# raw-lab/mercat2

Measured on AMD Instinct MI355X. Metric: bases/sec at k=31, 10Mx150bp, higher is better.
Workload: dtype u64

## Files before the change

### include/mercat_hip.h

```cpp
#ifndef MERCAT_HIP_H
#define MERCAT_HIP_H

#include <stddef.h>
#include <stdint.h>

#ifdef __cplusplus
extern "C" {
#endif

#define MK_OK 0
#define MK_ERR_ARG (-1)
#define MK_ERR_HIP (-2)
#define MK_ERR_NOMEM (-3)
#define MK_ERR_STATE (-4)
#define MK_ERR_NON_ASCII (-5)
#define MK_ERR_IO (-6)
#define MK_ERR_RANGE (-7)
#define MK_ERR_UNSUPPORTED (-8)

#define MK_ALPHABET_NT2 0
#define MK_ALPHABET_AA5 1
#define MK_ALPHABET_RAW 2

typedef struct mk_ctx mk_ctx;

typedef struct mk_stats_t {
  uint64_t raw_bytes;
  uint64_t symbols;
  uint64_t windows;
  uint64_t exotic_windows;
  uint64_t chunks;
  uint64_t survivors;
  uint64_t rows;
  uint64_t table_slots;
  int32_t mode;
  int32_t profiled;
  double ms_parse, ms_pack, ms_count, ms_exotic, ms_filter, ms_export;
  uint64_t n_parse, n_pack, n_count, n_exotic, n_filter, n_export;
  double ms_part;
  uint64_t n_part;
  uint64_t records;
  uint64_t distinct;
  uint64_t part_retries;
  uint64_t part_reused;
  uint64_t fused_chunks;
  uint64_t fuse_spilled;
  uint64_t parse_retries;
} mk_stats_t;

int mk_create(int device, int alphabet, int k, mk_ctx** out);
int mk_device_count(void);
void mk_destroy(mk_ctx* ctx);
const char* mk_last_error(const mk_ctx* ctx);
int mk_reset(mk_ctx* ctx);
int mk_reset_for(mk_ctx* ctx, uint64_t expect_rows);
int mk_set_canonical(mk_ctx* ctx, int on);

int mk_set_clean(mk_ctx* ctx, int on, int toupper);
typedef struct mk_clean_gpu_t {
  uint64_t raw_bytes;
  uint64_t symbols;
  uint64_t gc_count;
  uint64_t n_bytes;
  uint64_t n_runs;
  uint64_t header_lines;
  uint64_t last_runs;
} mk_clean_gpu_t;
int mk_clean_stats(mk_ctx* ctx, mk_clean_gpu_t* out);
int mk_clean_runs(mk_ctx* ctx, uint64_t* starts, uint64_t* ends, size_t cap, size_t* n);

int mk_chunk_begin(mk_ctx* ctx);
int mk_chunk_feed(mk_ctx* ctx, const uint8_t* text, size_t n);
int mk_chunk_feed_device(mk_ctx* ctx, const uint8_t* d_text, size_t n);
int mk_chunk_end(mk_ctx* ctx, uint64_t min_count);
int mk_count_device(mk_ctx* ctx, const uint8_t* d_text, size_t n, uint64_t min_count);

typedef struct mk_file_stats_t {
  uint64_t disk_bytes;
  uint64_t text_bytes;
  uint64_t chunks;
  int32_t gz;
  int32_t chunked;
  int32_t members;
  int32_t threads;
  int32_t contexts;
  int32_t devices;
  int32_t split_pieces;
  int32_t pad_;
  double s_wait_io;
  double s_wait_gpu;
  double s_total;
  double s_merge;
  double s_setup;
  double s_scan;
  double s_feed;
  double s_retire;
  double s_drain;
} mk_file_stats_t;
int mk_count_file(mk_ctx* const* ctxs, int nctx, const char* path, uint64_t chunk_bytes, uint64_t min_count,
                  int threads, mk_file_stats_t* st);

int mk_export_size(mk_ctx* ctx, size_t* rows);
int mk_export(mk_ctx* ctx, uint8_t* kmers, uint64_t* counts, size_t rows_cap);
int mk_write_tsv(mk_ctx* ctx, const char* path, const char* basename, size_t* rows);

typedef struct mk_export_stats_t {
  uint64_t rows;
  uint64_t bytes;
  double s_sort;
  double s_d2h;
  double s_format;
  double s_write;
  double s_total;
} mk_export_stats_t;
int mk_export_stats(mk_ctx* ctx, mk_export_stats_t* out);

int mk_merged_export(mk_ctx* const* ctxs, int n, uint8_t* kmers, uint64_t* matrix, size_t rows_cap, size_t* rows);
int mk_write_merged_tsv(mk_ctx* const* ctxs, int n, const char* const* names, const char* first_column,
                        const char* path, size_t* rows);
int mk_write_merged_tsv_as_reference(mk_ctx* const* ctxs, int n, const char* const* names, const char* first_column,
                                     const char* path, size_t* rows);
int mk_write_merged_tsv_t(mk_ctx* const* ctxs, int n, const char* const* names, const char* path, size_t* rows);
typedef struct mk_alpha_t {
  uint64_t observed;
  uint64_t total;
  uint64_t freq[11];
  double sum_sq;
  double sum_clnc;
} mk_alpha_t;
int mk_alpha_stats(mk_ctx* ctx, mk_alpha_t* out);

int mk_trim(mk_ctx* ctx);

int mk_export_pairs_device(mk_ctx* ctx, uint64_t* d_keys, uint64_t* d_counts, size_t cap, size_t* rows);
int mk_import_pairs_device(mk_ctx* ctx, const uint64_t* d_keys, const uint64_t* d_counts, size_t rows);
int mk_export_exotic(mk_ctx* ctx, uint8_t* kmers, uint64_t* counts, size_t cap, size_t* rows);
int mk_import_exotic(mk_ctx* ctx, const uint8_t* kmers, const uint64_t* counts, size_t rows);
int mk_words_per_key(const mk_ctx* ctx);
int mk_merge_from(mk_ctx* dst, mk_ctx* src);

int mk_share_table(mk_ctx* ctx, mk_ctx* owner);

int mk_owner_bounds(int key_bits, int n, uint64_t* bounds);
int mk_plan_contexts(const int* devices, int ndev, int streams, int* ctx_device);
int mk_bucket_rows_device(mk_ctx* ctx, const uint64_t* bounds, int n, uint64_t* d_rows, size_t cap_rows, uint64_t* counts);
int mk_import_rows_device(mk_ctx* ctx, const uint64_t* d_rows, size_t rows);

int mk_sample_keys(mk_ctx* ctx, size_t stride, uint64_t* out, size_t cap, size_t* n);
int mk_dense_bins_device(mk_ctx* ctx, uint64_t* d_bins, size_t nbins, int store);

#define MK_MERGE_RANGES 0
#define MK_MERGE_GATHER 1
#define MK_MERGE_BALANCED 2
#define MK_MERGE_RCCL 4
typedef struct mk_merge_stats_t {
  uint64_t rows_in;
  uint64_t rows_out;
  uint64_t rows_moved;
  uint64_t bytes_moved;
  uint64_t max_owned;
  int32_t contexts, devices;
  int32_t peer_direct;
  int32_t rccl;
  double s_bucket, s_copy, s_import, s_total;
} mk_merge_stats_t;
int mk_merge_devices(mk_ctx* const* ctxs, int n, int flags, mk_merge_stats_t* st);
int mk_export_size_multi(mk_ctx* const* ctxs, int n, size_t* rows);
int mk_export_multi(mk_ctx* const* ctxs, int n, uint8_t* kmers, uint64_t* counts, size_t rows_cap);
int mk_write_tsv_multi(mk_ctx* const* ctxs, int n, const char* path, const char* basename, size_t* rows);

int mk_filter_min(mk_ctx* ctx, uint64_t min_count);

int mk_set_profiling(mk_ctx* ctx, int on);
int mk_get_stats(mk_ctx* ctx, mk_stats_t* out);
int mk_reset_stats(mk_ctx* ctx);

int mk_chunk_cuts(const uint8_t* text, size_t n, uint64_t chunksize, uint64_t* cuts, size_t cap, size_t* ncuts);
int mk_stream_cuts(const uint8_t* text, size_t n, uint64_t chunksize, size_t block, uint64_t* cuts, size_t cap,
                   size_t* ncuts);
int mk_record_cuts(const uint8_t* text, size_t n, uint64_t piece, size_t block, uint64_t* cuts, size_t cap, size_t* ncuts);
int mk_gunzip(const uint8_t* gz, size_t n, uint8_t* out, size_t cap, size_t block, size_t* written, int* members);
int mk_gunzip_parallel(const uint8_t* gz, size_t n, uint8_t* out, size_t cap, int threads, size_t piece_bytes,
                       size_t* written, int* members);
uint32_t mk_crc32_of(const uint8_t* p, size_t n, uint32_t seed);
typedef struct mk_clean_stats_t {
  uint64_t gc_count;
  uint64_t total_length;
  uint64_t records, split_records, pieces, n_runs;
  int64_t unsupported_record;
} mk_clean_stats_t;
int mk_remove_n(const uint8_t* text, size_t n, int toupper, uint8_t** out, size_t* out_len, mk_clean_stats_t* st);
void mk_free(void* p);
int mk_textwrap(const uint8_t* text, size_t n, size_t width, uint8_t** out, size_t* out_len);
int mk_synth_reads(uint64_t genome_len, uint64_t genome_seed, uint64_t reads, uint32_t read_len,
                   uint64_t read_seed, uint32_t sub_ppm, uint64_t first_index, uint8_t* out, size_t cap,
                   size_t* written);
const char* mk_version(void);

#ifdef __cplusplus
}
#endif
#endif
```

### mercat2_amd/csrc/mk_api.hip

```cpp
#include "mk_common.h"
#include <algorithm>
#include <chrono>
#include <cstdio>
#include <cstdlib>
#include <cstring>
#include <new>
#include <thread>

typedef unsigned long long u64;

static thread_local std::string g_err;

static size_t pow2_at_least(size_t v) {
  size_t p = 1024;
  while (p < v) p <<= 1;
  return p;
}

static void drain_table_users(mk_ctx* t);

int mk_buf_reserve(mk_ctx* c, MkDevBuf& b, size_t bytes, bool keep) {
  if (bytes <= b.cap) return MK_OK;
  size_t want = bytes;
  if (keep && b.cap) want = std::max(bytes, b.cap + b.cap / 2);
  want = (want + 255) & ~(size_t)255;
  void* p = nullptr;
  hipError_t e = hipMalloc(&p, want);
  if (e != hipSuccess) {
    c->err = "hipMalloc(" + std::to_string(want) + " bytes): " + hipGetErrorString(e);
    return MK_ERR_NOMEM;
  }
  if (b.p) {
    if (keep) {
      e = hipMemcpyAsync(p, b.p, b.cap, hipMemcpyDeviceToDevice, c->stream);
      if (e == hipSuccess) e = hipStreamSynchronize(c->stream);
      if (e != hipSuccess) {
        (void)hipFree(p);
        c->err = std::string("hipMemcpy (grow): ") + hipGetErrorString(e);
        return MK_ERR_HIP;
      }
    } else {
      (void)hipStreamSynchronize(c->stream);
    }
    (void)hipFree(b.p);
  }
  b.p = p;
  b.cap = want;
  return MK_OK;
}

static void buf_free(MkDevBuf& b) {
  if (b.p) (void)hipFree(b.p);
  b.p = nullptr;
  b.cap = 0;
}

static hipEvent_t get_event(mk_ctx* c) {
  if (!c->event_pool.empty()) {
    hipEvent_t e = c->event_pool.back();
    c->event_pool.pop_back();
    return e;
  }
  hipEvent_t e = nullptr;
  (void)hipEventCreate(&e);
  return e;
}

void mk_prof_begin(mk_ctx* c, int id) {
  if (!c->profile) return;
  MkEventPair p{get_event(c), get_event(c), id};
  (void)hipEventRecord(p.a, c->stream);
  c->events.push_back(p);
}

void mk_prof_end(mk_ctx* c) {
  if (!c->profile || c->events.empty()) return;
  (void)hipEventRecord(c->events.back().b, c->stream);
}

static void prof_collect(mk_ctx* c) {
  if (c->events.empty()) return;
  (void)hipStreamSynchronize(c->stream);
  double* ms[MK_K_NUM] = {&c->st.ms_parse, &c->st.ms_pack, &c->st.ms_count, &c->st.ms_exotic, &c->st.ms_filter, &c->st.ms_export, &c->st.ms_part};
  uint64_t* nn[MK_K_NUM] = {&c->st.n_parse, &c->st.n_pack, &c->st.n_count, &c->st.n_exotic, &c->st.n_filter, &c->st.n_export, &c->st.n_part};
  for (auto& p : c->events) {
    float t = 0.f;
    if (hipEventElapsedTime(&t, p.a, p.b) == hipSuccess) {
      *ms[p.id] += t;
      *nn[p.id] += 1;
    }
    c->event_pool.push_back(p.a);
    c->event_pool.push_back(p.b);
  }
  c->events.clear();
}

extern "C" const char* mk_version(void) { return "mercat_hip 4.0 (gfx950)"; }

extern "C" int mk_device_count(void) {
  int n = 0;
  if (hipGetDeviceCount(&n) != hipSuccess) { (void)hipGetLastError(); return 0; }
  return n < 0 ? 0 : n;
}

extern "C" const char* mk_last_error(const mk_ctx* c) { return c ? c->err.c_str() : g_err.c_str(); }

extern "C" int mk_words_per_key(const mk_ctx* c) { return c ? (c->mode == MK_MODE_HASH128 ? 2 : 1) : 0; }

static void fold_pending(mk_ctx* c) {
  if (!c->pending_rows) return;
  const MkChunkInfo* p = c->h_info + 1;
  if (c->mode == MK_MODE_HASH128) c->run128_rows += (size_t)p->new_rows;
  else c->run_rows += (size_t)p->new_rows;
  c->run_ref_rows += (size_t)p->new_rows_ref;
  c->pending_rows = false;
}

static int pull_info(mk_ctx* c) {
  if (c->clean_mode && c->clean_meta.p) MK_HIP(hipMemcpyAsync(c->h_clean, c->clean_meta.p, 8 * sizeof(u64), hipMemcpyDeviceToHost, c->stream));
  MK_HIP(hipMemcpyAsync(c->h_info, c->info.p, sizeof(MkChunkInfo), hipMemcpyDeviceToHost, c->stream));
  MK_HIP(hipStreamSynchronize(c->stream));
  fold_pending(c);
  return MK_OK;
}

static int settle(mk_ctx* c) {
  if (!c->pending_rows) return MK_OK;
  MK_HIP(hipSetDevice(c->device));
  MK_HIP(hipStreamSynchronize(c->stream));
  fold_pending(c);
  return MK_OK;
}

int mk_settle(mk_ctx* c) { return settle(c); }
int mk_pull_info(mk_ctx* c) { return pull_info(c); }

extern "C" int mk_create(int device, int alphabet, int k, mk_ctx** out) {
  if (!out) { g_err = "mk_create: out is NULL"; return MK_ERR_ARG; }
  *out = nullptr;
  if (k < 1 || k > (1 << 20)) { g_err = "mk_create: k must be in [1, 2^20]"; return MK_ERR_ARG; }
  if (alphabet != MK_ALPHABET_NT2 && alphabet != MK_ALPHABET_AA5 && alphabet != MK_ALPHABET_RAW) {
    g_err = "mk_create: unknown alphabet";
    return MK_ERR_ARG;
  }
  int ndev = 0;
  hipError_t e = hipGetDeviceCount(&ndev);
  if (e != hipSuccess || ndev <= 0) {
    g_err = std::string("mk_create: no HIP device (") + (e == hipSuccess ? "0 devices" : hipGetErrorString(e)) +
            "); this engine has no CPU fallback";
    return MK_ERR_HIP;
  }
  if (device < 0 || device >= ndev) { g_err = "mk_create: device index out of range"; return MK_ERR_ARG; }
  mk_ctx* c = new (std::nothrow) mk_ctx();
  if (!c) { g_err = "mk_create: out of host memory"; return MK_ERR_NOMEM; }
  c->device = device;
  c->alphabet = alphabet;
  c->k = k;
  c->bits = alphabet == MK_ALPHABET_NT2 ? 2 : (alphabet == MK_ALPHABET_AA5 ? 5 : 0);
  c->syms_per_word = alphabet == MK_ALPHABET_NT2 ? 32 : 12;
  const long kb = (long)k * c->bits;
  c->mode = (c->bits == 0) ? MK_MODE_BYREF : (kb <= 15 ? MK_MODE_DENSE : (kb <= 64 ? MK_MODE_HASH64 : MK_MODE_BYREF));
  if (alphabet == MK_ALPHABET_NT2 && k >= 33 && k <= 64) c->mode = MK_MODE_HASH128;
  if (alphabet == MK_ALPHABET_AA5 && k >= 13 && k <= 25 && !getenv("MK_NO_AA128")) c->mode = MK_MODE_HASH128;
  c->st.mode = c->mode;
  c->use_partition = getenv("MK_NO_PARTITION") ? 0 : 1;
  c->use_fast_parse = getenv("MK_NO_FAST_PARSE") ? 0 : 1;
  c->use_superkmer = getenv("MK_NO_SUPERKMER") ? 0 : 1;
  c->use_superkmer2 = getenv("MK_NO_SUPERKMER2") ? 0 : 1;
  c->run_bucket_major = (getenv("MK_BUCKET_MAJOR") && alphabet == MK_ALPHABET_NT2 && c->mode == MK_MODE_HASH64 && k >= 12 && k <= 32) ? 1 : 0;
  if (const char* e = getenv("MK_SK_MIN_K")) { const int v = atoi(e); if (v >= 12 && v <= 33) c->sk_min_k = v; }
  int rc = MK_OK;
  auto fail = [&](int code, const std::string& msg) {
    g_err = msg;
    mk_destroy(c);
    return code;
  };
  if ((e = hipSetDevice(device)) != hipSuccess) return fail(MK_ERR_HIP, std::string("hipSetDevice: ") + hipGetErrorString(e));
  if ((e = hipStreamCreateWithFlags(&c->stream, hipStreamNonBlocking)) != hipSuccess)
    return fail(MK_ERR_HIP, std::string("hipStreamCreate: ") + hipGetErrorString(e));
  c->use_speculation = getenv("MK_NO_SPECULATION") ? 0 : 1;
  c->use_reuse = getenv("MK_NO_REUSE") ? 0 : 1;
  c->use_fused = getenv("MK_NO_FUSE") ? 0 : 1;
  c->dup_hint = 2.0;
  c->nk_hint = 5.0;
  if ((e = hipHostMalloc((void**)&c->h_info, 2 * sizeof(MkChunkInfo) + 8 * sizeof(u64), hipHostMallocDefault)) != hipSuccess)
    return fail(MK_ERR_HIP, std::string("hipHostMalloc: ") + hipGetErrorString(e));
  c->h_clean = (u64*)(c->h_info + 2);
  if ((rc = mk_buf_reserve(c, c->info, sizeof(MkChunkInfo) + 64)) != MK_OK) return fail(rc, c->err);
  if (c->mode == MK_MODE_DENSE) {
    const size_t bytes = ((size_t)1 << kb) * sizeof(u64);
    if ((rc = mk_buf_reserve(c, c->ctab, bytes)) != MK_OK) return fail(rc, c->err);
    if ((rc = mk_buf_reserve(c, c->run, bytes)) != MK_OK) return fail(rc, c->err);
    (void)hipMemsetAsync(c->ctab.p, 0, bytes, c->stream);
    (void)hipMemsetAsync(c->run.p, 0, bytes, c->stream);
    c->ctab_slots = c->run_slots = (size_t)1 << kb;
  }
  if ((e = hipStreamSynchronize(c->stream)) != hipSuccess)
    return fail(MK_ERR_HIP, std::string("hipStreamSynchronize: ") + hipGetErrorString(e));
  *out = c;
  return MK_OK;
}

extern "C" void mk_destroy(mk_ctx* c) {
  if (!c) return;
  (void)hipSetDevice(c->device);
  if (c->stream) (void)hipStreamSynchronize(c->stream);
  if (c->share_owner) (void)mk_share_table(c, nullptr);
  for (mk_ctx* s : std::vector<mk_ctx*>(c->sharers)) (void)mk_share_table(s, nullptr);
  for (auto& p : c->events) { (void)hipEventDestroy(p.a); (void)hipEventDestroy(p.b); }
  for (auto& e : c->event_pool) (void)hipEventDestroy(e);
  MkDevBuf* all[] = {&c->raw, &c->seq, &c->codes, &c->bad, &c->tile_maps, &c->info, &c->ctab, &c->rtab_chunk, &c->run,
                     &c->run_ref, &c->arena, &c->run128, &c->ex128, &c->ex128_out, &c->ex_keys, &c->ex_cnts, &c->ex_keys2, &c->ex_cnts2, &c->ex_tmp, &c->part, &c->part_meta, &c->surv_keys, &c->surv_cnts, &c->surv_keys2,
                     &c->xfer_out, &c->xfer_in, &c->xfer_meta, &c->clean_meta, &c->clean_runs};
  for (auto* b : all) buf_free(*b);
  if (c->h_info) (void)hipHostFree(c->h_info);
  if (c->ingest_ring) (void)hipHostFree(c->ingest_ring);
  if (c->tsv_pin) { (void)hipHostUnregister(c->tsv_pin); free(c->tsv_pin); }
  if (c->stream) (void)hipStreamDestroy(c->stream);
  delete c;
}

static int reset_impl(mk_ctx* c, size_t expect_rows) {
  if (!c) return MK_ERR_ARG;
  MK_HIP(hipSetDevice(c->device));
  if (c->pending_rows) { MK_HIP(hipStreamSynchronize(c->stream)); c->pending_rows = false; }
  std::unique_lock<std::shared_mutex> table_lock(c->table_mu, std::defer_lock);
  if (!c->sharers.empty()) { table_lock.lock(); drain_table_users(c); }
  if (expect_rows && c->mode != MK_MODE_DENSE) {
    const size_t want = pow2_at_least(4 * expect_rows);
    if (c->run_slots > want) c->run_slots = want;
    if (c->run128_slots > want) c->run128_slots = want;
  }
  if (c->mode == MK_MODE_DENSE) {
    MK_HIP(hipMemsetAsync(c->run.p, 0, c->run_slots * sizeof(u64), c->stream));
  } else if (c->run_slots) {
    int rc = mk_launch_clear_slots(c, (MkSlot*)c->run.p, c->run_slots);
    if (rc) return rc;
  }
  if (c->run_ref_slots) {
    int rc = mk_launch_clear_slots(c, (MkSlot*)c->run_ref.p, c->run_ref_slots);
    if (rc) return rc;
  }
  if (c->run128_slots) MK_HIP(hipMemsetAsync(c->run128.p, 0, c->run128_slots * sizeof(MkSlot128), c->stream));
  c->run_rows = 0;
  c->run_ref_rows = 0;
  c->run128_rows = 0;
  c->run_side = 0;
  c->in_chunk = false;
  c->raw_len = 0;
  c->part_reuse_ok = false;
  c->dup_known = false;
  c->fuse_cap = 0;
  c->clean_n_runs = c->clean_n_bytes = c->clean_gc = c->clean_symbols = c->clean_raw = c->clean_headers = c->clean_last_runs = 0;
  MK_HIP(hipStreamSynchronize(c->stream));
  return MK_OK;
}
extern "C" int mk_reset(mk_ctx* c) { return reset_impl(c, 0); }
extern "C" int mk_reset_for(mk_ctx* c, uint64_t expect_rows) { return reset_impl(c, (size_t)(expect_rows ? expect_rows : 1)); }

extern "C" int mk_set_canonical(mk_ctx* c, int on) {
  if (!c) return MK_ERR_ARG;
  { int rc_ = settle(c); if (rc_) return rc_; }
  if (on && c->alphabet != MK_ALPHABET_NT2) { c->err = "mk_set_canonical: only the nucleotide alphabet has a reverse complement"; return MK_ERR_ARG; }
  if (on && c->mode != MK_MODE_DENSE && c->mode != MK_MODE_HASH64 && !(c->mode == MK_MODE_HASH128 && c->use_superkmer2)) {
    c->err = "mk_set_canonical: canonical counting is implemented for nucleotide k <= 64 (two-word keys: on the partitioned path only)";
    return MK_ERR_ARG;
  }
  c->part_reuse_ok = false;
  if (c->in_chunk || c->run_rows || c->run_ref_rows || c->run128_rows || c->run_side || c->st.chunks) {
    if ((on != 0) != (c->canonical != 0) && (c->run_rows || c->run_ref_rows || c->run128_rows || c->run_side || c->in_chunk)) {
      c->err = "mk_set_canonical: the running table already holds rows counted in the other mode (mk_reset first)";
      return MK_ERR_STATE;
    }
  }
  c->canonical = on ? 1 : 0;
  return MK_OK;
}

extern "C" int mk_set_clean(mk_ctx* c, int on, int toupper) {
  if (!c) return MK_ERR_ARG;
  if (on && c->alphabet != MK_ALPHABET_NT2) { c->err = "mk_set_clean: removeN applies to nucleotide FASTA (bin/mercat2.py:276)"; return MK_ERR_ARG; }
  if (c->in_chunk) { c->err = "mk_set_clean: a chunk is open"; return MK_ERR_STATE; }
  c->clean_mode = on ? 1 : 0;
  c->clean_upper = (on && toupper) ? 1 : 0;
  return MK_OK;
}

extern "C" int mk_clean_stats(mk_ctx* c, mk_clean_gpu_t* out) {
  if (!c || !out) return MK_ERR_ARG;
  out->raw_bytes = c->clean_raw;
  out->symbols = c->clean_symbols;
  out->gc_count = c->clean_gc;
  out->n_bytes = c->clean_n_bytes;
  out->n_runs = c->clean_n_runs;
  out->header_lines = c->clean_headers;
  out->last_runs = c->clean_last_runs;
  return MK_OK;
}

extern "C" int mk_clean_runs(mk_ctx* c, uint64_t* starts, uint64_t* ends, size_t cap, size_t* n) {
  if (!c || !n || (cap && (!starts || !ends))) return MK_ERR_ARG;
  if ((size_t)c->clean_last_runs > ((size_t)1 << 16)) {
    *n = 0;
    c->err = "mk_clean_runs: the last chunk holds " + std::to_string(c->clean_last_runs) + " runs of N, more than the 65536 the list keeps";
    return MK_ERR_RANGE;
  }
  const size_t kept = (size_t)c->clean_last_runs;
  *n = kept;
  if (!kept || !cap) return MK_OK;
  MK_HIP(hipSetDevice(c->device));
  std::vector<u64> a(kept), b(kept);
  MK_HIP(hipMemcpyAsync(a.data(), c->clean_runs.p, kept * 8, hipMemcpyDeviceToHost, c->stream));
  MK_HIP(hipMemcpyAsync(b.data(), (const u64*)c->clean_runs.p + ((size_t)1 << 16), kept * 8, hipMemcpyDeviceToHost, c->stream));
  MK_HIP(hipStreamSynchronize(c->stream));
  std::sort(a.begin(), a.end());
  std::sort(b.begin(), b.end());
  for (size_t i = 0; i < kept && i < cap; ++i) { starts[i] = a[i]; ends[i] = b[i]; }
  return MK_OK;
}

static int grow_run64(mk_ctx* c, size_t need_rows);
static int grow_run64_body(mk_ctx* c, size_t need_rows);
static mk_ctx* table_of_ctx(mk_ctx* c) { return c->share_owner ? c->share_owner : c; }

static void drain_table_users(mk_ctx* t) {
  (void)hipStreamSynchronize(t->stream);
  for (mk_ctx* s : t->sharers) (void)hipStreamSynchronize(s->stream);
}

extern "C" int mk_share_table(mk_ctx* c, mk_ctx* owner) {
  if (!c || c == owner) return MK_ERR_ARG;
  if (c->in_chunk) { c->err = "mk_share_table: a chunk is open"; return MK_ERR_STATE; }
  if (c->share_owner == owner) return MK_OK;
  if (c->share_owner) {
    mk_ctx* old = c->share_owner;
    std::unique_lock<std::shared_mutex> wr(old->table_mu);
    (void)hipSetDevice(c->device);
    (void)hipStreamSynchronize(c->stream);
    old->sharers.erase(std::remove(old->sharers.begin(), old->sharers.end(), c), old->sharers.end());
    c->share_owner = nullptr;
    c->fuse_target = nullptr;
  }
  if (!owner) return MK_OK;
  if (owner->share_owner || !c->sharers.empty()) { c->err = "mk_share_table: tables are shared one level deep (the owner must own its table, a sharer cannot be an owner)"; return MK_ERR_ARG; }
  if (owner->device != c->device || owner->alphabet != c->alphabet || owner->k != c->k || owner->canonical != c->canonical || owner->mode != c->mode) {
    c->err = "mk_share_table: contexts differ in device, alphabet, k or canonical mode";
    return MK_ERR_ARG;
  }
  if (c->mode != MK_MODE_HASH64) { c->err = "mk_share_table: only one-word hashed tables are shared"; return MK_ERR_ARG; }
  std::unique_lock<std::shared_mutex> wr(owner->table_mu);
  owner->sharers.push_back(c);
  c->share_owner = owner;
  return MK_OK;
}

extern "C" int mk_chunk_begin(mk_ctx* c) {
  if (!c) return MK_ERR_ARG;
  if (c->in_chunk) { c->err = "mk_chunk_begin: a chunk is already open"; return MK_ERR_STATE; }
  c->in_chunk = true;
  c->raw_len = 0;
  return MK_OK;
}

static int feed(mk_ctx* c, const uint8_t* p, size_t n, hipMemcpyKind kind) {
  if (!c) return MK_ERR_ARG;
  if (!c->in_chunk) { c->err = "mk_chunk_feed: no open chunk (call mk_chunk_begin)"; return MK_ERR_STATE; }
  if (n == 0) return MK_OK;
  if (!p) { c->err = "mk_chunk_feed: text is NULL"; return MK_ERR_ARG; }
  MK_HIP(hipSetDevice(c->device));
  int rc = mk_buf_reserve(c, c->raw, c->raw_len + n + 64, true);
  if (rc) return rc;
  MK_HIP(hipMemcpyAsync((uint8_t*)c->raw.p + c->raw_len, p, n, kind, c->stream));
  if (kind == hipMemcpyHostToDevice) MK_HIP(hipStreamSynchronize(c->stream));
  c->raw_len += n;
  return MK_OK;
}

int mk_feed_host_async(mk_ctx* c, const uint8_t* p, size_t n, bool wait) {
  if (!c || !c->in_chunk) return MK_ERR_STATE;
  if (n == 0) return MK_OK;
  MK_HIP(hipSetDevice(c->device));
  int rc = mk_buf_reserve(c, c->raw, c->raw_len + n + 64, true);
  if (rc) return rc;
  MK_HIP(hipMemcpyAsync((uint8_t*)c->raw.p + c->raw_len, p, n, hipMemcpyHostToDevice, c->stream));
  if (wait) MK_HIP(hipStreamSynchronize(c->stream));
  c->raw_len += n;
  return MK_OK;
}

int mk_reserve_raw(mk_ctx* c, size_t bytes) {
  MK_HIP(hipSetDevice(c->device));
  return mk_buf_reserve(c, c->raw, bytes, true);
}

extern "C" int mk_chunk_feed(mk_ctx* c, const uint8_t* text, size_t n) { return feed(c, text, n, hipMemcpyHostToDevice); }
extern "C" int mk_chunk_feed_device(mk_ctx* c, const uint8_t* d_text, size_t n) {
  return feed(c, d_text, n, hipMemcpyDeviceToDevice);
}

static size_t run_slots_for(size_t need_rows) {
  static const bool x4 = getenv("MK_GROW_X4") != nullptr;
  return pow2_at_least(x4 ? 4 * need_rows : need_rows * 5 / 2);
}

static int grow_run64_body(mk_ctx* c, size_t need_rows);
static int grow_run64(mk_ctx* c, size_t need_rows) {
  if (c->sharers.empty()) return grow_run64_body(c, need_rows);
  std::unique_lock<std::shared_mutex> wr(c->table_mu);
  if (2 * need_rows <= c->run_slots) return MK_OK;
  drain_table_users(c);
  return grow_run64_body(c, need_rows);
}
static int grow_run64_body(mk_ctx* c, size_t need_rows) {
  if (2 * need_rows <= c->run_slots) return MK_OK;
  const size_t slots = run_slots_for(need_rows);
  MkDevBuf nb;
  int rc = mk_buf_reserve(c, nb, slots * sizeof(MkSlot));
  if (rc) return rc;
  if ((rc = mk_launch_clear_slots(c, (MkSlot*)nb.p, slots)) != MK_OK) return rc;
  if (c->run_slots && (rc = mk_launch_rehash64(c, (const MkSlot*)c->run.p, c->run_slots, (MkSlot*)nb.p, slots)) != MK_OK) return rc;
  MK_HIP(hipStreamSynchronize(c->stream));
  buf_free(c->run);
  c->run = nb;
  c->run_slots = slots;
  return MK_OK;
}

static int grow_run128(mk_ctx* c, size_t need_rows) {
  if (2 * need_rows <= c->run128_slots) return MK_OK;
  const size_t slots = pow2_at_least(4 * need_rows);
  MkDevBuf nb;
  int rc = mk_buf_reserve(c, nb, slots * sizeof(MkSlot128));
  if (rc) return rc;
  MK_HIP(hipMemsetAsync(nb.p, 0, slots * sizeof(MkSlot128), c->stream));
  if (c->run128_slots && (rc = mk_launch_rehash128(c, (const MkSlot128*)c->run128.p, c->run128_slots, (MkSlot128*)nb.p, slots)) != MK_OK) return rc;
  MK_HIP(hipStreamSynchronize(c->stream));
  buf_free(c->run128);
  c->run128 = nb;
  c->run128_slots = slots;
  return MK_OK;
}

static int grow_run_ref(mk_ctx* c, size_t need_rows) {
  int rc;
  if (need_rows > c->arena_rows_cap) {
    const size_t rows = std::max(need_rows, c->arena_rows_cap * 2);
    if ((rc = mk_buf_reserve(c, c->arena, rows * (size_t)c->k + 64, true)) != MK_OK) return rc;
    c->arena_rows_cap = rows;
  }
  if (2 * need_rows <= c->run_ref_slots) return MK_OK;
  const size_t slots = pow2_at_least(4 * need_rows);
  MkDevBuf nb;
  if ((rc = mk_buf_reserve(c, nb, slots * sizeof(MkSlot))) != MK_OK) return rc;
  if ((rc = mk_launch_clear_slots(c, (MkSlot*)nb.p, slots)) != MK_OK) return rc;
  if (c->run_ref_slots &&
      (rc = mk_launch_rehash_ref(c, (const MkSlot*)c->run_ref.p, c->run_ref_slots, (MkSlot*)nb.p, slots)) != MK_OK)
    return rc;
  MK_HIP(hipStreamSynchronize(c->stream));
  buf_free(c->run_ref);
  c->run_ref = nb;
  c->run_ref_slots = slots;
  return MK_OK;
}

int mk_grow_run(mk_ctx* c, size_t more_rows) {
  if (c->mode == MK_MODE_HASH64) return grow_run64(c, c->run_rows + more_rows);
  if (c->mode == MK_MODE_HASH128) return grow_run128(c, c->run128_rows + more_rows);
  return MK_OK;
}

bool mk_binned_takes(const mk_ctx* c);
int mk_launch_count_binned(mk_ctx* c, size_t seq_len, uint64_t min_count);

#define MK_RETRY_GENERAL 1

static int process_chunk_fast(mk_ctx* c, const uint8_t* d_raw, size_t n, u64 min_count) {
  int rc;
  const size_t begin = (size_t)((uintptr_t)d_raw & 15);
  const uint8_t* d_al = d_raw - begin;
  MK_HIP(hipSetDevice(c->device));
  MK_HIP(hipMemsetAsync(c->info.p, 0, sizeof(MkChunkInfo), c->stream));
  if ((rc = mk_buf_reserve(c, c->seq, n + 256)) != MK_OK) return rc;
  const size_t bad_words = n / 64 + 4;
  if ((rc = mk_buf_reserve(c, c->bad, (bad_words + 2) * 8)) != MK_OK) return rc;
  if ((rc = mk_buf_reserve(c, c->codes, (2 * bad_words + 8) * 8)) != MK_OK) return rc;
  static const bool always_seq = getenv("MK_ALWAYS_SEQ") != nullptr;
  if ((rc = mk_launch_fparse(c, d_al, begin, n, true, always_seq)) != MK_OK) return rc;
  const bool two = c->mode == MK_MODE_HASH128;
  c->rtab_chunk_slots = 0;
  c->surv_regions = 0;
  c->ctab_slots = 0;
  c->fuse_cap = 0;
  if (!two && c->use_fused && min_count >= 2 && c->surv_hint_ok && !c->run_bucket_major) {
    static const bool cores = getenv("MK_CORES") != nullptr;
    const unsigned long long per_bucket = (c->surv_hint >> 13) * (cores ? 2 : 1);
    const int cap = per_bucket <= 110 ? 512 : (per_bucket <= 360 ? 1024 : 0);
    if (cap) {
      if ((rc = settle(c)) != MK_OK) return rc;
      mk_ctx* t = table_of_ctx(c);
      static const bool roomy = getenv("MK_FUSE_ROOMY") != nullptr;
      const size_t expect = (roomy ? 2 * (size_t)c->surv_hint : (size_t)c->surv_hint) + 4096;
      if (t != c) {
        std::shared_lock<std::shared_mutex> rd(t->table_mu);
        size_t rows_now;
        { std::lock_guard<std::mutex> g(t->rows_mu); rows_now = t->run_rows; }
        if (t->run_slots < 1024 || 2 * (rows_now + expect) > t->run_slots) t = c;
      }
      if (t == c) {
        size_t rows_now;
        { std::lock_guard<std::mutex> g(c->rows_mu); rows_now = c->run_rows; }
        if ((rc = grow_run64(c, rows_now + expect * (1 + c->sharers.size()))) != MK_OK) return rc;
      }
      c->fuse_target = t;
      c->fuse_cap = cap;
    }
  }
  {
    mk_ctx* t = c->fuse_cap ? c->fuse_target : c;
    std::shared_lock<std::shared_mutex> rd(t->table_mu, std::defer_lock);
    if (t != c) rd.lock();
    rc = two ? mk_launch_count_superkmer2(c, n, min_count) : mk_launch_count_superkmer(c, n, min_count);
  }
  c->fuse_cap = 0;
  if (rc) return rc;
  const bool fused = !two && c->fused_last;
  if ((rc = pull_info(c)) != MK_OK) return rc;
  MkChunkInfo* h = c->h_info;
  if (h->parse_fallback) { c->st.parse_retries += 1; return MK_RETRY_GENERAL; }
  if (h->non_ascii) {
    c->err = "input holds " + std::to_string(h->non_ascii) +
             " sequence byte(s) >= 0x80 (non-ASCII sequence text is not supported; the chunk was not counted)";
    return MK_ERR_NON_ASCII;
  }
  const size_t seq_len = (size_t)h->seq_len;
  if (h->bad_symbols) {
    if (!always_seq) {
      if ((rc = mk_buf_reserve(c, c->ex_tmp, sizeof(MkChunkInfo) + 64)) != MK_OK) return rc;
      MK_HIP(hipMemcpyAsync(c->ex_tmp.p, c->info.p, sizeof(MkChunkInfo), hipMemcpyDeviceToDevice, c->stream));
      if ((rc = mk_launch_fparse(c, d_al, begin, n, false, true)) != MK_OK) return rc;
      MK_HIP(hipMemcpyAsync(c->info.p, c->ex_tmp.p, sizeof(MkChunkInfo), hipMemcpyDeviceToDevice, c->stream));
    }
    const u64 bound = std::min<u64>((u64)seq_len, h->bad_symbols * (u64)c->k);
    c->rtab_chunk_slots = pow2_at_least(2 * (size_t)bound);
    if ((rc = mk_buf_reserve(c, c->rtab_chunk, c->rtab_chunk_slots * sizeof(MkSlot))) != MK_OK) return rc;
    if ((rc = mk_launch_clear_slots(c, (MkSlot*)c->rtab_chunk.p, c->rtab_chunk_slots)) != MK_OK) return rc;
    if ((rc = mk_launch_count_byref(c, seq_len, true)) != MK_OK) return rc;
    if ((rc = mk_launch_count_survivors(c, min_count)) != MK_OK) return rc;
    if ((rc = pull_info(c)) != MK_OK) return rc;
  }
  if (h->part_overflow) {
    if (!c->part_sampled) { c->err = "partition overflow without sampling (internal error)"; return MK_ERR_STATE; }
    if (getenv("MK_VERBOSE")) fprintf(stderr, "[mk] sampled partition too small (where=%llu): exact pass\n", h->part_overflow);
    h->windows = h->records = h->distinct = h->survivors = h->side = h->errors = h->part_overflow = 0;
    MK_HIP(hipMemcpyAsync(c->info.p, h, sizeof(MkChunkInfo), hipMemcpyHostToDevice, c->stream));
    c->st.part_retries += 1;
    rc = two ? mk_launch_count_superkmer2(c, seq_len, min_count, true) : mk_launch_count_superkmer(c, seq_len, min_count, true);
    if (rc) return rc;
    if ((rc = pull_info(c)) != MK_OK) return rc;
    if (h->part_overflow) { c->err = "partition overflow after the exact pass (internal error: nothing was counted)"; return MK_ERR_STATE; }
  }
  if (h->errors) {
    c->err = "counting kernel reported " + std::to_string(h->errors) + " unrecoverable condition(s) (bucket too large to split)";
    return MK_ERR_RANGE;
  }
  c->part_dirty = false;
  const bool fused_done = !two && c->fused_last;
  if (fused_done) {
    {
      mk_ctx* t = c->fuse_target ? c->fuse_target : c;
      std::lock_guard<std::mutex> g(t->rows_mu);
      t->run_rows += (size_t)h->new_rows;
    }
    h->new_rows = 0;
    c->st.fused_chunks += 1;
    c->st.fuse_spilled += h->spilled;
    if (h->spilled || h->survivors_ref)
      MK_HIP(hipMemsetAsync(&((MkChunkInfo*)c->info.p)->new_rows, 0, sizeof(unsigned long long), c->stream));
    if (h->spilled) {
      if ((rc = grow_run64(c, c->run_rows + (size_t)h->spilled)) != MK_OK) return rc;
      if ((rc = mk_launch_import_pairs(c, (const uint64_t*)c->surv_keys.p, (const uint64_t*)c->surv_cnts.p, (size_t)h->spilled)) != MK_OK) return rc;
    }
  }
  (void)fused;
  if (!two && !fused_done && h->survivors && (rc = grow_run64(c, c->run_rows + (size_t)h->survivors)) != MK_OK) return rc;
  if (h->survivors_ref && (rc = grow_run_ref(c, c->run_ref_rows + (size_t)h->survivors_ref)) != MK_OK) return rc;
  if (two && (h->survivors || h->survivors_ref) &&
      (rc = grow_run128(c, c->run128_rows + (size_t)h->survivors + (size_t)h->survivors_ref)) != MK_OK) return rc;
  if (h->survivors && seq_len && !fused_done) {
    const size_t p1 = (size_t)1 << c->p1_log2;
    const uint64_t* meta = (const uint64_t*)c->part_meta.p;
    mk_prof_begin(c, MK_K_FILTER);
    rc = two ? mk_launch_import128_regions(c, (const uint64_t*)c->surv_keys.p, (const uint64_t*)c->surv_keys2.p,
                                           (const uint64_t*)c->surv_cnts.p, meta + 4 * p1 + 1, meta + 6 * p1 + 2, p1)
             : mk_launch_import_regions(c, (const uint64_t*)c->surv_keys.p, (const uint64_t*)c->surv_cnts.p,
                                        meta + 4 * p1 + 1, meta + 6 * p1 + 2, p1, (size_t)h->survivors);
    mk_prof_end(c);
    if (rc) return rc;
  }
  if ((rc = mk_launch_accumulate(c, min_count)) != MK_OK) return rc;
  if (!fused_done || h->spilled || h->survivors_ref) {
    MK_HIP(hipMemcpyAsync(c->h_info + 1, c->info.p, sizeof(MkChunkInfo), hipMemcpyDeviceToHost, c->stream));
    c->pending_rows = true;
  }
  if (h->side && h->side >= min_count) c->run_side += h->side;
  const bool full_chunk = !c->dup_known || seq_len * 4 >= c->part_prev_len * 3;
  if (!two && (full_chunk || !c->surv_hint_ok)) { c->surv_hint = h->survivors; c->surv_hint_ok = true; }
  if (h->distinct && full_chunk) { c->dup_hint = (double)h->windows / (double)h->distinct; c->dup_known = true; }
  if (h->records) { c->nk_hint = (double)(h->windows + h->exotic) / (double)h->records; c->items_hint = (double)h->records * 32.0 / (double)(seq_len ? seq_len : 1); }
  if (getenv("MK_VERBOSE"))
    fprintf(stderr, "[mk] chunk (one read-back): raw=%zu seq=%zu windows=%llu records=%llu distinct=%llu survivors=%llu p1=2^%d dup=%.2f nk=%.2f fused=%d spilled=%llu rows=%zu slots=%zu\n",
            n, seq_len, (unsigned long long)h->windows, (unsigned long long)h->records, (unsigned long long)h->distinct,
            (unsigned long long)h->survivors, c->p1_log2, c->dup_hint, c->nk_hint, fused_done ? 1 : 0, (unsigned long long)h->spilled,
            c->run_rows, c->run_slots);
  c->st.table_slots = c->rtab_chunk_slots;
  c->st.raw_bytes += n;
  c->st.symbols += h->symbols;
  c->st.windows += h->windows + h->exotic;
  c->st.exotic_windows += h->exotic;
  c->st.chunks += 1;
  c->st.records += h->records;
  c->st.distinct += h->distinct;
  c->st.survivors += h->survivors + h->survivors_ref + ((h->side && h->side >= min_count) ? 1 : 0);
  return MK_OK;
}

static int process_chunk(mk_ctx* c, const uint8_t* d_raw, size_t n, u64 min_count) {
  int rc;
  bool known_blank = false;
  if (c->clean_mode) {
    if (!c->use_fast_parse) { c->err = "clean mode needs the fast parser (MK_NO_FAST_PARSE is set)"; return MK_ERR_UNSUPPORTED; }
    if (d_raw != (const uint8_t*)c->raw.p) { c->err = "clean mode rewrites the text in place: feed it (mk_chunk_feed), do not pass caller memory"; return MK_ERR_STATE; }
    MK_HIP(hipSetDevice(c->device));
    if ((rc = mk_launch_clean_pre(c, (uint8_t*)c->raw.p, n)) != MK_OK) return rc;
  }
  if (!c->clean_mode && c->use_speculation && c->use_fast_parse && c->alphabet == MK_ALPHABET_NT2 && n && n < 0xFE000000ull &&
      ((c->mode == MK_MODE_HASH64 && c->use_partition && c->use_superkmer && c->k >= c->sk_min_k && c->k <= 32) ||
       (c->mode == MK_MODE_HASH128 && c->use_superkmer2))) {
    rc = process_chunk_fast(c, d_raw, n, min_count);
    if (rc != MK_RETRY_GENERAL) return rc;
    known_blank = true;
  }
  if ((rc = settle(c)) != MK_OK) return rc;
  const size_t begin = (size_t)((uintptr_t)d_raw & 15);
  const uint8_t* d_al = d_raw - begin;
  MK_HIP(hipSetDevice(c->device));
  MK_HIP(hipMemsetAsync(c->info.p, 0, sizeof(MkChunkInfo), c->stream));
  if ((rc = mk_buf_reserve(c, c->seq, n + 256)) != MK_OK) return rc;
  const bool packed = c->mode != MK_MODE_BYREF;
  const size_t bad_words = n / 64 + 4;
  const size_t code_words = c->alphabet == MK_ALPHABET_NT2 ? 2 * bad_words : (bad_words * 64 + 11) / 12;
  if (packed) {
    if ((rc = mk_buf_reserve(c, c->bad, (bad_words + 2) * 8)) != MK_OK) return rc;
    if ((rc = mk_buf_reserve(c, c->codes, (code_words + 8) * 8)) != MK_OK) return rc;
  }
  for (int attempt = 0; attempt < 2; ++attempt) {
    const bool fast = c->use_fast_parse && attempt == 0 && !known_blank;
    const bool fused = fast && packed && c->alphabet == MK_ALPHABET_NT2;
    if (!fast && begin) {
      if ((rc = mk_buf_reserve(c, c->raw, n + 64)) != MK_OK) return rc;
      MK_HIP(hipMemcpyAsync(c->raw.p, d_raw, n, hipMemcpyDeviceToDevice, c->stream));
      d_raw = (const uint8_t*)c->raw.p;
    }
    if ((rc = fast ? mk_launch_fparse(c, d_al, begin, n, fused) : mk_launch_parse(c, d_raw, n)) != MK_OK) return rc;
    if (packed && !fused && (rc = mk_launch_pack(c, n)) != MK_OK) return rc;
    if (c->clean_mode && (rc = mk_launch_clean_post(c, n)) != MK_OK) return rc;
    if ((rc = pull_info(c)) != MK_OK) return rc;
    if (c->clean_mode) {
      const u64* m = c->h_clean;
      const u64 headers = c->h_info->seq_len - c->h_info->symbols;
      const char* why = c->h_info->parse_fallback ? "a blank inside a sequence line"
                        : m[2]                    ? "a 0x7F byte in the text, or blanks in front of the first header"
                        : m[1] != headers         ? "a '>' that does not start a header line"
                                                  : nullptr;
      if (why) {
        c->err = std::string("clean mode: ") + why + " (removeN's rewrite of such text is not reproduced on the GPU; nothing was counted)";
        return MK_ERR_UNSUPPORTED;
      }
      c->clean_raw += n;
      c->clean_headers += headers;
      c->clean_n_bytes += m[3];
      c->clean_n_runs += m[4];
      c->clean_gc += m[5];
      c->clean_symbols += c->h_info->symbols - m[3];
      c->clean_last_runs = m[4];
      c->h_info->symbols -= m[3];
      break;
    }
    if (!fast || !c->h_info->parse_fallback) break;
    c->st.parse_retries += 1;
    MK_HIP(hipMemsetAsync(c->info.p, 0, sizeof(MkChunkInfo), c->stream));
  }
  if (c->h_info->non_ascii) {
    c->err = "input holds " + std::to_string(c->h_info->non_ascii) +
             " sequence byte(s) >= 0x80 (non-ASCII sequence text is not supported; the chunk was not counted)";
    return MK_ERR_NON_ASCII;
  }
  const size_t seq_len = (size_t)c->h_info->seq_len;
  const u64 bad_symbols = c->h_info->bad_symbols;

  c->rtab_chunk_slots = 0;
  const bool partitioned = c->mode == MK_MODE_HASH64 && c->use_partition;
  c->surv_regions = 0;
  c->ctab_slots = c->mode == MK_MODE_DENSE ? c->ctab_slots : 0;
  if (c->mode == MK_MODE_HASH64 && !partitioned) {
    c->ctab_slots = pow2_at_least(2 * seq_len);
    if ((rc = mk_buf_reserve(c, c->ctab, c->ctab_slots * sizeof(MkSlot))) != MK_OK) return rc;
    if ((rc = mk_launch_clear_slots(c, (MkSlot*)c->ctab.p, c->ctab_slots)) != MK_OK) return rc;
  }
  const bool sk2 = c->mode == MK_MODE_HASH128 && c->alphabet == MK_ALPHABET_NT2 && c->use_superkmer2 && seq_len < 0xFFFFFF00ull;
  if (c->mode == MK_MODE_HASH128 && c->canonical && !sk2) {
    c->err = "canonical counting of 33..64-mers needs the partitioned path (chunk of 4 G symbols or more)";
    return MK_ERR_RANGE;
  }
  if (c->mode == MK_MODE_BYREF || (c->mode == MK_MODE_HASH128 && !sk2)) {
    c->rtab_chunk_slots = pow2_at_least(2 * seq_len);
  } else if (bad_symbols) {
    const u64 bound = std::min<u64>((u64)seq_len, bad_symbols * (u64)c->k);
    c->rtab_chunk_slots = pow2_at_least(2 * (size_t)bound);
  }
  if (c->rtab_chunk_slots) {
    if ((rc = mk_buf_reserve(c, c->rtab_chunk, c->rtab_chunk_slots * sizeof(MkSlot))) != MK_OK) return rc;
    if ((rc = mk_launch_clear_slots(c, (MkSlot*)c->rtab_chunk.p, c->rtab_chunk_slots)) != MK_OK) return rc;
  }
  c->st.table_slots = (c->mode == MK_MODE_BYREF || c->mode == MK_MODE_HASH128) ? c->rtab_chunk_slots : c->ctab_slots;

  if (c->mode == MK_MODE_DENSE) rc = mk_launch_count_dense(c, seq_len);
  else if (partitioned) {
    const bool sk = c->use_superkmer && c->alphabet == MK_ALPHABET_NT2 && c->k >= c->sk_min_k && c->k <= 32 && seq_len < 0xFE000000ull;
    const bool binned = !sk && mk_binned_takes(c) && seq_len < 0xFFFFFF00ull;
    rc = sk ? mk_launch_count_superkmer(c, seq_len, min_count)
            : (binned ? mk_launch_count_binned(c, seq_len, min_count) : mk_launch_count_partitioned(c, seq_len, min_count));
  }
  else if (c->mode == MK_MODE_HASH64) rc = mk_launch_count_hash64(c, seq_len);
  else if (c->mode == MK_MODE_HASH128) rc = sk2 ? mk_launch_count_superkmer2(c, seq_len, min_count) : mk_launch_count_ref128(c, seq_len);
  if (rc) return rc;
  if (c->rtab_chunk_slots && (c->mode != MK_MODE_HASH128 || bad_symbols) &&
      (rc = mk_launch_count_byref(c, seq_len, packed)) != MK_OK) return rc;

  if ((rc = mk_launch_count_survivors(c, min_count)) != MK_OK) return rc;
  if ((rc = pull_info(c)) != MK_OK) return rc;
  if (c->h_info->part_overflow) {
    if (!c->part_sampled) { c->err = "partition overflow without sampling (internal error)"; return MK_ERR_STATE; }
    MkChunkInfo* h = c->h_info;
    if (getenv("MK_VERBOSE")) fprintf(stderr, "[mk] sampled partition too small (where=%llu: 1 records total, 2 survivors total, 4 a bucket, 8 a survivor region): exact pass\n", h->part_overflow);
    h->windows = h->records = h->distinct = h->survivors = h->side = h->errors = h->part_overflow = 0;
    MK_HIP(hipMemcpyAsync(c->info.p, h, sizeof(MkChunkInfo), hipMemcpyHostToDevice, c->stream));
    c->st.part_retries += 1;
    rc = sk2 ? mk_launch_count_superkmer2(c, seq_len, min_count, true)
             : mk_launch_count_superkmer(c, seq_len, min_count, true);
    if (rc) return rc;
    if ((rc = pull_info(c)) != MK_OK) return rc;
    if (c->h_info->part_overflow) { c->err = "partition overflow after the exact pass (internal error: nothing was counted)"; return MK_ERR_STATE; }
  }
  if (c->h_info->errors) {
    c->err = "counting kernel reported " + std::to_string(c->h_info->errors) + " unrecoverable condition(s) (bucket too large to split)";
    return MK_ERR_RANGE;
  }
  c->part_dirty = false;
  if (c->mode == MK_MODE_HASH64 && c->h_info->survivors)
    if ((rc = grow_run64(c, c->run_rows + (size_t)c->h_info->survivors)) != MK_OK) return rc;
  if (c->h_info->survivors_ref)
    if ((rc = grow_run_ref(c, c->run_ref_rows + (size_t)c->h_info->survivors_ref)) != MK_OK) return rc;
  if (c->mode == MK_MODE_HASH128 && (c->h_info->survivors || c->h_info->survivors_ref))
    if ((rc = grow_run128(c, c->run128_rows + (size_t)c->h_info->survivors + (size_t)c->h_info->survivors_ref)) != MK_OK) return rc;
  if (sk2 && c->surv_regions == 2 && seq_len && c->h_info->survivors) {
    const size_t p1 = (size_t)1 << c->p1_log2;
    const uint64_t* meta = (const uint64_t*)c->part_meta.p;
    mk_prof_begin(c, MK_K_FILTER);
    rc = mk_launch_import128_regions(c, (const uint64_t*)c->surv_keys.p, (const uint64_t*)c->surv_keys2.p,
                                     (const uint64_t*)c->surv_cnts.p, meta + 4 * p1 + 1, meta + 6 * p1 + 2, p1);
    mk_prof_end(c);
    if (rc) return rc;
  }
  if (partitioned && c->h_info->survivors) {
    mk_prof_begin(c, MK_K_FILTER);
    if (c->surv_regions) {
      const size_t p1 = (size_t)1 << c->p1_log2;
      const uint64_t* meta = (const uint64_t*)c->part_meta.p;
      rc = mk_launch_import_regions(c, (const uint64_t*)c->surv_keys.p, (const uint64_t*)c->surv_cnts.p,
                                    meta + 4 * p1 + 1, meta + 6 * p1 + 2, p1, (size_t)c->h_info->survivors);
    } else {
      rc = mk_launch_import_pairs(c, (const uint64_t*)c->surv_keys.p, (const uint64_t*)c->surv_cnts.p, (size_t)c->h_info->survivors, true);
    }
    mk_prof_end(c);
    if (rc) return rc;
  }
  if ((rc = mk_launch_accumulate(c, min_count)) != MK_OK) return rc;
  if ((rc = pull_info(c)) != MK_OK) return rc;
  if (c->mode == MK_MODE_HASH128) c->run128_rows += (size_t)c->h_info->new_rows;
  else c->run_rows += (size_t)c->h_info->new_rows;
  c->run_ref_rows += (size_t)c->h_info->new_rows_ref;
  if (c->h_info->side && c->h_info->side >= min_count) c->run_side += c->h_info->side;
  if (partitioned && c->h_info->distinct) { c->dup_hint = (double)c->h_info->windows / (double)c->h_info->distinct; c->dup_known = true; }
  if (sk2 && c->h_info->distinct) { c->dup_hint = (double)c->h_info->windows / (double)c->h_info->distinct; c->dup_known = true; }
  if ((partitioned || sk2) && c->h_info->records) {
    c->nk_hint = (double)(c->h_info->windows + c->h_info->exotic) / (double)c->h_info->records;
    c->items_hint = (double)c->h_info->records * 32.0 / (double)(seq_len ? seq_len : 1);
  }

  if (getenv("MK_VERBOSE"))
    fprintf(stderr, "[mk] chunk: raw=%zu seq=%zu windows=%llu records=%llu distinct=%llu survivors=%llu new_rows=%llu p1=2^%d dup=%.2f nk=%.2f\n", n, seq_len,
            (unsigned long long)c->h_info->windows, (unsigned long long)c->h_info->records, (unsigned long long)c->h_info->distinct,
            (unsigned long long)c->h_info->survivors, (unsigned long long)c->h_info->new_rows, c->p1_log2, c->dup_hint, c->nk_hint);
  c->st.raw_bytes += n;
  c->st.symbols += c->h_info->symbols;
  c->st.windows += c->h_info->windows + c->h_info->exotic;
  c->st.exotic_windows += c->h_info->exotic;
  c->st.chunks += 1;
  c->st.records += c->h_info->records;
  c->st.distinct += c->h_info->distinct;
  c->st.survivors += c->h_info->survivors + c->h_info->survivors_ref +
                     ((c->h_info->side && c->h_info->side >= min_count) ? 1 : 0);
  return MK_OK;
}

extern "C" int mk_chunk_end(mk_ctx* c, uint64_t min_count) {
  if (!c) return MK_ERR_ARG;
  if (!c->in_chunk) { c->err = "mk_chunk_end: no open chunk"; return MK_ERR_STATE; }
  c->in_chunk = false;
  int rc = process_chunk(c, (const uint8_t*)c->raw.p, c->raw_len, min_count);
  c->raw_len = 0;
  return rc;
}

extern "C" int mk_count_device(mk_ctx* c, const uint8_t* d_text, size_t n, uint64_t min_count) {
  if (!c) return MK_ERR_ARG;
  if (c->in_chunk) { c->err = "mk_count_device: a chunk is open"; return MK_ERR_STATE; }
  if (n && !d_text) { c->err = "mk_count_device: d_text is NULL"; return MK_ERR_ARG; }
  if (!c->clean_mode && (((uintptr_t)d_text & 15) == 0 || c->use_fast_parse)) return process_chunk(c, d_text, n, min_count);
  int rc = mk_chunk_begin(c);
  if (!rc) rc = mk_chunk_feed_device(c, d_text, n);
  if (rc) { c->in_chunk = false; return rc; }
  return mk_chunk_end(c, min_count);
}

struct ExportView {
  std::vector<u64> pkeys, pcnts;
  int words = 1;
  size_t packed_rows() const { return pcnts.size(); }
  std::vector<uint8_t> rstr;
  std::vector<u64> rcnt;
  std::vector<u64> rorder;
};

static int gather_packed(mk_ctx* c, ExportView& v, u64* d_keys_out, u64* d_cnts_out, size_t cap, size_t* rows_out,
                         bool to_host) {
  int rc;
  size_t rows = 0;
  const auto t_gather = std::chrono::steady_clock::now();
  if (c->mode == MK_MODE_DENSE) {
    const size_t nbins = c->run_slots;
    std::vector<u64> bins(nbins);
    MK_HIP(hipMemcpyAsync(bins.data(), c->run.p, nbins * sizeof(u64), hipMemcpyDeviceToHost, c->stream));
    MK_HIP(hipStreamSynchronize(c->stream));
    for (size_t i = 0; i < nbins; ++i)
      if (bins[i]) { v.pkeys.push_back(i); v.pcnts.push_back(bins[i]); }
    rows = v.pkeys.size();
    if (!to_host) {
      if (rows > cap) { c->err = "export: device buffers too small"; return MK_ERR_RANGE; }
      if (rows) {
        MK_HIP(hipMemcpyAsync(d_keys_out, v.pkeys.data(), rows * 8, hipMemcpyHostToDevice, c->stream));
        MK_HIP(hipMemcpyAsync(d_cnts_out, v.pcnts.data(), rows * 8, hipMemcpyHostToDevice, c->stream));
        MK_HIP(hipStreamSynchronize(c->stream));
      }
    }
  } else if (c->mode == MK_MODE_HASH64) {
    rows = c->run_rows;
    const size_t side = c->run_side ? 1 : 0;
    if (!to_host && rows + side > cap) { c->err = "export: device buffers too small"; return MK_ERR_RANGE; }
    if (rows) {
      mk_prof_begin(c, MK_K_EXPORT);
      if ((rc = mk_buf_reserve(c, c->ex_keys, rows * 8 + 64)) != MK_OK) return rc;
      if ((rc = mk_buf_reserve(c, c->ex_cnts, rows * 8 + 64)) != MK_OK) return rc;
      u64* d_cursor = (u64*)((char*)c->info.p + sizeof(MkChunkInfo));
      MK_HIP(hipMemsetAsync(d_cursor, 0, 8, c->stream));
      if ((rc = mk_launch_compact(c, (const MkSlot*)c->run.p, c->run_slots, (uint64_t*)c->ex_keys.p,
                                  (uint64_t*)c->ex_cnts.p, rows, (uint64_t*)d_cursor)) != MK_OK) return rc;
      u64* ok = d_keys_out;
      u64* oc = d_cnts_out;
      if (to_host) {
        if ((rc = mk_buf_reserve(c, c->ex_keys2, rows * 8 + 64)) != MK_OK) return rc;
        if ((rc = mk_buf_reserve(c, c->ex_cnts2, rows * 8 + 64)) != MK_OK) return rc;
        ok = (u64*)c->ex_keys2.p;
        oc = (u64*)c->ex_cnts2.p;
      }
      if ((rc = mk_sort_pairs(c, (const uint64_t*)c->ex_keys.p, (const uint64_t*)c->ex_cnts.p, (uint64_t*)ok,
                              (uint64_t*)oc, rows, c->bits * c->k)) != MK_OK) return rc;
      mk_prof_end(c);
      if (to_host) {
        MK_HIP(hipStreamSynchronize(c->stream));
        c->ex_st.s_sort += std::chrono::duration<double>(std::chrono::steady_clock::now() - t_gather).count();
        v.pkeys.resize(rows);
        v.pcnts.resize(rows);
        MK_HIP(hipMemcpyAsync(v.pkeys.data(), ok, rows * 8, hipMemcpyDeviceToHost, c->stream));
        MK_HIP(hipMemcpyAsync(v.pcnts.data(), oc, rows * 8, hipMemcpyDeviceToHost, c->stream));
      }
      u64 got = 0;
      MK_HIP(hipMemcpyAsync(&got, d_cursor, 8, hipMemcpyDeviceToHost, c->stream));
      MK_HIP(hipStreamSynchronize(c->stream));
      if (got != rows) {
        c->err = "export: table holds " + std::to_string(got) + " rows, expected " + std::to_string(rows);
        return MK_ERR_STATE;
      }
    }
    if (side) {
      if (to_host) { v.pkeys.push_back(MK_EMPTY); v.pcnts.push_back(c->run_side); }
      else {
        u64 kk = MK_EMPTY, cc = c->run_side;
        MK_HIP(hipMemcpyAsync(d_keys_out + rows, &kk, 8, hipMemcpyHostToDevice, c->stream));
        MK_HIP(hipMemcpyAsync(d_cnts_out + rows, &cc, 8, hipMemcpyHostToDevice, c->stream));
        MK_HIP(hipStreamSynchronize(c->stream));
      }
      rows += 1;
    }
  }
  else if (c->mode == MK_MODE_HASH128) {
    v.words = 2;
    rows = c->run128_rows;
    if (!to_host && rows > cap) { c->err = "export: device buffers too small"; return MK_ERR_RANGE; }
    if (rows) {
      mk_prof_begin(c, MK_K_EXPORT);
      if ((rc = mk_buf_reserve(c, c->ex128, 7 * rows * 8 + 64)) != MK_OK) return rc;
      u64* hi = (u64*)c->ex128.p;
      u64* lo = hi + rows;
// ... 896 lines not shown
```

### mercat2_amd/csrc/mk_common.h

```cpp
#pragma once
#include <hip/hip_runtime.h>
#include <stdint.h>
#include <stddef.h>
#include <string>
#include <mutex>
#include <shared_mutex>
#include <vector>
#include "../../include/mercat_hip.h"


#ifndef MK_SK_MIN_K
#define MK_SK_MIN_K 12
#endif
#define MK_SEP 0x0Au
#define MK_EMPTY 0xFFFFFFFFFFFFFFFFull

struct __attribute__((aligned(16))) MkSlot {
  unsigned long long key;
  unsigned long long cnt;
};

#define MK_LOCK128 0xFFFFFFFFFFFFFFFFull
struct __attribute__((aligned(32))) MkSlot128 {
  unsigned long long hi;
  unsigned long long lo;
  unsigned long long cnt;
  unsigned long long pad;
};

struct MkChunkInfo {
  unsigned long long seq_len;
  unsigned long long symbols;
  unsigned long long non_ascii;
  unsigned long long bad_symbols;
  unsigned long long windows;
  unsigned long long exotic;
  unsigned long long survivors;
  unsigned long long survivors_ref;
  unsigned long long side;
  unsigned long long new_rows;
  unsigned long long new_rows_ref;
  unsigned long long distinct;
  unsigned long long errors;
  unsigned long long parse_fallback;
  unsigned long long records;
  unsigned long long part_overflow;
  unsigned long long spilled;
};

enum MkMode { MK_MODE_DENSE = 0, MK_MODE_HASH64 = 1, MK_MODE_HASH128 = 2, MK_MODE_BYREF = 3 };
enum MkKernelId { MK_K_PARSE = 0, MK_K_PACK, MK_K_COUNT, MK_K_EXOTIC, MK_K_FILTER, MK_K_EXPORT, MK_K_PART, MK_K_NUM };

__host__ __device__ static inline unsigned long long mk_mix64(unsigned long long x) {
  x ^= x >> 30;
  x *= 0xBF58476D1CE4E5B9ull;
  x ^= x >> 27;
  x *= 0x94D049BB133111EBull;
  x ^= x >> 31;
  return x;
}

#define MK_POLY_B 0x9E3779B97F4A7C15ull

struct MkDevBuf {
  void* p = nullptr;
  size_t cap = 0;
};

struct mk_ctx;
int mk_buf_reserve(mk_ctx* c, MkDevBuf& b, size_t bytes, bool keep = false);
int mk_feed_host_async(mk_ctx* c, const uint8_t* p, size_t n, bool wait);
int mk_reserve_raw(mk_ctx* c, size_t bytes);

struct MkEventPair {
  hipEvent_t a, b;
  int id;
};

struct mk_ctx {
  int device = 0;
  int alphabet = 0;
  int k = 0;
  int bits = 0;
  int syms_per_word = 0;
  int mode = 0;
  hipStream_t stream = nullptr;
  std::string err;
  bool in_chunk = false;
  bool profile = false;

  MkDevBuf raw;
  size_t raw_len = 0;
  MkDevBuf seq, codes, bad;
  MkDevBuf tile_maps;
  MkDevBuf info;
  MkChunkInfo* h_info = nullptr;
  bool pending_rows = false;
  int use_speculation = 1;

  MkDevBuf ctab;
  size_t ctab_slots = 0;
  MkDevBuf rtab_chunk;
  size_t rtab_chunk_slots = 0;

  MkDevBuf run;
  size_t run_slots = 0;
  size_t run_rows = 0;
  unsigned long long run_side = 0;
  MkDevBuf run_ref;
  size_t run_ref_slots = 0;
  size_t run_ref_rows = 0;
  MkDevBuf arena;
  size_t arena_rows_cap = 0;
  MkDevBuf run128;
  size_t run128_slots = 0;
  size_t run128_rows = 0;

  MkDevBuf part;
  MkDevBuf part_meta;
  MkDevBuf surv_keys, surv_cnts;
  MkDevBuf surv_keys2;
  int use_superkmer2 = 1;
  int p1_log2 = 10;
  double dup_hint = 1.0;
  bool dup_known = false;
  int use_partition = 1;
  int use_fast_parse = 1;
  int canonical = 0;
  int use_superkmer = 1;
  int run_bucket_major = 0;
  int sk_min_k = MK_SK_MIN_K;
  bool part_sampled = false;
  bool part_reuse_ok = false;
  bool part_dirty = false;
  size_t part_prev_len = 0;
  int part_prev_p1 = 0;
  int part_nseg = 1;
  unsigned long long part_prev_minc = 0;
  int part_cooldown = 0;
  int use_reuse = 1;
  int surv_regions = 0;
  double nk_hint = 8.0;
  double items_hint = 0;
  int use_fused = 1;
  int fuse_cap = 0;
  bool fused_last = false;
  unsigned long long surv_hint = 0;
  bool surv_hint_ok = false;
  mk_ctx* share_owner = nullptr;
  mk_ctx* fuse_target = nullptr;
  std::vector<mk_ctx*> sharers;
  std::shared_mutex table_mu;
  std::mutex rows_mu;

  MkDevBuf ex_keys, ex_cnts, ex_keys2, ex_cnts2, ex_tmp;
  MkDevBuf ex128, ex128_out;

  int clean_mode = 0, clean_upper = 0;
  MkDevBuf clean_meta, clean_runs;
  unsigned long long* h_clean = nullptr;
  unsigned long long clean_n_runs = 0, clean_n_bytes = 0, clean_gc = 0, clean_symbols = 0, clean_raw = 0, clean_headers = 0;
  unsigned long long clean_last_runs = 0;

  MkDevBuf xfer_out, xfer_in, xfer_meta;

  void* ingest_ring = nullptr;
  size_t ingest_ring_bytes = 0;
  void* tsv_pin = nullptr;
  size_t tsv_pin_bytes = 0;

  mk_stats_t st{};
  mk_export_stats_t ex_st{};
  std::vector<MkEventPair> events;
  std::vector<hipEvent_t> event_pool;
};

#define MK_HIP(call)                                                                         \
  do {                                                                                       \
    hipError_t e__ = (call);                                                                 \
    if (e__ != hipSuccess) {                                                                 \
      c->err = std::string(#call) + ": " + hipGetErrorString(e__);                           \
      return MK_ERR_HIP;                                                                     \
    }                                                                                        \
  } while (0)

int mk_launch_parse(mk_ctx* c, const uint8_t* d_raw, size_t n);
int mk_launch_fparse(mk_ctx* c, const uint8_t* d_raw, size_t begin, size_t len, bool fuse_pack_nt, bool write_seq = true);
int mk_launch_pack(mk_ctx* c, size_t seq_cap);
int mk_launch_count_dense(mk_ctx* c, size_t seq_cap);
int mk_launch_count_hash64(mk_ctx* c, size_t seq_cap);
int mk_launch_count_byref(mk_ctx* c, size_t seq_cap, bool exotic_only);
int mk_launch_count_ref128(mk_ctx* c, size_t seq_len);
int mk_launch_count_partitioned(mk_ctx* c, size_t seq_len, uint64_t min_count);
int mk_launch_count_superkmer(mk_ctx* c, size_t seq_len, uint64_t min_count, bool exact = false);
bool mk_part_inherit(mk_ctx* c, size_t seq_len, int p1_log2, uint64_t min_count, bool sampled, bool exact);
void mk_launch_sk_scan(mk_ctx* c, const unsigned long long* hist, const unsigned long long* khist, unsigned long long* start,
                       unsigned* cursor, unsigned long long* kstart, int p1_log2, int sample_log2, int nkmax,
                       unsigned long long surv_div, unsigned long long part_cap, unsigned long long surv_cap, float sigmas,
                       int nseg);
int mk_launch_sk_count(mk_ctx* c, const unsigned long long* start, unsigned* cursor, const unsigned long long* kstart,
                       unsigned long long* nsurv, uint64_t min_count, int nkmax, size_t p1, bool exact, int nseg);
int mk_launch_sk_count_small(mk_ctx* c, const unsigned long long* start, unsigned* cursor, const unsigned long long* kstart,
                             unsigned long long* nsurv, uint64_t min_count, int nkmax, size_t p1, bool exact, int nseg);
int mk_launch_count_superkmer2(mk_ctx* c, size_t seq_len, uint64_t min_count, bool exact = false);
int mk_launch_import_ref128_regions(mk_ctx* c, const uint64_t* hi, const uint64_t* lo, const uint64_t* cnts,
                                    const uint64_t* kstart, const uint64_t* nsurv, size_t p1);
int mk_launch_clear_slots(mk_ctx* c, MkSlot* t, size_t slots);
int mk_launch_count_survivors(mk_ctx* c, uint64_t min_count);
int mk_sort_rows(mk_ctx* c, const uint8_t* d_arena, size_t rows, int k, uint64_t** d_order);
int mk_launch_rows_by_slot(mk_ctx* c, const uint64_t* slot_keys, const uint64_t* slot_cnts, size_t rows, uint64_t* cnt_by_row, uint64_t* d_bad);
int mk_launch_rows_gather(mk_ctx* c, const uint8_t* arena, const uint64_t* order, const uint64_t* cnt_by_row, size_t rows, int k,
                          uint8_t* out_rows, uint64_t* out_cnts);
int mk_launch_alpha(mk_ctx* c, unsigned long long* d_out);
int mk_launch_accumulate(mk_ctx* c, uint64_t min_count);
int mk_launch_merge_table64(mk_ctx* c, const MkSlot* from, size_t from_slots);
int mk_launch_rehash64(mk_ctx* c, const MkSlot* from, size_t from_slots, MkSlot* to, size_t to_slots);
int mk_launch_rehash_ref(mk_ctx* c, const MkSlot* from, size_t from_slots, MkSlot* to, size_t to_slots);
int mk_launch_import_pairs(mk_ctx* c, const uint64_t* d_keys, const uint64_t* d_counts, size_t rows, bool distinct = false);
int mk_launch_import_regions(mk_ctx* c, const uint64_t* d_keys, const uint64_t* d_counts, const uint64_t* kstart,
                             const uint64_t* nsurv, size_t p1, size_t survivors);
int mk_launch_import_ref(mk_ctx* c, const uint8_t* d_kmers, const uint64_t* d_counts, size_t rows);
int mk_launch_import128_regions(mk_ctx* c, const uint64_t* hi, const uint64_t* lo, const uint64_t* cnts, const uint64_t* kstart,
                                const uint64_t* nsurv, size_t p1);
int mk_launch_import128_pairs(mk_ctx* c, const uint64_t* d_keys2, const uint64_t* d_counts, size_t rows);
int mk_launch_refilter64(mk_ctx* c, const MkSlot* from, MkSlot* to, size_t slots, uint64_t min_count, uint64_t* d_kept);
int mk_launch_refilter128(mk_ctx* c, const MkSlot128* from, MkSlot128* to, size_t slots, uint64_t min_count, uint64_t* d_kept);
int mk_launch_refilter_dense(mk_ctx* c, uint64_t* bins, size_t nbins, uint64_t min_count);
int mk_launch_rehash128(mk_ctx* c, const MkSlot128* from, size_t from_slots, MkSlot128* to, size_t to_slots);
int mk_launch_compact128(mk_ctx* c, const MkSlot128* t, size_t slots, uint64_t* hi, uint64_t* lo, uint64_t* cnts, size_t cap,
                         uint64_t* d_cursor);
int mk_sort_pairs128(mk_ctx* c, const uint64_t* hi, const uint64_t* lo, const uint64_t* cnts, size_t n, int lo_bits,
                     uint64_t* scratch, uint64_t* keys2_out, uint64_t* cnts_out);
int mk_launch_compact(mk_ctx* c, const MkSlot* t, size_t slots, uint64_t* d_keys, uint64_t* d_counts, size_t cap,
                      uint64_t* d_cursor);
int mk_sort_pairs(mk_ctx* c, const uint64_t* keys_in, const uint64_t* vals_in, uint64_t* keys_out, uint64_t* vals_out,
                  size_t n, int key_bits);

int mk_settle(mk_ctx* c);
int mk_pull_info(mk_ctx* c);
int mk_grow_run(mk_ctx* c, size_t more_rows);
int mk_launch_import_rows(mk_ctx* c, const uint64_t* d_rows, size_t rows);

int mk_launch_clean_pre(mk_ctx* c, uint8_t* d_raw, size_t n);
int mk_launch_clean_post(mk_ctx* c, size_t seq_cap);

void mk_prof_begin(mk_ctx* c, int id);
void mk_prof_end(mk_ctx* c);
```

### mercat2_amd/csrc/mk_fparse.hip

```cpp
#include "mk_common.h"
#include "mk_device.h"

typedef unsigned long long u64;

#define FP_THREADS 256
#ifndef FP_SUB
#define FP_SUB 8
#endif
#define FP_WAVE_BYTES (FP_SUB * 1024)
#define FP_WAVES (FP_THREADS / 64)

struct FpEntry {
  unsigned a;
  unsigned b;
};

__device__ __forceinline__ uint4 classify16(const uint8_t* __restrict__ raw, size_t pos, size_t begin, size_t n, unsigned& nl,
                                            unsigned& gt, unsigned& st, unsigned& low, unsigned& hi) {
  uint4 v;
  if (pos + 16 <= n && pos >= begin) {
    v = *reinterpret_cast<const uint4*>(raw + pos);
  } else {
    unsigned w0 = 0, w1 = 0, w2 = 0, w3 = 0;
#pragma unroll
    for (int j = 0; j < 16; ++j) {
      const unsigned c = (pos + j < n && pos + j >= begin) ? (unsigned)raw[pos + j] : 10u;
      const unsigned sh = 8 * (j & 3);
      if (j < 4) w0 |= c << sh; else if (j < 8) w1 |= c << sh; else if (j < 12) w2 |= c << sh; else w3 |= c << sh;
    }
    v = make_uint4(w0, w1, w2, w3);
  }
#define FP_NZ7(t) ((((t) & 0x7F7F7F7Fu) + 0x7F7F7F7Fu) | (t))
  unsigned a_nl[2] = {0, 0}, a_gt[2] = {0, 0}, a_st[2] = {0, 0}, a_lo[2] = {0, 0}, a_hi[2] = {0, 0};
#pragma unroll
  for (int d = 0; d < 4; ++d) {
    const unsigned xd = d == 0 ? v.x : (d == 1 ? v.y : (d == 2 ? v.z : v.w));
    const unsigned K = (d & 1) ? 0x80402010u : 0x08040201u;
    const unsigned notnl = FP_NZ7(xd ^ 0x0A0A0A0Au) & FP_NZ7(xd ^ 0x0D0D0D0Du);
    const unsigned ge21 = ((xd & 0x7F7F7F7Fu) + 0x5F5F5F5Fu) | xd;
    a_nl[d >> 1] = __builtin_amdgcn_udot4(~notnl & 0x80808080u, K, a_nl[d >> 1], false);
    a_gt[d >> 1] = __builtin_amdgcn_udot4(~FP_NZ7(xd ^ 0x3E3E3E3Eu) & 0x80808080u, K, a_gt[d >> 1], false);
    a_st[d >> 1] = __builtin_amdgcn_udot4(~FP_NZ7(xd ^ 0x2A2A2A2Au) & 0x80808080u, K, a_st[d >> 1], false);
    a_lo[d >> 1] = __builtin_amdgcn_udot4(~ge21 & notnl & 0x80808080u, K, a_lo[d >> 1], false);
    a_hi[d >> 1] = __builtin_amdgcn_udot4(xd & 0x80808080u, K, a_hi[d >> 1], false);
  }
#undef FP_NZ7
  nl = (a_nl[0] >> 7) | ((a_nl[1] >> 7) << 8);
  gt = (a_gt[0] >> 7) | ((a_gt[1] >> 7) << 8);
  st = (a_st[0] >> 7) | ((a_st[1] >> 7) << 8);
  low = (a_lo[0] >> 7) | ((a_lo[1] >> 7) << 8);
  hi = (a_hi[0] >> 7) | ((a_hi[1] >> 7) << 8);
  return v;
}

__device__ __forceinline__ unsigned lane_header(unsigned start, unsigned nl, unsigned hin, unsigned& hout) {
  const unsigned p = ~nl & 0xFFFFu;
  const unsigned a = start | p, b = start;
  const unsigned sum = a + b + hin;
  const unsigned ci = sum ^ a ^ b;
  hout = (ci >> 16) & 1u;
  return (ci >> 1) & 0xFFFFu;
}

__device__ __forceinline__ unsigned wave_step(unsigned nl, unsigned gt, unsigned st, unsigned low, unsigned prev_nl,
                                              unsigned cin, unsigned& out, unsigned& sep, unsigned& bad_low,
                                              unsigned& last_nl) {
  const int lane = threadIdx.x & 63;
  const unsigned my_last_nl = (nl >> 15) & 1u;
  const unsigned prev = (unsigned)__builtin_amdgcn_update_dpp((int)prev_nl, (int)my_last_nl, 0x138, 0xf, 0xf, false);
  const unsigned ls = ((nl << 1) | prev) & 0xFFFFu;
  const unsigned start = ls & gt;
  unsigned hout0;
  (void)lane_header(start, nl, 0u, hout0);
  const u64 G = __ballot(hout0 != 0);
  const u64 P = __ballot(nl == 0);
  const u64 A = G | P, B = G;
  const u64 sum = A + B + (u64)cin;
  const u64 CI = sum ^ A ^ B;
  const unsigned hin = (unsigned)(CI >> lane) & 1u;
  unsigned hout;
  const unsigned H = lane_header(start, nl, hin, hout);
  sep = start;
  out = ((~H & ~nl & ~st) | start) & 0xFFFFu;
  bad_low = low & ~H;
  last_nl = mk_wave_last(my_last_nl);
  return mk_wave_last(hout);
}

__global__ __launch_bounds__(FP_THREADS) void mk_fparse_summ(const uint8_t* __restrict__ raw, size_t begin, size_t n, size_t nwaves,
                                                             FpEntry* __restrict__ entries, MkChunkInfo* __restrict__ info,
                                                             u64* __restrict__ zero_codes, u64* __restrict__ zero_bad,
                                                             size_t code_words, size_t bad_words) {
  const size_t wave = (size_t)blockIdx.x * FP_WAVES + (threadIdx.x >> 6);
  if (wave >= nwaves) return;
  const int lane = threadIdx.x & 63;
  const size_t base = wave * FP_WAVE_BYTES;
  if (zero_codes) {
    constexpr size_t CW = FP_WAVE_BYTES / 32, BW = FP_WAVE_BYTES / 64;
    const size_t c_end = wave + 1 == nwaves ? code_words : (wave + 1) * CW, b_end = wave + 1 == nwaves ? bad_words : (wave + 1) * BW;
    for (size_t w = wave * CW + (size_t)lane; w < c_end && w < code_words; w += 64) zero_codes[w] = 0ull;
    for (size_t w = wave * BW + (size_t)lane; w < b_end && w < bad_words; w += 64) zero_bad[w] = 0ull;
  }
  unsigned prev_nl = (base <= begin) ? 1u : ((raw[base - 1] == 10 || raw[base - 1] == 13) ? 1u : 0u);
  unsigned s0 = 0, s1 = 1, c0 = 0, c1 = 0, seps = 0, any_nl = 0, flag_low = 0;
#pragma unroll 1
  for (int sub = 0; sub < FP_SUB; ++sub) {
    const size_t pos = base + (size_t)sub * 1024 + (size_t)lane * 16;
    unsigned nl, gt, st, low, hi;
    (void)classify16(raw, pos, begin, n, nl, gt, st, low, hi);
    unsigned out, sep, bl, last_nl;
    const unsigned e0 = wave_step(nl, gt, st, low, prev_nl, s0, out, sep, bl, last_nl);
    c0 += __popc(out);
    seps += __popc(sep);
    (void)bl;
    if (s1 != s0) {
      unsigned out1, sep1, bl1, ln1;
      const unsigned e1 = wave_step(nl, gt, st, low, prev_nl, s1, out1, sep1, bl1, ln1);
      c1 += __popc(out1);
      s1 = e1;
    } else {
      c1 += __popc(out);
      s1 = e0;
    }
    s0 = e0;
    any_nl |= (__ballot(nl != 0) != 0) ? 1u : 0u;
    prev_nl = last_nl;
  }
  c0 = mk_wave_sum(c0);
  c1 = mk_wave_sum(c1);
  seps = mk_wave_sum(seps);
  (void)flag_low;
  if (lane == 0) {
    entries[wave].a = any_nl | (s0 << 1) | (seps << 2);
    entries[wave].b = c0 | (c1 << 16);
  }
}

struct FpScan {
  u64 off;
  unsigned st;
  unsigned pad;
};

__global__ __launch_bounds__(1024) void mk_fparse_scan(const FpEntry* __restrict__ entries, size_t nwaves,
                                                       FpScan* __restrict__ scan, MkChunkInfo* __restrict__ info,
                                                       u64* __restrict__ bad) {
  const size_t per = (nwaves + 1023) / 1024;
  const size_t lo = (size_t)threadIdx.x * per, hi = (lo + per < nwaves) ? lo + per : nwaves;
  unsigned e0 = 0, e1 = 1, has = 0;
  u64 c0 = 0, c1 = 0, nsep = 0;
  for (size_t w0 = lo; w0 < hi; w0 += 8) {
    FpEntry en[8];
#pragma unroll
    for (int i = 0; i < 8; ++i) en[i] = (w0 + i < hi) ? entries[w0 + i] : FpEntry{0u, 0u};
#pragma unroll
    for (int i = 0; i < 8; ++i) {
      if (w0 + i >= hi) break;
      const unsigned wnl = en[i].a & 1u, wx0 = (en[i].a >> 1) & 1u;
      const unsigned k0 = en[i].b & 0xFFFFu, k1 = en[i].b >> 16;
      nsep += en[i].a >> 2;
      c0 += e0 ? k1 : k0;
      c1 += e1 ? k1 : k0;
      e0 = wnl ? wx0 : (e0 | wx0);
      e1 = wnl ? wx0 : (e1 | wx0);
      has |= wnl;
    }
  }
  __shared__ unsigned long long w_G[16], w_P[16];
  __shared__ unsigned w_cin[16];
  __shared__ u64 w_cnt[16], w_sep[16];
  const int lane = threadIdx.x & 63, wv = threadIdx.x >> 6;
  const u64 G = __ballot(e0 != 0), P = __ballot(has == 0);
  if (lane == 0) { w_G[wv] = G; w_P[wv] = P; }
  __syncthreads();
  if (threadIdx.x == 0) {
    unsigned cin = 0;
    for (int w = 0; w < 16; ++w) {
      w_cin[w] = cin;
      const u64 A = w_G[w] | w_P[w], B = w_G[w];
      const u64 sum = A + B + cin;
      const u64 CI = sum ^ A ^ B;
      cin = (unsigned)((w_G[w] >> 63) | ((w_P[w] >> 63) & (CI >> 63))) & 1u;
    }
  }
  __syncthreads();
  unsigned q;
  {
    const u64 A = G | P, B = G;
    const u64 CI = (A + B + (u64)w_cin[wv]) ^ A ^ B;
    q = (unsigned)(CI >> lane) & 1u;
  }
  const u64 mine = q ? c1 : c0;
  u64 inc = mine;
#pragma unroll
  for (int d = 1; d < 64; d <<= 1) {
    const u64 up = __shfl_up(inc, d);
    if (lane >= d) inc += up;
  }
  for (int d = 32; d > 0; d >>= 1) nsep += __shfl_down(nsep, d);
  if (lane == 63) w_cnt[wv] = inc;
  if (lane == 0) w_sep[wv] = nsep;
  __syncthreads();
  u64 off = inc - mine;
  u64 total = 0, seps = 0;
#pragma unroll
  for (int w = 0; w < 16; ++w) {
    const u64 v = w_cnt[w];
    if (w < wv) off += v;
    total += v;
    seps += w_sep[w];
  }
  if (threadIdx.x == 0) {
    info->seq_len = total;
    info->symbols = total - seps;
    if (bad) {
      if (total & 63) atomicOr(&bad[total >> 6], ~0ull << (total & 63));
      const u64 w = (total + 63) >> 6;
      bad[w] = ~0ull;
      bad[w + 1] = ~0ull;
      bad[w + 2] = ~0ull;
    }
  }
  for (size_t w0 = lo; w0 < hi; w0 += 8) {
    FpEntry en[8];
#pragma unroll
    for (int i = 0; i < 8; ++i) en[i] = (w0 + i < hi) ? entries[w0 + i] : FpEntry{0u, 0u};
#pragma unroll
    for (int i = 0; i < 8; ++i) {
      if (w0 + i >= hi) break;
      scan[w0 + i].off = off;
      scan[w0 + i].st = q;
      const unsigned wnl = en[i].a & 1u, wx0 = (en[i].a >> 1) & 1u;
      off += q ? (en[i].b >> 16) : (en[i].b & 0xFFFFu);
      q = wnl ? wx0 : (q | wx0);
    }
  }
}

__global__ __launch_bounds__(FP_THREADS) void mk_fparse_emit(const uint8_t* __restrict__ raw, size_t begin, size_t n, size_t nwaves,
                                                             FpScan* __restrict__ scan, uint8_t* __restrict__ seq,
                                                             MkChunkInfo* __restrict__ info, u64* __restrict__ codes,
                                                             u64* __restrict__ bad, int write_seq) {
  __shared__ __attribute__((aligned(16))) uint8_t stage[FP_WAVES][64 + FP_WAVE_BYTES + 32 + 64 + 256];
  const int wv = threadIdx.x >> 6;
  const size_t wave = (size_t)blockIdx.x * FP_WAVES + wv;
  if (wave >= nwaves) return;
  const int lane = threadIdx.x & 63;
  const size_t base = wave * FP_WAVE_BYTES;
  const FpScan sc = scan[wave];
  const unsigned shift = (unsigned)(sc.off & 15);
  uint8_t* __restrict__ lds = stage[wv] + 64;
  unsigned prev_nl = (base <= begin) ? 1u : ((raw[base - 1] == 10 || raw[base - 1] == 13) ? 1u : 0u);
  unsigned state = sc.st;
  unsigned filled = 0;
  int nbad = 0;
  unsigned flag_low = 0;
  unsigned nhi = 0;
#pragma unroll 1
  for (int sub = 0; sub < FP_SUB; ++sub) {
    const size_t pos = base + (size_t)sub * 1024 + (size_t)lane * 16;
    unsigned nl, gt, st, low, hi;
    const uint4 v = classify16(raw, pos, begin, n, nl, gt, st, low, hi);
    unsigned out, sep, bl, last_nl;
    state = wave_step(nl, gt, st, low, prev_nl, state, out, sep, bl, last_nl);
    prev_nl = last_nl;
    flag_low |= bl;
    const unsigned cnt = __popc(out);
    nbad -= (int)__popc(sep);
    nhi += __popc(hi & out & ~sep);
    const unsigned inc = mk_wave_scan_incl(cnt);
    unsigned at = shift + filled + inc - cnt;
#define FP_BYTE(j) ((uint8_t)(((j) < 4 ? v.x : ((j) < 8 ? v.y : ((j) < 12 ? v.z : v.w))) >> (8 * ((j) & 3))))
    if (out == 0xFFFFu && sep == 0) {
#ifdef FP_BYTE_STORES
#pragma unroll
      for (int j = 0; j < 16; ++j) lds[at + j] = FP_BYTE(j);
#else
      __builtin_memcpy(lds + at, &v, 16);
#endif
    } else if (out) {
      const unsigned dump = FP_WAVE_BYTES + 32 + 64 + ((unsigned)lane << 2);
      unsigned a = at;
#pragma unroll
      for (int j = 0; j < 16; ++j) {
        const unsigned kept = (out >> j) & 1u;
        lds[kept ? a : dump] = FP_BYTE(j);
        a += kept;
      }
      for (unsigned sp = sep; sp; sp &= sp - 1) lds[at + __popc(out & ((1u << (__ffs(sp) - 1)) - 1u))] = (uint8_t)MK_SEP;
    }
#undef FP_BYTE
    filled += mk_wave_last(inc);
  }
  __builtin_amdgcn_wave_barrier();
  __threadfence_block();
  uint8_t* __restrict__ dst = seq + (sc.off - shift);
  const unsigned end = shift + filled;
  for (unsigned c = (unsigned)lane * 16; write_seq && c < end; c += 64 * 16) {
    if (c >= shift && c + 16 <= end) {
      *reinterpret_cast<uint4*>(dst + c) = *reinterpret_cast<const uint4*>(lds + c);
    } else {
      const unsigned lo = c < shift ? shift : c;
      const unsigned hi = c + 16 < end ? c + 16 : end;
      for (unsigned j = lo; j < hi; ++j) dst[j] = lds[j];
    }
  }
  if (codes) {
    const u64 g0 = sc.off, g1 = sc.off + filled;
    for (u64 b = (g0 >> 6) + lane; b < ((g1 + 63) >> 6); b += 64) {
      const u64 s_lo = b << 6, s_hi = s_lo + 64;
      const u64 lo = s_lo > g0 ? s_lo : g0, hi = s_hi < g1 ? s_hi : g1;
      u64 w0 = 0, w1 = 0, bd = 0;
      unsigned b8[8] = {0, 0, 0, 0, 0, 0, 0, 0};
      const uint4* p = reinterpret_cast<const uint4*>(lds + (long)shift + (long)(s_lo - g0));
#pragma unroll
      for (int q = 0; q < 4; ++q) {
        const uint4 v = p[q];
#pragma unroll
        for (int d = 0; d < 4; ++d) {
          const unsigned xd = d == 0 ? v.x : (d == 1 ? v.y : (d == 2 ? v.z : v.w));
          const unsigned c = ((xd >> 1) & 0x03030303u) ^ ((xd >> 2) & 0x01010101u);
          const unsigned df = __builtin_amdgcn_perm(0u, 0x54474341u, c) ^ xd;
          const unsigned nz = (((df & 0x7F7F7F7Fu) + 0x7F7F7F7Fu) | df) & 0x80808080u;
          const unsigned m1 = nz >> 7;
          const unsigned ck = c & ~(m1 | (m1 << 1));
          const unsigned g = __builtin_amdgcn_udot4(ck, 0x01041040u, 0u, false);
          const int idx = q * 4 + d;
          if (idx < 8) w0 |= (u64)g << (56 - 8 * idx); else w1 |= (u64)g << (56 - 8 * (idx - 8));
          b8[idx >> 1] = __builtin_amdgcn_udot4(nz, (idx & 1) ? 0x80402010u : 0x08040201u, b8[idx >> 1], false);
        }
      }
#pragma unroll
      for (int i = 0; i < 8; ++i) bd |= (u64)(b8[i] >> 7) << (8 * i);
      if (hi - lo == 64) {
        codes[2 * b] = w0;
        codes[2 * b + 1] = w1;
        bad[b] = bd;
      } else {
        const unsigned a = (unsigned)(lo - s_lo), e = (unsigned)(hi - s_lo);
        const u64 inmask = ((e - a) >= 64 ? ~0ull : ((1ull << (e - a)) - 1)) << a;
        const unsigned a0 = a < 32 ? a : 32, e0 = e < 32 ? e : 32, a1 = a > 32 ? a - 32 : 0, e1 = e > 32 ? e - 32 : 0;
        const u64 m0 = a0 < e0 ? ((~0ull >> (2 * a0)) & ~(e0 == 32 ? 0ull : (~0ull >> (2 * e0)))) : 0ull;
        const u64 m1 = a1 < e1 ? ((~0ull >> (2 * a1)) & ~(e1 == 32 ? 0ull : (~0ull >> (2 * e1)))) : 0ull;
        w0 &= m0;
        w1 &= m1;
        bd &= inmask;
        if (w0) atomicOr(&codes[2 * b], w0);
        if (w1) atomicOr(&codes[2 * b + 1], w1);
        if (bd) atomicOr(&bad[b], bd);
      }
      nbad += (int)__popcll(bd);
    }
  }
  for (int d = 32; d > 0; d >>= 1) nbad += __shfl_down(nbad, d);
  if (codes && lane == 0 && nbad > 0) atomicAdd(&info->bad_symbols, (u64)nbad);
  if (__ballot(flag_low != 0) && lane == 0) atomicOr(&info->parse_fallback, 1ull);
  if (__ballot(nhi != 0)) {
    for (int d = 32; d > 0; d >>= 1) nhi += __shfl_down(nhi, d);
    if (lane == 0) atomicAdd(&info->non_ascii, (u64)nhi);
  }
}

int mk_launch_fparse(mk_ctx* c, const uint8_t* d_raw, size_t begin, size_t len, bool fuse_pack_nt, bool write_seq) {
  if (!fuse_pack_nt) write_seq = true;
  const size_t n = begin + len;
  u64* codes = fuse_pack_nt ? (u64*)c->codes.p : nullptr;
  u64* bad = fuse_pack_nt ? (u64*)c->bad.p : nullptr;
  const size_t bad_words = n / 64 + 4;
  if (fuse_pack_nt && len == 0) {
    MK_HIP(hipMemsetAsync(c->codes.p, 0, 2 * bad_words * sizeof(u64), c->stream));
    MK_HIP(hipMemsetAsync(c->bad.p, 0, bad_words * sizeof(u64), c->stream));
    if (n == 0) MK_HIP(hipMemsetAsync(c->bad.p, 0xFF, 4 * sizeof(u64), c->stream));
  }
  if (len == 0) return MK_OK;
  const size_t nwaves = (n + FP_WAVE_BYTES - 1) / FP_WAVE_BYTES;
  const size_t e_bytes = (nwaves * sizeof(FpEntry) + 15) & ~(size_t)15;
  int rc = mk_buf_reserve(c, c->tile_maps, e_bytes + nwaves * sizeof(FpScan));
  if (rc) return rc;
  FpEntry* entries = (FpEntry*)c->tile_maps.p;
  FpScan* scan = (FpScan*)((char*)c->tile_maps.p + e_bytes);
  MkChunkInfo* info = (MkChunkInfo*)c->info.p;
  const unsigned blocks = (unsigned)((nwaves + FP_WAVES - 1) / FP_WAVES);
  mk_prof_begin(c, MK_K_PARSE);
  hipLaunchKernelGGL(mk_fparse_summ, dim3(blocks), dim3(FP_THREADS), 0, c->stream, d_raw, begin, n, nwaves, entries, info, codes, bad,
                     2 * bad_words, bad_words);
  hipLaunchKernelGGL(mk_fparse_scan, dim3(1), dim3(1024), 0, c->stream, (const FpEntry*)entries, nwaves, scan, info, bad);
  hipLaunchKernelGGL(mk_fparse_emit, dim3(blocks), dim3(FP_THREADS), 0, c->stream, d_raw, begin, n, nwaves, scan,
                     (uint8_t*)c->seq.p, info, codes, bad, write_seq ? 1 : 0);
  mk_prof_end(c);
  MK_HIP(hipGetLastError());
  return MK_OK;
}
```

### mercat2_amd/csrc/mk_skmer.hip

```cpp
#include "mk_skmer_dev.h"
#include <cstdlib>
#include <cstdio>
#include <vector>
#include <type_traits>

#define SK_NKMAX 8
#ifndef SK_HIST_THREADS
#define SK_HIST_THREADS 256
#endif
#ifndef SK_HIST_GRID
#define SK_HIST_GRID 512
#endif
#ifndef SK_SCAT_THREADS
#define SK_SCAT_THREADS 1024
#endif
#ifndef SK_SCAT_GRID
#define SK_SCAT_GRID 4096
#endif
#ifndef SK_SCAT_SUBT
#define SK_SCAT_SUBT 2
#endif
#ifndef SK_MAX_P1_LOG2
#define SK_MAX_P1_LOG2 14
#endif
#define SK_MAX_P1 (1 << SK_MAX_P1_LOG2)
#define SK_LH_LOG2 13
#define SK_LH (1 << SK_LH_LOG2)
#ifndef SK_BUCKET_SYMS
#define SK_BUCKET_SYMS 8192
#endif
#define SK_NOFIT 0xFF000000u
static size_t div_up(size_t a, size_t b) { return (a + b - 1) / b; }

template <int W, class F>
__device__ __forceinline__ void sk_for_each_record(u64 w0, u64 w1, u64 badw, int k, int nkmax, bool canon, F&& emit) {
  const SkRuns r = sk_analyse<W>(w0, w1, sk_valid32(badw, k), canon);
  sk_walk(r, w0, w1, nkmax, canon, emit);
}

__device__ __forceinline__ ulonglong2 sk_make_record(u64 w0, u64 w1, int jstart, int nk, int k) {
  const int s = 2 * jstart;
  u64 hi = (w0 << s) | ((w1 >> 1) >> (63 - s));
  u64 lo = w1 << s;
  const int t = 2 * (nk + k - 1);
  const u64 mh = t >= 64 ? ~0ull : (~0ull << ((64 - t) & 63));
  const u64 ml = t <= 64 ? 0ull : (~0ull << ((128 - t) & 63));
  hi &= mh;
  lo = (lo & ml) | (u64)nk;
  return make_ulonglong2(hi, lo);
}

template <int W, bool CANON>
__global__ __launch_bounds__(SK_HIST_THREADS) void mk_sk_hist_k(const u64* __restrict__ codes, const u64* __restrict__ bad,
                                                                const MkChunkInfo* __restrict__ info, u64* __restrict__ hist,
                                                                u64* __restrict__ khist, int p1_log2, int k, int nkmax,
                                                                size_t nthreads_total, int canon, int sample_log2) {
  extern __shared__ unsigned sk_hist_lds[];
  const unsigned p1 = 1u << p1_log2;
  unsigned* const lh = sk_hist_lds;
  unsigned* const lk = sk_hist_lds + p1;
  for (unsigned i = threadIdx.x; i < p1; i += blockDim.x) { lh[i] = 0; lk[i] = 0; }
  __syncthreads();
  const size_t seq_len = info->seq_len;
  const size_t ngroups = (nthreads_total + ((size_t)1 << sample_log2) - 1) >> sample_log2;
  for (size_t g = (size_t)blockIdx.x * blockDim.x + threadIdx.x; g < ngroups; g += (size_t)gridDim.x * blockDim.x) {
    size_t t = g;
    if (sample_log2) t = (g << sample_log2) + (((unsigned)g * 0x9E3779B1u >> 7) & ((1u << sample_log2) - 1));
    const size_t p0 = t * SK_R;
    if (t >= nthreads_total || p0 >= seq_len) continue;
    const u64 w0 = codes[t], w1 = codes[t + 1];
    const u64 badw = bad_window(bad, p0);
    (void)canon;
    sk_for_each_record<W>(w0, w1, badw, k, nkmax, CANON, [&](int, int nk, unsigned mm) {
      const unsigned b = sk_bucket(mm, p1_log2);
      atomicAdd(&lh[b], 1u);
      atomicAdd(&lk[b], (unsigned)nk);
    });
  }
  __syncthreads();
  for (unsigned b = threadIdx.x; b < p1; b += blockDim.x) {
    const unsigned v = lh[b];
    if (v) atomicAdd(&hist[b], (u64)v | ((u64)lk[b] << 32));
  }
}

#ifndef SK_TU_CANON
__device__ __forceinline__ u64 sk_cap(u64 h, int sample_log2, u64 weight, float sigmas) {
  if (sample_log2 == 0) return h;
  const u64 est = h << sample_log2;
  const float dev = sigmas * __builtin_sqrtf((float)((u64)weight << sample_log2) * (float)est);
  return est + (u64)dev + 1 + (sigmas > 0 ? 16 * weight : 0);
}
__device__ __forceinline__ u64 sk_seg_cap(u64 h, int sample_log2, u64 weight, float sigmas, int nseg) {
  const float est = (float)(h << sample_log2);
  const float var = (float)weight * est * (1.0f / (float)nseg + (float)(1u << sample_log2) / (float)(nseg * nseg));
  return (u64)(est / (float)nseg) + (u64)(sigmas * __builtin_sqrtf(var)) + 1 + (sigmas > 0 ? 4 * weight : 0);
}
__global__ __launch_bounds__(1024) void mk_sk_scan_k(const u64* __restrict__ hist, const u64* __restrict__ khist,
                                                     u64* __restrict__ start, SkCursor* __restrict__ cursor, u64* __restrict__ kstart,
                                                     MkChunkInfo* __restrict__ info, int p1_log2, int sample_log2, int nkmax,
                                                     u64 div, u64 part_cap, u64 surv_cap, float sigmas, int nseg) {
  constexpr int PER = SK_MAX_P1 / 1024;
  __shared__ u64 wsum[16], wksum[16];
  const unsigned p1 = 1u << p1_log2;
  const unsigned per = (p1 + 1023) / 1024;
  const unsigned lo = threadIdx.x * per;
  const int lane = threadIdx.x & 63, wv = threadIdx.x >> 6;
  u64 cap[PER], kcap[PER];
  u64 acc = 0, kacc = 0;
#pragma unroll
  for (int q = 0; q < PER; ++q) {
    const unsigned i = lo + q;
    const bool on = (unsigned)q < per && i < p1;
    const u64 hk = on ? hist[i] : 0ull;
    cap[q] = !on ? 0 : (nseg > 1 ? sk_seg_cap(hk & 0xFFFFFFFFull, sample_log2, SK_R / SK_NKMAX, sigmas, 8)
                                 : sk_cap(hk & 0xFFFFFFFFull, sample_log2, SK_R / SK_NKMAX, sigmas));
    kcap[q] = on ? (sk_cap(hk >> 32, sample_log2, SK_R, sigmas) + div - 1) / div : 0;
    acc += cap[q];
    kacc += kcap[q];
  }
  u64 inc = acc, kinc = kacc;
#pragma unroll
  for (int d = 1; d < 64; d <<= 1) {
    const u64 a = __shfl_up(inc, d), b = __shfl_up(kinc, d);
    if (lane >= d) { inc += a; kinc += b; }
  }
  if (lane == 63) { wsum[wv] = inc; wksum[wv] = kinc; }
  __syncthreads();
  u64 run = inc - acc, krun = kinc - kacc;
  for (int w = 0; w < wv; ++w) { run += wsum[w]; krun += wksum[w]; }
  __shared__ u64 s_total;
  if (threadIdx.x == 1023) {
    const u64 total = run + acc, ktotal = krun + kacc;
    s_total = total;
    const u64 all = nseg > 1 ? 16 * total : total;
    start[(size_t)nseg * p1] = all;
    kstart[p1] = ktotal;
    if (all > part_cap) atomicOr(&info->part_overflow, 1ull);
    if (ktotal > surv_cap) atomicOr(&info->part_overflow, 2ull);
  }
  __shared__ unsigned s_run[SK_MAX_P1];
#pragma unroll
  for (int q = 0; q < PER; ++q) {
    const unsigned i = lo + q;
    if ((unsigned)q < per && i < p1) {
      s_run[i] = (unsigned)run;
      kstart[i] = krun;
      run += cap[q];
      krun += kcap[q];
    }
  }
  __syncthreads();
  const u64 total = s_total;
  for (int x = 0; x < nseg; ++x)
    for (unsigned i = threadIdx.x; i < p1; i += 1024) {
      const u64 at = x < 8 ? (u64)x * total + s_run[i] : 8 * total + 8 * (u64)s_run[i];
      start[(size_t)x * p1 + i] = at;
      cursor[(size_t)x * p1 + i] = (SkCursor)at;
    }
}

#endif

template <int W, bool CANON>
__global__ __launch_bounds__(1024) void mk_sk_scatter_k(const u64* __restrict__ codes, const u64* __restrict__ bad,
                                                                   MkChunkInfo* __restrict__ info, const u64* __restrict__ start,
                                                                   SkCursor* __restrict__ cursor, ulonglong2* __restrict__ part,
                                                                   int p1_log2, int k, int nkmax, size_t ntiles, int canon) {
  __shared__ unsigned lh[SK_MAX_P1];
  constexpr int PK = SK_SCAT_SUBT > 1 ? SK_SCAT_SUBT - 1 : 1;
  __shared__ uint2 pk_mask[PK][SK_SCAT_THREADS];
  __shared__ ulonglong2 pk_w[PK][SK_SCAT_THREADS];
  __shared__ ulonglong2 pk_pos[PK][2][SK_SCAT_THREADS];
  __shared__ unsigned s_abort;
  if (threadIdx.x == 0) s_abort = info->part_overflow != 0;
  __syncthreads();
  if (s_abort) return;
  unsigned spilled = 0;
  constexpr int NB = SK_MAX_P1 / SK_SCAT_THREADS;
  const unsigned p1 = 1u << p1_log2;
  const size_t seq_len = info->seq_len;
  for (unsigned i = threadIdx.x; i < p1; i += blockDim.x) lh[i] = 0;
  __syncthreads();
  for (size_t tile = blockIdx.x; tile < ntiles; tile += gridDim.x) {
    SkRuns runs;
    u64 ww0 = 0, ww1 = 0;
#pragma unroll
    for (int st = 0; st < SK_SCAT_SUBT; ++st) {
      const size_t t = (tile * SK_SCAT_SUBT + st) * SK_SCAT_THREADS + threadIdx.x;
      const size_t p0 = t * SK_R;
      runs.valid = 0;
      runs.starts = 0;
      runs.pos[0] = runs.pos[1] = runs.pos[2] = runs.pos[3] = 0;
      ww0 = ww1 = 0;
      if (p0 < seq_len) {
        ww0 = codes[t];
        ww1 = codes[t + 1];
        runs = sk_analyse<W>(ww0, ww1, sk_valid32(bad_window(bad, p0), k), CANON);
        sk_walk(runs, ww0, ww1, nkmax, CANON,
                [&](int, int, unsigned mm) { atomicAdd(&lh[sk_bucket(mm, p1_log2)], 1u); });
      }
      if (st + 1 < SK_SCAT_SUBT) {
        pk_mask[st][threadIdx.x] = make_uint2(runs.valid, runs.starts);
        pk_w[st][threadIdx.x] = make_ulonglong2(ww0, ww1);
        pk_pos[st][0][threadIdx.x] = make_ulonglong2(runs.pos[0], runs.pos[1]);
        pk_pos[st][1][threadIdx.x] = make_ulonglong2(runs.pos[2], runs.pos[3]);
      }
    }
    __syncthreads();
    {
      unsigned v[NB];
      u64 r[NB];
#pragma unroll
      for (int i = 0; i < NB; ++i) {
        const unsigned b = threadIdx.x + i * SK_SCAT_THREADS;
        v[i] = b < p1 ? lh[b] : 0u;
      }
#pragma unroll
      for (int i = 0; i < NB; ++i) {
        const unsigned b = threadIdx.x + i * SK_SCAT_THREADS;
#ifdef SK_ABL_NOCURSOR
        r[i] = v[i] ? start[b] : 0ull;
#elif defined(SK_ABL_WGSCOPE)
        r[i] = v[i] ? __hip_atomic_fetch_add(&cursor[b], (u64)v[i], __ATOMIC_RELAXED, __HIP_MEMORY_SCOPE_WORKGROUP) : 0ull;
#else
        r[i] = v[i] ? atomicAdd(&cursor[b], (u64)v[i]) : 0ull;
#endif
      }
#pragma unroll
      for (int i = 0; i < NB; ++i) {
        const unsigned b = threadIdx.x + i * SK_SCAT_THREADS;
        if (b < p1) {
          const bool fits = v[i] == 0 || r[i] + v[i] <= start[b + 1];
          spilled |= fits ? 0u : 1u;
          lh[b] = fits ? (unsigned)r[i] : SK_NOFIT;
        }
      }
    }
    __syncthreads();
#pragma unroll
    for (int st = SK_SCAT_SUBT - 1; st >= 0; --st) {
      if (st + 1 < SK_SCAT_SUBT) {
        const uint2 m = pk_mask[st][threadIdx.x];
        const ulonglong2 w = pk_w[st][threadIdx.x], pa = pk_pos[st][0][threadIdx.x], pb = pk_pos[st][1][threadIdx.x];
        runs.valid = m.x;
        runs.starts = m.y;
        runs.pos[0] = pa.x; runs.pos[1] = pa.y; runs.pos[2] = pb.x; runs.pos[3] = pb.y;
        ww0 = w.x;
        ww1 = w.y;
      }
      const u64 w0 = ww0, w1 = ww1;
      (void)canon;
      sk_walk(runs, w0, w1, nkmax, CANON, [&](int jstart, int nk, unsigned mm) {
        const unsigned b = sk_bucket(mm, p1_log2);
        const unsigned at = atomicAdd(&lh[b], 1u);
        ulonglong2 rec = sk_make_record(w0, w1, jstart, nk, k);
        asm volatile("" : "+v"(rec.x), "+v"(rec.y));
#ifdef SK_ABL_NOSTORE
        if (at == 0xFFFFFFFFu) part[(size_t)at] = rec;
#else
        if (at < SK_NOFIT) part[(size_t)at] = rec;
#endif
      });
    }
    __syncthreads();
    for (unsigned i = threadIdx.x; i < p1; i += blockDim.x) lh[i] = 0;
    __syncthreads();
  }
  if (spilled) atomicOr(&info->part_overflow, 4ull);
}

#ifdef MK_STAMP
static __device__ u64 skq_dbg[1024 * 8];
#endif
#define SKQ_CAP 512
#if defined(SK_ABL_COARSE) && !defined(SK_PLAIN_CURSORS)
#error "SK_ABL_COARSE needs -DSK_PLAIN_CURSORS (the ablation's region ends differ from the ones sk_reserve8k checks)"
#endif
#ifndef SKQ_THREADS
#define SKQ_THREADS 512
#endif
#define SKQ_WAVES (SKQ_THREADS / 64)
#define SKQ_WALKED 0xFFFFFFFFu
template <int W, bool CANON, int SKQ_SUBT, int SKQ_QCAP>
__global__ __launch_bounds__(SKQ_THREADS) __attribute__((amdgpu_waves_per_eu(4, 4))) void mk_sk_scatterq_k(const u64* __restrict__ codes, const u64* __restrict__ bad,
                                                         MkChunkInfo* __restrict__ info, const u64* __restrict__ start,
                                                         SkCursor* __restrict__ cursor, ulonglong2* __restrict__ part,
                                                         int p1_log2, int k, int nkmax, size_t ntiles, unsigned qcap, int nseg) {
  SkCursor* const shared_cursor = cursor + ((size_t)8 << p1_log2);
  const u64* const shared_start = start + ((size_t)8 << p1_log2);
  if (nseg > 1) {
    unsigned xcc;
    asm volatile("s_getreg_b32 %0, hwreg(HW_REG_XCC_ID)" : "=s"(xcc));
    const size_t seg = xcc & 7u;
    cursor += seg << p1_log2;
    start += seg << p1_log2;
  }
  __shared__ unsigned lh[SK_LH];
  __shared__ u64 pk_x[SKQ_SUBT][SKQ_WAVES][65];
  __shared__ unsigned queue[SKQ_SUBT][SKQ_WAVES][SKQ_QCAP];
  __shared__ unsigned s_abort;
  if (threadIdx.x == 0) s_abort = info->part_overflow != 0;
  __syncthreads();
  if (s_abort) return;
  unsigned spilled = 0;
  constexpr int NB = SK_LH / SKQ_THREADS;
  const unsigned p1 = 1u << p1_log2;
  const unsigned lhn = p1 < (unsigned)SK_LH ? p1 : (unsigned)SK_LH;
  const unsigned nround = p1 / lhn;
  const size_t seq_len = info->seq_len;
  const int lane = threadIdx.x & 63;
#define wv sk_wave_id()
  auto sk_wave_id = [&]() { int w = (int)threadIdx.x; asm volatile("" : "+v"(w)); return w >> 6; };
  for (unsigned i = threadIdx.x; i < lhn; i += blockDim.x) lh[i] = 0;
  __syncthreads();
  u64 tA = 0, tB = 0, tC = 0, tD = 0, tE = 0, tF = 0, t0 = 0, ntile = 0;
  (void)tA; (void)tB; (void)tC; (void)tD; (void)tE; (void)tF; (void)t0; (void)ntile;
  STAMP(t0);
  for (size_t tile = blockIdx.x; tile < ntiles; tile += gridDim.x) {
    ntile += 1;
    unsigned qn[SKQ_SUBT];
#pragma unroll
    for (int st = 0; st < SKQ_SUBT; ++st) {
      const size_t t = (tile * SKQ_SUBT + st) * SKQ_THREADS + threadIdx.x;
      const size_t p0 = t * SK_R;
      SkRuns runs;
      runs.valid = 0;
      runs.starts = 0;
      runs.pos[0] = runs.pos[1] = runs.pos[2] = runs.pos[3] = 0;
      u64 ww0 = 0, ww1 = 0;
      if (p0 < seq_len) {
        ww0 = codes[t];
        ww1 = codes[t + 1];
        runs = sk_analyse<W>(ww0, ww1, sk_valid32(bad_window(bad, p0), k), CANON);
      } else if (p0 < seq_len + SK_R) {
        ww0 = codes[t];
      }
      pk_x[st][wv][lane] = ww0;
      if (lane == 63) pk_x[st][wv][64] = ww1;
      const unsigned s2 = sk_cut_starts(runs.starts, runs.valid, nkmax);
      const unsigned cnt = __popc(s2);
      const unsigned inc = mk_wave_scan_incl(cnt);
      const unsigned total = mk_wave_last(inc);
      unsigned* const myq = queue[st][wv];
      if (total <= qcap) {
        unsigned todo = s2, at = inc - cnt;
        while (todo) {
          const int j = __ffs(todo) - 1;
          todo &= todo - 1;
          const unsigned stop = (s2 | ~runs.valid) & ~((2u << j) - 1);
          const int nk = (stop ? (__ffs(stop) - 1) : SK_R) - j;
          const u64 pw = j < 10 ? runs.pos[0] : (j < 20 ? runs.pos[1] : (j < 30 ? runs.pos[2] : runs.pos[3]));
          const unsigned best = (unsigned)(pw >> (6 * (j % 10))) & 63u;
          myq[at++] = (unsigned)lane | ((unsigned)j << 6) | ((unsigned)nk << 11) | (best << 16);
        }
        __builtin_amdgcn_fence(__ATOMIC_RELEASE, "wavefront");
        __builtin_amdgcn_wave_barrier();
        __builtin_amdgcn_fence(__ATOMIC_ACQUIRE, "wavefront");
        for (unsigned base = 0; base < total; base += 64) {
          const unsigned i = base + lane;
          if (i < total) {
            const unsigned it = myq[i];
            const u64* const wp = &pk_x[st][wv][it & 63u];
            const unsigned mm = sk_canon_mmer(sk_mmer(wp[0], wp[1], (int)(it >> 16)), CANON);
#ifdef SK_ABL_COARSE
            const unsigned b = sk_bucket(mm, p1_log2) & ~63u;
#else
            const unsigned b = sk_bucket(mm, p1_log2);
#endif
            if ((b >> SK_LH_LOG2) == 0) atomicAdd(&lh[b & (SK_LH - 1)], 1u);
            myq[i] = (it & 0xFFFFu) | (b << 16);
          }
        }
        qn[st] = total;
      } else {
        if (p0 < seq_len)
          sk_walk(runs, ww0, ww1, nkmax, CANON, [&](int, int, unsigned mm) {
            const unsigned b = sk_bucket(mm, p1_log2);
            if ((b >> SK_LH_LOG2) == 0) atomicAdd(&lh[b & (SK_LH - 1)], 1u);
          });
        qn[st] = SKQ_WALKED;
      }
    }
#pragma unroll 1
    for (unsigned round = 0; round < nround; ++round) {
    SkCursor* const rcursor = cursor + (size_t)round * SK_LH;
    const u64* const rstart = start + (size_t)round * SK_LH;
    if (round) {
#pragma unroll
      for (int st = 0; st < SKQ_SUBT; ++st) {
        if (qn[st] != SKQ_WALKED) {
          const unsigned total = qn[st];
          const unsigned* const myq = queue[st][wv];
          for (unsigned base = 0; base < total; base += 64) {
            const unsigned i = base + lane;
            if (i < total) {
              const unsigned b = myq[i] >> 16;
              if ((b >> SK_LH_LOG2) == round) atomicAdd(&lh[b & (SK_LH - 1)], 1u);
            }
          }
        } else {
          const size_t t = (tile * SKQ_SUBT + st) * SKQ_THREADS + threadIdx.x;
          const size_t p0 = t * SK_R;
          if (p0 < seq_len) {
            const ulonglong2 w = make_ulonglong2(pk_x[st][wv][lane], pk_x[st][wv][lane + 1]);
            const SkRuns runs = sk_analyse<W>(w.x, w.y, sk_valid32(bad_window(bad, p0), k), CANON);
            sk_walk(runs, w.x, w.y, nkmax, CANON, [&](int, int, unsigned mm) {
              const unsigned b = sk_bucket(mm, p1_log2);
              if ((b >> SK_LH_LOG2) == round) atomicAdd(&lh[b & (SK_LH - 1)], 1u);
            });
          }
        }
      }
    }
    STAMP_ADD(tA, t0);
    __syncthreads();
    STAMP_ADD(tB, t0);
#ifndef SK_PLAIN_CURSORS
    if (lhn == SK_LH) {
      static_assert(NB % 8 == 0, "sk_reserve8");
#pragma unroll
      for (int h = 0; h < NB; h += 8) {
        unsigned v[8], at[8];
#pragma unroll
        for (int i = 0; i < 8; ++i) v[i] = lh[threadIdx.x + (h + i) * SKQ_THREADS];
        unsigned nofit = sk_reserve8<SKQ_THREADS>(v, rcursor + h * SKQ_THREADS, rstart + h * SKQ_THREADS, SK_NOFIT, at);
        if (nseg > 1 && __any(nofit)) {
          unsigned v2[8], at2[8];
#pragma unroll
          for (int i = 0; i < 8; ++i) {
            v2[i] = at[i] >= SK_NOFIT ? v[i] : 0u;
            const unsigned pad = at[i] >= SK_NOFIT ? at[i] & 0xFFFFFFu : 0u;
            if (pad) {
              const u64 end = rstart[threadIdx.x + (h + i) * SKQ_THREADS + 1];
              for (unsigned q = 0; q < pad; ++q) part[end - pad + q] = make_ulonglong2(0, 0);
            }
          }
          nofit = sk_reserve8<SKQ_THREADS>(v2, shared_cursor + (size_t)round * SK_LH + h * SKQ_THREADS,
                                           shared_start + (size_t)round * SK_LH + h * SKQ_THREADS, SK_NOFIT, at2);
#pragma unroll
          for (int i = 0; i < 8; ++i) at[i] = v2[i] ? at2[i] : at[i];
        }
        spilled |= nofit;
#pragma unroll
        for (int i = 0; i < 8; ++i) lh[threadIdx.x + (h + i) * SKQ_THREADS] = at[i];
      }
    } else
#endif
    {
      for (unsigned b = threadIdx.x; b < lhn; b += SKQ_THREADS) {
        const unsigned v = lh[b];
        u64 r = v ? (u64)atomicAdd(&rcursor[b], v) : 0ull;
#ifdef SK_ABL_COARSE
        const bool fits = v == 0 || r + v <= rstart[b + 64 < p1 ? b + 64 : p1];
#else
        bool fits = v == 0 || r + v <= rstart[b + 1];
        if (!fits && nseg > 1) {
          for (u64 q = r; q < rstart[b + 1]; ++q) part[q] = make_ulonglong2(0, 0);
          r = (u64)atomicAdd(&shared_cursor[b], v);
          fits = r + v <= shared_start[b + 1];
        }
#endif
        spilled |= fits ? 0u : 1u;
        lh[b] = fits ? (unsigned)r : SK_NOFIT;
      }
    }
    STAMP_ADD(tC, t0);
    __syncthreads();
    STAMP_ADD(tD, t0);
#pragma unroll
    for (int st = 0; st < SKQ_SUBT; ++st) {
      if (qn[st] != SKQ_WALKED) {
        const unsigned total = qn[st];
        const unsigned* const myq = queue[st][wv];
        for (unsigned base = 0; base < total; base += 64) {
          const unsigned i = base + lane;
          if (i < total && ((myq[i] >> 16) >> SK_LH_LOG2) == round) {
            const unsigned it = myq[i];
            const unsigned at = atomicAdd(&lh[(it >> 16) & (SK_LH - 1)], 1u);
            const u64* const wp = &pk_x[st][wv][it & 63u];
            ulonglong2 rec = sk_make_record(wp[0], wp[1], (int)((it >> 6) & 31u), (int)((it >> 11) & 31u), k);
            asm volatile("" : "+v"(rec.x), "+v"(rec.y));
#ifdef SK_NT_STORE
            typedef unsigned long long u64x2_t __attribute__((ext_vector_type(2)));
            if (at < SK_NOFIT) __builtin_nontemporal_store(u64x2_t{rec.x, rec.y}, (u64x2_t*)&part[(size_t)at]);
#else
            if (at < SK_NOFIT) part[(size_t)at] = rec;
#endif
          }
        }
      } else {
        const size_t t = (tile * SKQ_SUBT + st) * SKQ_THREADS + threadIdx.x;
        const size_t p0 = t * SK_R;
        if (p0 < seq_len) {
          const ulonglong2 w = make_ulonglong2(pk_x[st][wv][lane], pk_x[st][wv][lane + 1]);
          const SkRuns runs = sk_analyse<W>(w.x, w.y, sk_valid32(bad_window(bad, p0), k), CANON);
          sk_walk(runs, w.x, w.y, nkmax, CANON, [&](int jstart, int nk, unsigned mm) {
            const unsigned b = sk_bucket(mm, p1_log2);
            if ((b >> SK_LH_LOG2) != round) return;
            const unsigned at = atomicAdd(&lh[b & (SK_LH - 1)], 1u);
            if (at < SK_NOFIT) part[(size_t)at] = sk_make_record(w.x, w.y, jstart, nk, k);
          });
        }
      }
    }
    STAMP_ADD(tE, t0);
    __syncthreads();
    for (unsigned i = threadIdx.x; i < lhn; i += blockDim.x) lh[i] = 0;
    __syncthreads();
    STAMP_ADD(tF, t0);
    }
  }
#ifdef MK_STAMP
  if (threadIdx.x == 0 && blockIdx.x < 1024) { u64* d = skq_dbg + (size_t)blockIdx.x * 8; d[0] = tA; d[1] = tB; d[2] = tC; d[3] = tD; d[4] = tE; d[5] = tF; d[6] = ntile; }
#endif
  if (spilled) atomicOr(&info->part_overflow, 4ull);
}
#undef wv

#ifdef SK_EXP_SORT
__global__ __launch_bounds__(256) void mk_sk_expsort_k(ulonglong2* __restrict__ part, const u64* __restrict__ start,
                                                       const SkCursor* __restrict__ cursor, unsigned p1, int classes) {
  __shared__ ulonglong2 buf[6144];
  __shared__ unsigned cnt[64], base[64];
  for (unsigned b = blockIdx.x; b < p1; b += gridDim.x) {
    const u64 lo = start[b], n = cursor[b] - start[b];
    if (n == 0 || n > 6144) continue;
    if (threadIdx.x < 64) cnt[threadIdx.x] = 0;
    __syncthreads();
    for (u64 i = threadIdx.x; i < n; i += blockDim.x) {
      const ulonglong2 r = part[lo + i];
      buf[i] = r;
      const int nk = (int)(r.y & 63);
      const int cls = classes == 2 ? (nk >= 5 ? 0 : 1) : (32 - nk);
      atomicAdd(&cnt[cls], 1u);
    }
    __syncthreads();
    if (threadIdx.x == 0) { unsigned a = 0; for (int q = 0; q < 64; ++q) { base[q] = a; a += cnt[q]; } }
    __syncthreads();
    for (u64 i = threadIdx.x; i < n; i += blockDim.x) {
      const ulonglong2 r = buf[i];
      const int nk = (int)(r.y & 63);
      const int cls = classes == 2 ? (nk >= 5 ? 0 : 1) : (32 - nk);
      part[lo + atomicAdd(&base[cls], 1u)] = r;
    }
    __syncthreads();
  }
}
#endif


#ifndef SK_TU_CANON
void mk_launch_sk_scan(mk_ctx* c, const u64* hist, const u64* khist, u64* start, SkCursor* cursor, u64* kstart, int p1_log2,
                       int sample_log2, int nkmax, u64 surv_div, u64 part_cap, u64 surv_cap, float sigmas, int nseg) {
  hipLaunchKernelGGL(mk_sk_scan_k, dim3(1), dim3(1024), 0, c->stream, hist, khist, start, cursor, kstart,
                     (MkChunkInfo*)c->info.p, p1_log2, sample_log2, nkmax, surv_div, part_cap, surv_cap, sigmas, nseg);
}

#endif

template <int W, bool CANON>
static void launch_wc(mk_ctx* c, size_t seq_len, int p1_log2, int nkmax, int sample_log2, u64 surv_div, u64 part_cap, u64 surv_cap,
                     u64* hist, u64* start, SkCursor* cursor, u64* khist, u64* kstart, bool reuse, int nseg) {
  MkChunkInfo* info = (MkChunkInfo*)c->info.p;
  float sigmas = 6.0f;
  if (const char* e = getenv("MK_SAMPLE_SIGMAS")) sigmas = (float)atof(e);
  const size_t threads = div_up(seq_len, SK_R);
  const size_t tiles = div_up(div_up(threads, (size_t)1 << sample_log2), SK_HIST_THREADS);
  const size_t stiles = div_up(threads, (size_t)SK_SCAT_THREADS * SK_SCAT_SUBT);
  const size_t hist_grid = sample_log2 ? SK_HIST_GRID / 2 : SK_HIST_GRID;
  if (!reuse) {
    hipLaunchKernelGGL((mk_sk_hist_k<W, CANON>), dim3((unsigned)(tiles < hist_grid ? tiles : hist_grid)), dim3(SK_HIST_THREADS),
                       2 * sizeof(unsigned) << p1_log2, c->stream,
                       (const u64*)c->codes.p, (const u64*)c->bad.p, info, hist, khist, p1_log2, c->k, nkmax, threads, c->canonical,
                       sample_log2);
    mk_launch_sk_scan(c, (const u64*)hist, (const u64*)khist, start, cursor, kstart, p1_log2, sample_log2, nkmax, surv_div, part_cap,
                      surv_cap, sigmas, nseg);
  }
  static const bool walked = getenv("MK_SCATTER_WALK") != nullptr;
  const int force_subt = getenv("MK_SKQ_SUBT") ? atoi(getenv("MK_SKQ_SUBT")) : 0;
  const bool three = force_subt == 3 || (force_subt != 2 && c->items_hint > 0 && c->items_hint * 64.0 + 48.0 < 376.0);
  unsigned qcap = three ? 376u : 512u;
  if (const char* e = getenv("MK_SKQ_CAP")) { const int v = atoi(e); if (v >= 0 && (unsigned)v < qcap) qcap = (unsigned)v; }
  if (walked)
    hipLaunchKernelGGL((mk_sk_scatter_k<W, CANON>), dim3((unsigned)(stiles < SK_SCAT_GRID ? stiles : SK_SCAT_GRID)), dim3(SK_SCAT_THREADS), 0,
                       c->stream, (const u64*)c->codes.p, (const u64*)c->bad.p, info, (const u64*)start, cursor,
                       (ulonglong2*)c->part.p, p1_log2, c->k, nkmax, stiles, c->canonical);
  else {
    const size_t qtiles = div_up(threads, (size_t)SKQ_THREADS * (three ? 3 : 2));
    const dim3 qgrid((unsigned)(qtiles < SK_SCAT_GRID ? qtiles : SK_SCAT_GRID));
    if (three)
      hipLaunchKernelGGL((mk_sk_scatterq_k<W, CANON, 3, 376>), qgrid, dim3(SKQ_THREADS), 0, c->stream, (const u64*)c->codes.p,
                         (const u64*)c->bad.p, info, (const u64*)start, cursor, (ulonglong2*)c->part.p, p1_log2, c->k, nkmax, qtiles, qcap, nseg);
    else
      hipLaunchKernelGGL((mk_sk_scatterq_k<W, CANON, 2, 512>), qgrid, dim3(SKQ_THREADS), 0, c->stream, (const u64*)c->codes.p,
                         (const u64*)c->bad.p, info, (const u64*)start, cursor, (ulonglong2*)c->part.p, p1_log2, c->k, nkmax, qtiles, qcap, nseg);
  }
#ifdef MK_STAMP
  if (!walked) {
    (void)hipStreamSynchronize(c->stream);
    const size_t qtiles = div_up(threads, (size_t)SKQ_THREADS * (three ? 3 : 2));
    const unsigned g = (unsigned)(qtiles < SK_SCAT_GRID ? qtiles : SK_SCAT_GRID);
    std::vector<u64> h(8 * 1024);
    (void)hipMemcpyFromSymbol(h.data(), HIP_SYMBOL(skq_dbg), h.size() * 8);
    double a[7] = {0, 0, 0, 0, 0, 0, 0};
    for (unsigned w = 0; w < g && w < 1024; ++w) for (int q = 0; q < 7; ++q) a[q] += (double)h[w * 8 + q] / g;
    fprintf(stderr, "[stamp scatterq] per WG (wave 0): analyse+list+pass1=%.0f barrier1=%.0f cursors=%.0f barrier2=%.0f pass2=%.0f barrier3+clear=%.0f tiles=%.2f grid=%u\n",
            a[0], a[1], a[2], a[3], a[4], a[5], a[6], g);
  }
#endif
}


template <bool CANON>
static bool sk_partition(int W, mk_ctx* c, size_t seq_len, int p1_log2, int nkmax, int sample_log2, u64 surv_div, u64 part_cap, u64 surv_cap,
                         u64* hist, u64* start, SkCursor* cursor, u64* khist, u64* kstart, bool reuse, int nseg) {
  switch (W) {
#define SK_CASE(W_)                                                                                                      \
  case W_: launch_wc<W_, CANON>(c, seq_len, p1_log2, nkmax, sample_log2, surv_div, part_cap, surv_cap, hist, start, cursor, khist, kstart, reuse, nseg); return true;
    SK_CASE(2) SK_CASE(3) SK_CASE(4) SK_CASE(5) SK_CASE(6) SK_CASE(7)
    SK_CASE(8) SK_CASE(9) SK_CASE(10) SK_CASE(11) SK_CASE(12) SK_CASE(13) SK_CASE(14) SK_CASE(15) SK_CASE(16)
    SK_CASE(17) SK_CASE(18) SK_CASE(19) SK_CASE(20) SK_CASE(21) SK_CASE(22)
#undef SK_CASE
    default: return false;
  }
}

#ifdef SK_TU_CANON
bool mk_sk_partition_canon(int W, mk_ctx* c, size_t seq_len, int p1_log2, int nkmax, int sample_log2, u64 surv_div, u64 part_cap,
                           u64 surv_cap, u64* hist, u64* start, SkCursor* cursor, u64* khist, u64* kstart, bool reuse, int nseg) {
  return sk_partition<true>(W, c, seq_len, p1_log2, nkmax, sample_log2, surv_div, part_cap, surv_cap, hist, start, cursor, khist, kstart, reuse, nseg);
}
#else
bool mk_sk_partition_canon(int W, mk_ctx* c, size_t seq_len, int p1_log2, int nkmax, int sample_log2, u64 surv_div, u64 part_cap,
                           u64 surv_cap, u64* hist, u64* start, SkCursor* cursor, u64* khist, u64* kstart, bool reuse, int nseg);

bool mk_part_inherit(mk_ctx* c, size_t seq_len, int p1_log2, uint64_t min_count, bool sampled, bool exact) {
  if (c->part_cooldown > 0 && !exact) c->part_cooldown -= 1;
  const bool reuse = c->use_reuse && !exact && sampled && c->part_reuse_ok && !c->part_dirty && c->part_cooldown == 0 &&
                     p1_log2 == c->part_prev_p1 && (unsigned long long)min_count == c->part_prev_minc &&
                     seq_len <= c->part_prev_len + c->part_prev_len / 100 && seq_len >= c->part_prev_len - c->part_prev_len / 50;
  if (reuse) c->st.part_reused += 1;
  c->part_dirty = true;
  if (exact) { c->part_reuse_ok = false; c->part_cooldown = 4; }
  else if (sampled && !reuse) {
    c->part_reuse_ok = true;
    c->part_prev_len = seq_len;
    c->part_prev_p1 = p1_log2;
    c->part_prev_minc = (unsigned long long)min_count;
  } else if (!reuse) c->part_reuse_ok = false;
  return reuse;
}

int mk_launch_count_superkmer(mk_ctx* c, size_t seq_len, uint64_t min_count, bool exact) {
  if (seq_len == 0) return MK_OK;
  MkChunkInfo* info = (MkChunkInfo*)c->info.p;
  const int k = c->k;
  static const bool cores = getenv("MK_CORES") != nullptr;
  const int max_log2 = cores ? SK_MAX_P1_LOG2 : SK_LH_LOG2;
  const size_t bucket_syms = cores ? SK_BUCKET_SYMS / 2 : SK_BUCKET_SYMS;
  int p1_log2 = 8;
  while (p1_log2 < max_log2 && (seq_len >> p1_log2) > bucket_syms) ++p1_log2;
  if (const char* e = getenv("MK_P1_LOG2")) { int v = atoi(e); if (v >= 4 && v <= SK_MAX_P1_LOG2) p1_log2 = v; }
  c->p1_log2 = p1_log2;
  const size_t p1 = (size_t)1 << p1_log2;
  int nkmax = 62 - k;
  if (nkmax > SK_NKMAX) nkmax = SK_NKMAX;
  if (const char* e = getenv("MK_NKMAX")) { int v = atoi(e); if (v >= 1 && v <= 31 && v <= 62 - k) nkmax = v; }
  int sample_log2 = 0;
  {
    int want = 3;
    size_t min_len = (size_t)8 << 20;
    if (const char* e = getenv("MK_SAMPLE_LOG2")) { int v = atoi(e); if (v >= 0 && v <= 6) want = v; }
    if (const char* e = getenv("MK_SAMPLE_MIN")) min_len = (size_t)atoll(e);
    if (!exact && seq_len >= min_len) sample_log2 = want;
  }
  c->part_sampled = sample_log2 != 0;
  const bool xseg_on = !(getenv("MK_XSEG") && atoi(getenv("MK_XSEG")) == 0);
  static const bool walked_env = getenv("MK_SCATTER_WALK") != nullptr;
  static const bool force_pre = getenv("MK_FORCE_PREFILTER") != nullptr;
  const int nseg = (xseg_on && sample_log2 != 0 && !walked_env && !force_pre && p1_log2 <= SK_LH_LOG2 &&
                    seq_len <= ((size_t)1 << 30)) ? 9 : 1;
  if (nseg != c->part_nseg) c->part_reuse_ok = false;
  c->part_nseg = nseg;
  const bool reuse = mk_part_inherit(c, seq_len, p1_log2, min_count, sample_log2 != 0, exact);
  int rc;
  if ((rc = mk_buf_reserve(c, c->part_meta, (7 * p1 + 16 + 14 * p1 + 8) * sizeof(u64))) != MK_OK) return rc;
  const size_t part_cap = nseg > 1 ? 2 * seq_len + 64 : seq_len + 64;
  if ((rc = mk_buf_reserve(c, c->part, part_cap * sizeof(ulonglong2))) != MK_OK) return rc;
  const u64 surv_div = min_count > 1 ? (u64)min_count : 1;
  size_t surv_cap = seq_len / surv_div + p1 + 64;
  if (sample_log2) {
    const double L = 1.25 * (double)seq_len, S = (double)(1u << sample_log2), w = (double)SK_R;
    surv_cap = (size_t)((L + 6.0 * sqrt((double)p1 * S * w * L) + 16.0 * w * (double)p1) / (double)surv_div) + 2 * p1 + 64;
  }
  if ((rc = mk_buf_reserve(c, c->surv_keys, surv_cap * sizeof(u64))) != MK_OK) return rc;
  if ((rc = mk_buf_reserve(c, c->surv_cnts, surv_cap * sizeof(u64))) != MK_OK) return rc;
  u64* hist = (u64*)c->part_meta.p;
  u64* start = hist + p1;
  SkCursor* cursor = (SkCursor*)(start + p1 + 1);
  u64* khist = start + p1 + 1 + p1;
  u64* kstart = khist + p1;
  u64* nsurv = kstart + p1 + 1 + p1;
  if (nseg > 1) {
    start = hist + 7 * p1 + 16;
    cursor = (SkCursor*)(start + 9 * p1 + 8);
  }
  if (!reuse) MK_HIP(hipMemsetAsync(hist, 0, (7 * p1 + 8) * sizeof(u64), c->stream));
  mk_prof_begin(c, MK_K_PART);
  if (c->canonical) {
    if (!mk_sk_partition_canon(k - SK_M + 1, c, seq_len, p1_log2, nkmax, sample_log2, surv_div, (u64)part_cap, (u64)surv_cap, hist, start, cursor, khist, kstart, reuse, nseg)) {
      c->err = "mk_launch_count_superkmer: k out of range";
      return MK_ERR_ARG;
    }
  } else if (!sk_partition<false>(k - SK_M + 1, c, seq_len, p1_log2, nkmax, sample_log2, surv_div, (u64)part_cap, (u64)surv_cap, hist, start, cursor, khist, kstart, reuse, nseg)) {
    c->err = "mk_launch_count_superkmer: k out of range";
    return MK_ERR_ARG;
  }
  mk_prof_end(c);
#ifdef SK_EXP_SORT
  if (const char* e = getenv("MK_EXP_SORT"))
    hipLaunchKernelGGL(mk_sk_expsort_k, dim3(2048), dim3(256), 0, c->stream, (ulonglong2*)c->part.p, (const u64*)start, (const SkCursor*)cursor,
                       (unsigned)p1, atoi(e));
#endif
  {
    const int rc_count = cores ? mk_launch_sk_count_small(c, (const u64*)start, cursor, (const u64*)kstart, nsurv, min_count, nkmax, p1, exact, nseg)
                               : mk_launch_sk_count(c, (const u64*)start, cursor, (const u64*)kstart, nsurv, min_count, nkmax, p1, exact, nseg);
    if (rc_count) return rc_count;
  }
  MK_HIP(hipGetLastError());
  c->surv_regions = 1;
  return MK_OK;
}
#endif
```

### mercat2_amd/native.py

```python
from __future__ import annotations

import ctypes as C
import os
from pathlib import Path
from typing import Optional, Sequence, Tuple

import numpy as np

ALPHABET_NT2, ALPHABET_AA5, ALPHABET_RAW = 0, 1, 2
MODE_NAMES = {0: "dense", 1: "hash64", 2: "hash128", 3: "byref"}

MK_OK = 0
ERR_NAMES = {-1: "MK_ERR_ARG", -2: "MK_ERR_HIP", -3: "MK_ERR_NOMEM", -4: "MK_ERR_STATE",
             -5: "MK_ERR_NON_ASCII", -6: "MK_ERR_IO", -7: "MK_ERR_RANGE", -8: "MK_ERR_UNSUPPORTED"}

ABI_SYMBOLS = [
    "mk_create", "mk_destroy", "mk_last_error", "mk_reset", "mk_set_canonical", "mk_chunk_begin", "mk_chunk_feed",
    "mk_chunk_feed_device", "mk_chunk_end", "mk_count_device", "mk_export_size", "mk_export",
    "mk_write_tsv", "mk_export_pairs_device", "mk_import_pairs_device", "mk_export_exotic",
    "mk_import_exotic", "mk_words_per_key", "mk_merge_from", "mk_set_profiling", "mk_get_stats", "mk_reset_stats",
    "mk_chunk_cuts", "mk_synth_reads", "mk_version", "mk_count_file", "mk_stream_cuts",
    "mk_merged_export", "mk_write_merged_tsv", "mk_trim", "mk_alpha_stats", "mk_gunzip", "mk_crc32_of", "mk_gunzip_parallel",
    "mk_filter_min", "mk_remove_n", "mk_free", "mk_write_merged_tsv_t", "mk_write_merged_tsv_as_reference",
    "mk_owner_bounds", "mk_plan_contexts", "mk_bucket_rows_device", "mk_import_rows_device", "mk_merge_devices",
    "mk_export_size_multi", "mk_export_multi", "mk_write_tsv_multi", "mk_record_cuts", "mk_sample_keys", "mk_dense_bins_device",
    "mk_device_count", "mk_reset_for", "mk_textwrap", "mk_set_clean", "mk_clean_stats", "mk_clean_runs",
    "mk_export_stats", "mk_share_table",
]
MK_ABI = 4
MERGE_RANGES, MERGE_GATHER, MERGE_BALANCED, MERGE_RCCL = 0, 1, 2, 4


class MercatHipError(RuntimeError):
    def __init__(self, code: int, message: str):
        super().__init__("%s (%d): %s" % (ERR_NAMES.get(code, "MK_ERR"), code, message))
        self.code = code


class NonAsciiInput(MercatHipError, UnicodeDecodeError.__base__):
    pass


class CleanUnsupported(MercatHipError):
    """Clean mode (Counter.set_clean): the text holds something whose rewrite by removeN the GPU does not reproduce;
    nothing was counted -- count the text mk_remove_n produces instead."""


class Stats(C.Structure):
    _fields_ = [(n, C.c_uint64) for n in ("raw_bytes", "symbols", "windows", "exotic_windows", "chunks",
                                           "survivors", "rows", "table_slots")] + \
               [("mode", C.c_int32), ("profiled", C.c_int32)] + \
               [(n, C.c_double) for n in ("ms_parse", "ms_pack", "ms_count", "ms_exotic", "ms_filter", "ms_export")] + \
               [(n, C.c_uint64) for n in ("n_parse", "n_pack", "n_count", "n_exotic", "n_filter", "n_export")] + \
               [("ms_part", C.c_double), ("n_part", C.c_uint64), ("records", C.c_uint64), ("distinct", C.c_uint64),
                ("part_retries", C.c_uint64), ("part_reused", C.c_uint64), ("fused_chunks", C.c_uint64), ("fuse_spilled", C.c_uint64), ("parse_retries", C.c_uint64)]

    def as_dict(self):
        return {n: getattr(self, n) for n, _ in self._fields_}


class FileStats(C.Structure):
    _fields_ = ([(n, C.c_uint64) for n in ("disk_bytes", "text_bytes", "chunks")] +
                [(n, C.c_int32) for n in ("gz", "chunked", "members", "threads", "contexts", "devices", "split_pieces", "pad_")] +
                [(n, C.c_double) for n in ("s_wait_io", "s_wait_gpu", "s_total", "s_merge",
                                           "s_setup", "s_scan", "s_feed", "s_retire", "s_drain")])

    def as_dict(self):
        return {n: getattr(self, n) for n, _ in self._fields_ if n != "pad_"}


class ExportStats(C.Structure):
    _fields_ = ([(n, C.c_uint64) for n in ("rows", "bytes")] +
                [(n, C.c_double) for n in ("s_sort", "s_d2h", "s_format", "s_write", "s_total")])

    def as_dict(self):
        return {n: getattr(self, n) for n, _ in self._fields_}


class CleanGpu(C.Structure):
    _fields_ = [(n, C.c_uint64) for n in ("raw_bytes", "symbols", "gc_count", "n_bytes", "n_runs", "header_lines", "last_runs")]


class MergeStats(C.Structure):
    _fields_ = ([(n, C.c_uint64) for n in ("rows_in", "rows_out", "rows_moved", "bytes_moved", "max_owned")] +
                [(n, C.c_int32) for n in ("contexts", "devices", "peer_direct", "rccl")] +
                [(n, C.c_double) for n in ("s_bucket", "s_copy", "s_import", "s_total")])

    def as_dict(self):
        return {n: getattr(self, n) for n, _ in self._fields_ if n != "pad_"}


class CleanStats(C.Structure):
    _fields_ = [(n, C.c_uint64) for n in ("gc_count", "total_length", "records", "split_records", "pieces", "n_runs")] + \
               [("unsupported_record", C.c_int64)]


class AlphaStats(C.Structure):
    _fields_ = [("observed", C.c_uint64), ("total", C.c_uint64), ("freq", C.c_uint64 * 11),
                ("sum_sq", C.c_double), ("sum_clnc", C.c_double)]


_LIB: Optional[C.CDLL] = None


def library_path() -> Path:
    return Path(os.environ.get("MERCAT_HIP_LIB", Path(__file__).resolve().parent / "libmercat_hip.so"))


def lib() -> C.CDLL:
    global _LIB
    if _LIB is not None:
        return _LIB
    path = library_path()
    if not path.exists():
        raise MercatHipError(-2, "HIP extension %s is missing: build it with `python -c 'import __graft_entry__ as g; "
                                 "g.build()'` or `make -C mercat2_amd/csrc` (there is no CPU fallback)" % path)
    L = C.CDLL(str(path))
    vp, u8p, u64p, szp = C.c_void_p, C.c_void_p, C.c_void_p, C.POINTER(C.c_size_t)
    sig = {
        "mk_create": (C.c_int, [C.c_int, C.c_int, C.c_int, C.POINTER(vp)]),
        "mk_destroy": (None, [vp]),
        "mk_last_error": (C.c_char_p, [vp]),
        "mk_reset": (C.c_int, [vp]),
        "mk_reset_for": (C.c_int, [vp, C.c_uint64]),
        "mk_set_canonical": (C.c_int, [vp, C.c_int]),
        "mk_set_clean": (C.c_int, [vp, C.c_int, C.c_int]),
        "mk_clean_stats": (C.c_int, [vp, C.POINTER(CleanGpu)]),
        "mk_clean_runs": (C.c_int, [vp, u64p, u64p, C.c_size_t, szp]),
        "mk_chunk_begin": (C.c_int, [vp]),
        "mk_chunk_feed": (C.c_int, [vp, u8p, C.c_size_t]),
        "mk_chunk_feed_device": (C.c_int, [vp, u8p, C.c_size_t]),
        "mk_chunk_end": (C.c_int, [vp, C.c_uint64]),
        "mk_count_device": (C.c_int, [vp, u8p, C.c_size_t, C.c_uint64]),
        "mk_export_size": (C.c_int, [vp, szp]),
        "mk_export": (C.c_int, [vp, u8p, u64p, C.c_size_t]),
        "mk_write_tsv": (C.c_int, [vp, C.c_char_p, C.c_char_p, szp]),
        "mk_export_stats": (C.c_int, [vp, C.POINTER(ExportStats)]),
        "mk_export_pairs_device": (C.c_int, [vp, u64p, u64p, C.c_size_t, szp]),
        "mk_import_pairs_device": (C.c_int, [vp, u64p, u64p, C.c_size_t]),
        "mk_export_exotic": (C.c_int, [vp, u8p, u64p, C.c_size_t, szp]),
        "mk_import_exotic": (C.c_int, [vp, u8p, u64p, C.c_size_t]),
        "mk_words_per_key": (C.c_int, [vp]),
        "mk_merge_from": (C.c_int, [vp, vp]),
        "mk_share_table": (C.c_int, [vp, vp]),
        "mk_set_profiling": (C.c_int, [vp, C.c_int]),
        "mk_get_stats": (C.c_int, [vp, C.POINTER(Stats)]),
        "mk_reset_stats": (C.c_int, [vp]),
        "mk_chunk_cuts": (C.c_int, [u8p, C.c_size_t, C.c_uint64, u64p, C.c_size_t, szp]),
        "mk_synth_reads": (C.c_int, [C.c_uint64, C.c_uint64, C.c_uint64, C.c_uint32, C.c_uint64, C.c_uint32,
                                     C.c_uint64, u8p, C.c_size_t, szp]),
        "mk_version": (C.c_char_p, []),
        "mk_count_file": (C.c_int, [C.POINTER(vp), C.c_int, C.c_char_p, C.c_uint64, C.c_uint64, C.c_int,
                                    C.POINTER(FileStats)]),
        "mk_merged_export": (C.c_int, [C.POINTER(vp), C.c_int, u8p, u64p, C.c_size_t, szp]),
        "mk_write_merged_tsv": (C.c_int, [C.POINTER(vp), C.c_int, C.POINTER(C.c_char_p), C.c_char_p, C.c_char_p, szp]),
        "mk_write_merged_tsv_as_reference": (C.c_int, [C.POINTER(vp), C.c_int, C.POINTER(C.c_char_p), C.c_char_p, C.c_char_p, szp]),
        "mk_write_merged_tsv_t": (C.c_int, [C.POINTER(vp), C.c_int, C.POINTER(C.c_char_p), C.c_char_p, szp]),
        "mk_trim": (C.c_int, [vp]),
        "mk_filter_min": (C.c_int, [vp, C.c_uint64]),
        "mk_remove_n": (C.c_int, [u8p, C.c_size_t, C.c_int, C.POINTER(C.c_void_p), szp, C.POINTER(CleanStats)]),
        "mk_free": (None, [C.c_void_p]),
        "mk_textwrap": (C.c_int, [u8p, C.c_size_t, C.c_size_t, C.POINTER(C.c_void_p), szp]),
        "mk_alpha_stats": (C.c_int, [vp, C.POINTER(AlphaStats)]),
        "mk_gunzip_parallel": (C.c_int, [u8p, C.c_size_t, u8p, C.c_size_t, C.c_int, C.c_size_t, szp, C.POINTER(C.c_int)]),
        "mk_crc32_of": (C.c_uint32, [u8p, C.c_size_t, C.c_uint32]),
        "mk_gunzip": (C.c_int, [u8p, C.c_size_t, u8p, C.c_size_t, C.c_size_t, szp, C.POINTER(C.c_int)]),
        "mk_stream_cuts": (C.c_int, [u8p, C.c_size_t, C.c_uint64, C.c_size_t, u64p, C.c_size_t, szp]),
        "mk_record_cuts": (C.c_int, [u8p, C.c_size_t, C.c_uint64, C.c_size_t, u64p, C.c_size_t, szp]),
        "mk_owner_bounds": (C.c_int, [C.c_int, C.c_int, u64p]),
        "mk_plan_contexts": (C.c_int, [C.POINTER(C.c_int), C.c_int, C.c_int, C.POINTER(C.c_int)]),
        "mk_bucket_rows_device": (C.c_int, [vp, u64p, C.c_int, u64p, C.c_size_t, u64p]),
        "mk_import_rows_device": (C.c_int, [vp, u64p, C.c_size_t]),
        "mk_merge_devices": (C.c_int, [C.POINTER(vp), C.c_int, C.c_int, C.POINTER(MergeStats)]),
        "mk_device_count": (C.c_int, []),
        "mk_sample_keys": (C.c_int, [vp, C.c_size_t, u64p, C.c_size_t, szp]),
        "mk_dense_bins_device": (C.c_int, [vp, u64p, C.c_size_t, C.c_int]),
        "mk_export_size_multi": (C.c_int, [C.POINTER(vp), C.c_int, szp]),
        "mk_export_multi": (C.c_int, [C.POINTER(vp), C.c_int, u8p, u64p, C.c_size_t]),
        "mk_write_tsv_multi": (C.c_int, [C.POINTER(vp), C.c_int, C.c_char_p, C.c_char_p, szp]),
    }
    L.mk_version.restype = C.c_char_p
    ver = (L.mk_version() or b"").decode()
    try:
        abi = int(ver.split()[1].split(".")[0])
    except (IndexError, ValueError):
        abi = -1
    if abi != MK_ABI:
        raise MercatHipError(-4, "%s announces '%s' but this binding is written for ABI %d: rebuild the library "
                                 "(make -C mercat2_amd/csrc) -- struct layouts would not match" % (path, ver, MK_ABI))
    for name, (res, args) in sig.items():
        fn = getattr(L, name)
        fn.restype, fn.argtypes = res, args
    _LIB = L
    return L


def _buf_ptr(data) -> Tuple[int, int, object]:
    if isinstance(data, np.ndarray):
        a = np.ascontiguousarray(data).view(np.uint8).reshape(-1)
        return a.ctypes.data, a.nbytes, a
    mv = memoryview(data)
    if mv.nbytes == 0:
        return 0, 0, None
    a = np.frombuffer(mv, dtype=np.uint8)
    return a.__array_interface__["data"][0], a.nbytes, a


def _big_u8(n: int) -> np.ndarray:
    import mmap
    if n == 0:
        return np.empty(0, dtype=np.uint8)
    return np.frombuffer(mmap.mmap(-1, n), dtype=np.uint8)


def chunk_cuts(text, chunksize: int) -> np.ndarray:
    L = lib()
    addr, n, keep = _buf_ptr(text)
    need = C.c_size_t(0)
    cap = 64
    while True:
        cuts = np.empty(cap, dtype=np.uint64)
        rc = L.mk_chunk_cuts(addr, n, int(chunksize), cuts.ctypes.data, cap, C.byref(need))
        if rc == MK_OK:
            return cuts[: need.value].copy()
        if rc != -7:
            raise MercatHipError(rc, "mk_chunk_cuts")
        cap = need.value


def remove_n(text, toupper: bool = False) -> Tuple[bytes, dict]:
    L = lib()
    addr, n, keep = _buf_ptr(text)
    out, out_len, st = C.c_void_p(), C.c_size_t(0), CleanStats()
    rc = L.mk_remove_n(addr, n, 1 if toupper else 0, C.byref(out), C.byref(out_len), C.byref(st))
    if rc == -7:
        raise IndexError("list index out of range")
    if rc == -5:
        raise NonAsciiInput(rc, "record %d holds sequence byte(s) >= 0x80 (non-ASCII sequence text is not supported)" % st.unsupported_record)
    if rc:
        raise MercatHipError(rc, "mk_remove_n")
    try:
        data = C.string_at(out, out_len.value) if out.value else b""
    finally:
        if out.value:
            L.mk_free(out)
    return data, {n_: int(getattr(st, n_)) for n_, _ in st._fields_}


def textwrap_lines(text, width: int = 80) -> list:
    L = lib()
    addr, n, keep = _buf_ptr(text)
    out, out_len = C.c_void_p(), C.c_size_t(0)
    rc = L.mk_textwrap(addr, n, int(width), C.byref(out), C.byref(out_len))
    if rc:
        raise MercatHipError(rc, "mk_textwrap")
    try:
        data = C.string_at(out, out_len.value) if out.value else b""
    finally:
        if out.value:
            L.mk_free(out)
    return data.split(b"\n")[:-1] if data else []


def default_streams(k: int, alphabet: int) -> int:
    one_word = (alphabet == ALPHABET_NT2 and k <= 32) or (alphabet == ALPHABET_AA5 and k <= 12)
    return 2 if one_word else 1


def gunzip(gz, cap: int, block: int = 4 << 20) -> Tuple[bytes, int]:
    L = lib()
    addr, n, keep = _buf_ptr(gz)
    out = np.empty(max(cap, 1), dtype=np.uint8)
    written, members = C.c_size_t(0), C.c_int(0)
    rc = L.mk_gunzip(addr, n, out.ctypes.data, cap, int(block), C.byref(written), C.byref(members))
    if rc:
        raise MercatHipError(rc, "mk_gunzip")
    return out[: written.value].tobytes(), members.value


def gunzip_parallel(gz, cap: int, threads: int = 4, piece: int = 1 << 20) -> Tuple[bytes, int]:
    L = lib()
    addr, n, keep = _buf_ptr(gz)
    out = np.empty(max(cap, 1), dtype=np.uint8)
    written, members = C.c_size_t(0), C.c_int(0)
    rc = L.mk_gunzip_parallel(addr, n, out.ctypes.data, cap, int(threads), int(piece), C.byref(written), C.byref(members))
    if rc:
        raise MercatHipError(rc, "mk_gunzip_parallel")
    return out[: written.value].tobytes(), members.value


def stream_cuts(text, chunksize: int, block: int) -> np.ndarray:
    L = lib()
    addr, n, keep = _buf_ptr(text)
    need = C.c_size_t(0)
    cap = 64
    while True:
        cuts = np.empty(cap, dtype=np.uint64)
        rc = L.mk_stream_cuts(addr, n, int(chunksize), int(block), cuts.ctypes.data, cap, C.byref(need))
        if rc == MK_OK:
            return cuts[: need.value].copy()
        if rc != -7:
            raise MercatHipError(rc, "mk_stream_cuts")
        cap = need.value


def record_cuts(text, piece: int, block: int = 1 << 20) -> np.ndarray:
    L = lib()
    addr, n, keep = _buf_ptr(text)
    need = C.c_size_t(0)
    cap = 64
    while True:
        cuts = np.empty(cap, dtype=np.uint64)
        rc = L.mk_record_cuts(addr, n, int(piece), int(block), cuts.ctypes.data, cap, C.byref(need))
        if rc == MK_OK:
            return cuts[: need.value].copy()
        if rc != -7:
            raise MercatHipError(rc, "mk_record_cuts")
        cap = need.value


def device_count() -> int:
    return int(lib().mk_device_count())


def owner_bounds(key_bits: int, n: int) -> list:
    out = np.zeros(max(1, n - 1), dtype=np.uint64)
    rc = lib().mk_owner_bounds(int(key_bits), int(n), out.ctypes.data)
    if rc:
        raise MercatHipError(rc, "mk_owner_bounds")
    return [int(x) for x in out[: n - 1]]


def plan_contexts(devices: Sequence[int], streams: int) -> list:
    nd = len(devices)
    arr = (C.c_int * nd)(*[int(d) for d in devices])
    out = (C.c_int * (nd * int(streams)))()
    rc = lib().mk_plan_contexts(arr, nd, int(streams), out)
    if rc:
        raise MercatHipError(rc, "mk_plan_contexts")
    return list(out)


def _ctx_array(ctxs: Sequence["Counter"]):
    return (C.c_void_p * len(ctxs))(*[c._h for c in ctxs])


def merge_devices(ctxs: Sequence["Counter"], flags: int = MERGE_RANGES) -> dict:
    st = MergeStats()
    rc = lib().mk_merge_devices(_ctx_array(ctxs), len(ctxs), int(flags), C.byref(st))
    if rc:
        ctxs[0]._check(rc)
    return st.as_dict()


def rows_multi(ctxs: Sequence["Counter"]) -> int:
    n = C.c_size_t(0)
    rc = lib().mk_export_size_multi(_ctx_array(ctxs), len(ctxs), C.byref(n))
    if rc:
# ... 261 lines not shown
```

Measured before the change: 159.8 billion.

## Fuse FASTA/FASTQ parsing into the super-k-mer scatter kernel on partition reuse

When the partition plan is reused from an earlier chunk, the separate fparse pass that writes packed codes and bad-symbol bitmaps is skipped. The scatter kernel instead reads the raw text directly, classifies it and packs it per span in-kernel. This removes one kernel launch and a full write-then-read of the packed code and bitmap arrays. If the in-kernel parse or the partition overflows, the chunk is handed back and redone through the old two-pass path, which adds retry cost and makes the scatter kernel more complex.

```diff
diff --git a/include/mercat_hip.h b/include/mercat_hip.h
--- a/include/mercat_hip.h
+++ b/include/mercat_hip.h
@@ -46,6 +46,7 @@
   uint64_t fused_chunks;
   uint64_t fuse_spilled;
   uint64_t parse_retries;
+  uint64_t raw_scattered;
 } mk_stats_t;
 
 int mk_create(int device, int alphabet, int k, mk_ctx** out);
diff --git a/mercat2_amd/csrc/mk_api.hip b/mercat2_amd/csrc/mk_api.hip
--- a/mercat2_amd/csrc/mk_api.hip
+++ b/mercat2_amd/csrc/mk_api.hip
@@ -180,6 +180,7 @@
     return fail(MK_ERR_HIP, std::string("hipStreamCreate: ") + hipGetErrorString(e));
   c->use_speculation = getenv("MK_NO_SPECULATION") ? 0 : 1;
   c->use_reuse = getenv("MK_NO_REUSE") ? 0 : 1;
+  c->use_fused_parse = getenv("MK_NO_FUSED_PARSE") ? 0 : 1;
   c->use_fused = getenv("MK_NO_FUSE") ? 0 : 1;
   c->dup_hint = 2.0;
   c->nk_hint = 5.0;
@@ -249,6 +250,7 @@
   c->in_chunk = false;
   c->raw_len = 0;
   c->part_reuse_ok = false;
+  c->fused_parse_off = false;
   c->dup_known = false;
   c->fuse_cap = 0;
   c->clean_n_runs = c->clean_n_bytes = c->clean_gc = c->clean_symbols = c->clean_raw = c->clean_headers = c->clean_last_runs = 0;
@@ -474,7 +476,7 @@
 
 #define MK_RETRY_GENERAL 1
 
-static int process_chunk_fast(mk_ctx* c, const uint8_t* d_raw, size_t n, u64 min_count) {
+static int process_chunk_fast(mk_ctx* c, const uint8_t* d_raw, size_t n, u64 min_count, bool raw = true) {
   int rc;
   const size_t begin = (size_t)((uintptr_t)d_raw & 15);
   const uint8_t* d_al = d_raw - begin;
@@ -485,8 +487,16 @@
   if ((rc = mk_buf_reserve(c, c->bad, (bad_words + 2) * 8)) != MK_OK) return rc;
   if ((rc = mk_buf_reserve(c, c->codes, (2 * bad_words + 8) * 8)) != MK_OK) return rc;
   static const bool always_seq = getenv("MK_ALWAYS_SEQ") != nullptr;
-  if ((rc = mk_launch_fparse(c, d_al, begin, n, true, always_seq)) != MK_OK) return rc;
   const bool two = c->mode == MK_MODE_HASH128;
+  c->raw_scattered = false;
+  c->parse_deferred = raw && !two && !always_seq && c->use_fused_parse && !c->fused_parse_off;
+  if (c->parse_deferred) {
+    c->raw_src = d_al;
+    c->raw_src_begin = begin;
+    c->raw_src_n = n;
+  } else if ((rc = mk_launch_fparse(c, d_al, begin, n, true, always_seq)) != MK_OK) {
+    return rc;
+  }
   c->rtab_chunk_slots = 0;
   c->surv_regions = 0;
   c->ctab_slots = 0;
@@ -522,11 +532,21 @@
     rc = two ? mk_launch_count_superkmer2(c, n, min_count) : mk_launch_count_superkmer(c, n, min_count);
   }
   c->fuse_cap = 0;
+  c->parse_deferred = false;
   if (rc) return rc;
   const bool fused = !two && c->fused_last;
   if ((rc = pull_info(c)) != MK_OK) return rc;
   MkChunkInfo* h = c->h_info;
-  if (h->parse_fallback) { c->st.parse_retries += 1; return MK_RETRY_GENERAL; }
+  if (h->parse_fallback & 1) { c->st.parse_retries += 1; return MK_RETRY_GENERAL; }
+  const bool raw_done = c->raw_scattered;
+  if (raw_done && (h->parse_fallback || h->part_overflow)) {
+    if (getenv("MK_VERBOSE"))
+      fprintf(stderr, "[mk] raw-text scatter handed the chunk back (parse_fallback=%llu part_overflow=%llu seq_len=%llu)\n",
+              h->parse_fallback, h->part_overflow, h->seq_len);
+    if (h->parse_fallback) c->fused_parse_off = true;
+    if (h->part_overflow) { c->part_reuse_ok = false; c->part_cooldown = 4; c->st.part_retries += 1; }
+    return process_chunk_fast(c, d_raw, n, min_count, false);
+  }
   if (h->non_ascii) {
     c->err = "input holds " + std::to_string(h->non_ascii) +
              " sequence byte(s) >= 0x80 (non-ASCII sequence text is not supported; the chunk was not counted)";
@@ -537,7 +557,7 @@
     if (!always_seq) {
       if ((rc = mk_buf_reserve(c, c->ex_tmp, sizeof(MkChunkInfo) + 64)) != MK_OK) return rc;
       MK_HIP(hipMemcpyAsync(c->ex_tmp.p, c->info.p, sizeof(MkChunkInfo), hipMemcpyDeviceToDevice, c->stream));
-      if ((rc = mk_launch_fparse(c, d_al, begin, n, false, true)) != MK_OK) return rc;
+      if ((rc = mk_launch_fparse(c, d_al, begin, n, raw_done, true)) != MK_OK) return rc;
       MK_HIP(hipMemcpyAsync(c->info.p, c->ex_tmp.p, sizeof(MkChunkInfo), hipMemcpyDeviceToDevice, c->stream));
     }
     const u64 bound = std::min<u64>((u64)seq_len, h->bad_symbols * (u64)c->k);
@@ -620,6 +640,7 @@
   c->st.chunks += 1;
   c->st.records += h->records;
   c->st.distinct += h->distinct;
+  c->st.raw_scattered += raw_done ? 1 : 0;
   c->st.survivors += h->survivors + h->survivors_ref + ((h->side && h->side >= min_count) ? 1 : 0);
   return MK_OK;
 }
diff --git a/mercat2_amd/csrc/mk_common.h b/mercat2_amd/csrc/mk_common.h
--- a/mercat2_amd/csrc/mk_common.h
+++ b/mercat2_amd/csrc/mk_common.h
@@ -139,6 +139,12 @@
   unsigned long long part_prev_minc = 0;
   int part_cooldown = 0;
   int use_reuse = 1;
+  int use_fused_parse = 1;
+  bool fused_parse_off = false;
+  bool parse_deferred = false;
+  bool raw_scattered = false;
+  const uint8_t* raw_src = nullptr;
+  size_t raw_src_begin = 0, raw_src_n = 0;
   int surv_regions = 0;
   double nk_hint = 8.0;
   double items_hint = 0;
diff --git a/mercat2_amd/csrc/mk_fparse.hip b/mercat2_amd/csrc/mk_fparse.hip
--- a/mercat2_amd/csrc/mk_fparse.hip
+++ b/mercat2_amd/csrc/mk_fparse.hip
@@ -1,7 +1,4 @@
-#include "mk_common.h"
-#include "mk_device.h"
-
-typedef unsigned long long u64;
+#include "mk_fparse_dev.h"
 
 #define FP_THREADS 256
 #ifndef FP_SUB
@@ -14,78 +11,6 @@
   unsigned a;
   unsigned b;
 };
-
-__device__ __forceinline__ uint4 classify16(const uint8_t* __restrict__ raw, size_t pos, size_t begin, size_t n, unsigned& nl,
-                                            unsigned& gt, unsigned& st, unsigned& low, unsigned& hi) {
-  uint4 v;
-  if (pos + 16 <= n && pos >= begin) {
-    v = *reinterpret_cast<const uint4*>(raw + pos);
-  } else {
-    unsigned w0 = 0, w1 = 0, w2 = 0, w3 = 0;
-#pragma unroll
-    for (int j = 0; j < 16; ++j) {
-      const unsigned c = (pos + j < n && pos + j >= begin) ? (unsigned)raw[pos + j] : 10u;
-      const unsigned sh = 8 * (j & 3);
-      if (j < 4) w0 |= c << sh; else if (j < 8) w1 |= c << sh; else if (j < 12) w2 |= c << sh; else w3 |= c << sh;
-    }
-    v = make_uint4(w0, w1, w2, w3);
-  }
-#define FP_NZ7(t) ((((t) & 0x7F7F7F7Fu) + 0x7F7F7F7Fu) | (t))
-  unsigned a_nl[2] = {0, 0}, a_gt[2] = {0, 0}, a_st[2] = {0, 0}, a_lo[2] = {0, 0}, a_hi[2] = {0, 0};
-#pragma unroll
-  for (int d = 0; d < 4; ++d) {
-    const unsigned xd = d == 0 ? v.x : (d == 1 ? v.y : (d == 2 ? v.z : v.w));
-    const unsigned K = (d & 1) ? 0x80402010u : 0x08040201u;
-    const unsigned notnl = FP_NZ7(xd ^ 0x0A0A0A0Au) & FP_NZ7(xd ^ 0x0D0D0D0Du);
-    const unsigned ge21 = ((xd & 0x7F7F7F7Fu) + 0x5F5F5F5Fu) | xd;
-    a_nl[d >> 1] = __builtin_amdgcn_udot4(~notnl & 0x80808080u, K, a_nl[d >> 1], false);
-    a_gt[d >> 1] = __builtin_amdgcn_udot4(~FP_NZ7(xd ^ 0x3E3E3E3Eu) & 0x80808080u, K, a_gt[d >> 1], false);
-    a_st[d >> 1] = __builtin_amdgcn_udot4(~FP_NZ7(xd ^ 0x2A2A2A2Au) & 0x80808080u, K, a_st[d >> 1], false);
-    a_lo[d >> 1] = __builtin_amdgcn_udot4(~ge21 & notnl & 0x80808080u, K, a_lo[d >> 1], false);
-    a_hi[d >> 1] = __builtin_amdgcn_udot4(xd & 0x80808080u, K, a_hi[d >> 1], false);
-  }
-#undef FP_NZ7
-  nl = (a_nl[0] >> 7) | ((a_nl[1] >> 7) << 8);
-  gt = (a_gt[0] >> 7) | ((a_gt[1] >> 7) << 8);
-  st = (a_st[0] >> 7) | ((a_st[1] >> 7) << 8);
-  low = (a_lo[0] >> 7) | ((a_lo[1] >> 7) << 8);
-  hi = (a_hi[0] >> 7) | ((a_hi[1] >> 7) << 8);
-  return v;
-}
-
-__device__ __forceinline__ unsigned lane_header(unsigned start, unsigned nl, unsigned hin, unsigned& hout) {
-  const unsigned p = ~nl & 0xFFFFu;
-  const unsigned a = start | p, b = start;
-  const unsigned sum = a + b + hin;
-  const unsigned ci = sum ^ a ^ b;
-  hout = (ci >> 16) & 1u;
-  return (ci >> 1) & 0xFFFFu;
-}
-
-__device__ __forceinline__ unsigned wave_step(unsigned nl, unsigned gt, unsigned st, unsigned low, unsigned prev_nl,
-                                              unsigned cin, unsigned& out, unsigned& sep, unsigned& bad_low,
-                                              unsigned& last_nl) {
-  const int lane = threadIdx.x & 63;
-  const unsigned my_last_nl = (nl >> 15) & 1u;
-  const unsigned prev = (unsigned)__builtin_amdgcn_update_dpp((int)prev_nl, (int)my_last_nl, 0x138, 0xf, 0xf, false);
-  const unsigned ls = ((nl << 1) | prev) & 0xFFFFu;
-  const unsigned start = ls & gt;
-  unsigned hout0;
-  (void)lane_header(start, nl, 0u, hout0);
-  const u64 G = __ballot(hout0 != 0);
-  const u64 P = __ballot(nl == 0);
-  const u64 A = G | P, B = G;
-  const u64 sum = A + B + (u64)cin;
-  const u64 CI = sum ^ A ^ B;
-  const unsigned hin = (unsigned)(CI >> lane) & 1u;
-  unsigned hout;
-  const unsigned H = lane_header(start, nl, hin, hout);
-  sep = start;
-  out = ((~H & ~nl & ~st) | start) & 0xFFFFu;
-  bad_low = low & ~H;
-  last_nl = mk_wave_last(my_last_nl);
-  return mk_wave_last(hout);
-}
 
 __global__ __launch_bounds__(FP_THREADS) void mk_fparse_summ(const uint8_t* __restrict__ raw, size_t begin, size_t n, size_t nwaves,
                                                              FpEntry* __restrict__ entries, MkChunkInfo* __restrict__ info,
@@ -319,12 +244,8 @@
 #pragma unroll
         for (int d = 0; d < 4; ++d) {
           const unsigned xd = d == 0 ? v.x : (d == 1 ? v.y : (d == 2 ? v.z : v.w));
-          const unsigned c = ((xd >> 1) & 0x03030303u) ^ ((xd >> 2) & 0x01010101u);
-          const unsigned df = __builtin_amdgcn_perm(0u, 0x54474341u, c) ^ xd;
-          const unsigned nz = (((df & 0x7F7F7F7Fu) + 0x7F7F7F7Fu) | df) & 0x80808080u;
-          const unsigned m1 = nz >> 7;
-          const unsigned ck = c & ~(m1 | (m1 << 1));
-          const unsigned g = __builtin_amdgcn_udot4(ck, 0x01041040u, 0u, false);
+          unsigned g, nz;
+          fp_code4(xd, g, nz);
           const int idx = q * 4 + d;
           if (idx < 8) w0 |= (u64)g << (56 - 8 * idx); else w1 |= (u64)g << (56 - 8 * (idx - 8));
           b8[idx >> 1] = __builtin_amdgcn_udot4(nz, (idx & 1) ? 0x80402010u : 0x08040201u, b8[idx >> 1], false);
diff --git a/mercat2_amd/csrc/mk_fparse_dev.h b/mercat2_amd/csrc/mk_fparse_dev.h
--- /dev/null
+++ b/mercat2_amd/csrc/mk_fparse_dev.h
@@ -0,0 +1,238 @@
+#pragma once
+#include "mk_common.h"
+#include "mk_device.h"
+
+typedef unsigned long long u64;
+
+__device__ __forceinline__ uint4 classify16(const uint8_t* __restrict__ raw, size_t pos, size_t begin, size_t n, unsigned& nl,
+                                            unsigned& gt, unsigned& st, unsigned& low, unsigned& hi) {
+  uint4 v;
+  if (pos + 16 <= n && pos >= begin) {
+    v = *reinterpret_cast<const uint4*>(raw + pos);
+  } else {
+    unsigned w0 = 0, w1 = 0, w2 = 0, w3 = 0;
+#pragma unroll 1
+    for (int j = 0; j < 16; ++j) {
+      const unsigned c = (pos + j < n && pos + j >= begin) ? (unsigned)raw[pos + j] : 10u;
+      w0 = (w0 >> 8) | (w1 << 24);
+      w1 = (w1 >> 8) | (w2 << 24);
+      w2 = (w2 >> 8) | (w3 << 24);
+      w3 = (w3 >> 8) | (c << 24);
+    }
+    v = make_uint4(w0, w1, w2, w3);
+  }
+#define FP_NZ7(t) ((((t) & 0x7F7F7F7Fu) + 0x7F7F7F7Fu) | (t))
+  unsigned a_nl[2] = {0, 0}, a_gt[2] = {0, 0}, a_st[2] = {0, 0}, a_lo[2] = {0, 0}, a_hi[2] = {0, 0};
+#pragma unroll
+  for (int d = 0; d < 4; ++d) {
+    const unsigned xd = d == 0 ? v.x : (d == 1 ? v.y : (d == 2 ? v.z : v.w));
+    const unsigned K = (d & 1) ? 0x80402010u : 0x08040201u;
+    const unsigned notnl = FP_NZ7(xd ^ 0x0A0A0A0Au) & FP_NZ7(xd ^ 0x0D0D0D0Du);
+    const unsigned ge21 = ((xd & 0x7F7F7F7Fu) + 0x5F5F5F5Fu) | xd;
+    a_nl[d >> 1] = __builtin_amdgcn_udot4(~notnl & 0x80808080u, K, a_nl[d >> 1], false);
+    a_gt[d >> 1] = __builtin_amdgcn_udot4(~FP_NZ7(xd ^ 0x3E3E3E3Eu) & 0x80808080u, K, a_gt[d >> 1], false);
+    a_st[d >> 1] = __builtin_amdgcn_udot4(~FP_NZ7(xd ^ 0x2A2A2A2Au) & 0x80808080u, K, a_st[d >> 1], false);
+    a_lo[d >> 1] = __builtin_amdgcn_udot4(~ge21 & notnl & 0x80808080u, K, a_lo[d >> 1], false);
+    a_hi[d >> 1] = __builtin_amdgcn_udot4(xd & 0x80808080u, K, a_hi[d >> 1], false);
+  }
+#undef FP_NZ7
+  nl = (a_nl[0] >> 7) | ((a_nl[1] >> 7) << 8);
+  gt = (a_gt[0] >> 7) | ((a_gt[1] >> 7) << 8);
+  st = (a_st[0] >> 7) | ((a_st[1] >> 7) << 8);
+  low = (a_lo[0] >> 7) | ((a_lo[1] >> 7) << 8);
+  hi = (a_hi[0] >> 7) | ((a_hi[1] >> 7) << 8);
+  return v;
+}
+
+__device__ __forceinline__ unsigned lane_header(unsigned start, unsigned nl, unsigned hin, unsigned& hout) {
+  const unsigned p = ~nl & 0xFFFFu;
+  const unsigned a = start | p, b = start;
+  const unsigned sum = a + b + hin;
+  const unsigned ci = sum ^ a ^ b;
+  hout = (ci >> 16) & 1u;
+  return (ci >> 1) & 0xFFFFu;
+}
+
+__device__ __forceinline__ unsigned wave_step(unsigned nl, unsigned gt, unsigned st, unsigned low, unsigned prev_nl,
+                                              unsigned cin, unsigned& out, unsigned& sep, unsigned& bad_low,
+                                              unsigned& last_nl) {
+  const int lane = threadIdx.x & 63;
+  const unsigned my_last_nl = (nl >> 15) & 1u;
+  const unsigned prev = (unsigned)__builtin_amdgcn_update_dpp((int)prev_nl, (int)my_last_nl, 0x138, 0xf, 0xf, false);
+  const unsigned ls = ((nl << 1) | prev) & 0xFFFFu;
+  const unsigned start = ls & gt;
+  unsigned hout0;
+  (void)lane_header(start, nl, 0u, hout0);
+  const u64 G = __ballot(hout0 != 0);
+  const u64 P = __ballot(nl == 0);
+  const u64 A = G | P, B = G;
+  const u64 sum = A + B + (u64)cin;
+  const u64 CI = sum ^ A ^ B;
+  const unsigned hin = (unsigned)(CI >> lane) & 1u;
+  unsigned hout;
+  const unsigned H = lane_header(start, nl, hin, hout);
+  sep = start;
+  out = ((~H & ~nl & ~st) | start) & 0xFFFFu;
+  bad_low = low & ~H;
+  last_nl = mk_wave_last(my_last_nl);
+  return mk_wave_last(hout);
+}
+
+__device__ __forceinline__ void fp_code4(unsigned xd, unsigned& g, unsigned& nz) {
+  const unsigned c = ((xd >> 1) & 0x03030303u) ^ ((xd >> 2) & 0x01010101u);
+  const unsigned df = __builtin_amdgcn_perm(0u, 0x54474341u, c) ^ xd;
+  nz = (((df & 0x7F7F7F7Fu) + 0x7F7F7F7Fu) | df) & 0x80808080u;
+  const unsigned m1 = nz >> 7;
+  const unsigned ck = c & ~(m1 | (m1 << 1));
+  g = __builtin_amdgcn_udot4(ck, 0x01041040u, 0u, false);
+}
+
+#define FP_SPAN 2048
+#define FP_ROW_WORDS 65
+__device__ __forceinline__ void fp_compact16(unsigned out, unsigned& codes, unsigned& badm) {
+  unsigned drop = ~out & 0xFFFFu;
+  while (drop) {
+    const unsigned a = (unsigned)__builtin_ctz(drop);
+    const unsigned after = out & (0xFFFFu << a);
+    const unsigned b = after ? (unsigned)__builtin_ctz(after) : 16u;
+    const unsigned hi = (unsigned)((u64)codes >> (32 - 2 * a)), lo = codes & (unsigned)((1ull << (2 * (16 - b))) - 1);
+    codes = (unsigned)(((u64)hi << (2 * (16 - b))) | lo);
+    const unsigned bhi = badm >> (16 - a), blo = badm & ((1u << (16 - b)) - 1);
+    badm = (bhi << (16 - b)) | blo;
+    drop &= ~((2u << (b - 1)) - 1);
+  }
+}
+
+__device__ __forceinline__ void fp_row_or(u64* row, unsigned* brow, unsigned at, unsigned cnt, unsigned codes, unsigned badm) {
+  if (cnt == 0) return;
+  const unsigned w = at >> 5, o = at & 31;
+  const u64 top = (u64)codes << (64 - 2 * cnt);
+  const unsigned lsb = __builtin_bitreverse32(badm) >> (32 - cnt);
+  const bool two = o + cnt > 32;
+  if (w < FP_ROW_WORDS) {
+    if (top >> (2 * o)) atomicOr(&row[w], top >> (2 * o));
+    if (lsb << o) atomicOr(&brow[w], lsb << o);
+  }
+  if (two && w + 1 < FP_ROW_WORDS) {
+    if (top << (64 - 2 * o)) atomicOr(&row[w + 1], top << (64 - 2 * o));
+    if (lsb >> (32 - o)) atomicOr(&brow[w + 1], lsb >> (32 - o));
+  }
+}
+
+__device__ __forceinline__ size_t fp_lane16() {
+  unsigned l = threadIdx.x;
+  asm volatile("" : "+v"(l));
+  return (size_t)(l & 63u) * 16;
+}
+
+__device__ __forceinline__ unsigned fp_span_step(const uint8_t* __restrict__ raw, size_t begin, size_t n, size_t pos0, unsigned filled,
+                                                 u64* row, unsigned* brow, unsigned& state, unsigned& prev_nl, unsigned& out,
+                                                 unsigned& sep, unsigned& bl, unsigned& hi, unsigned& badk) {
+  unsigned nl, gt, st, low;
+  const uint4 v = classify16(raw, pos0 + fp_lane16(), begin, n, nl, gt, st, low, hi);
+  unsigned last_nl;
+  state = wave_step(nl, gt, st, low, prev_nl, state, out, sep, bl, last_nl);
+  prev_nl = last_nl;
+  unsigned codes = 0, b8[2] = {0, 0};
+#pragma unroll
+  for (int d = 0; d < 4; ++d) {
+    const unsigned xd = d == 0 ? v.x : (d == 1 ? v.y : (d == 2 ? v.z : v.w));
+    unsigned g, nz;
+    fp_code4(xd, g, nz);
+    codes |= g << (24 - 8 * d);
+    b8[d >> 1] = __builtin_amdgcn_udot4(nz, (d & 1) ? 0x80402010u : 0x08040201u, b8[d >> 1], false);
+  }
+  const unsigned bad16 = ((b8[0] >> 7) | ((b8[1] >> 7) << 8)) | sep;
+  badk = bad16 & out;
+  unsigned badm = __builtin_bitreverse32(bad16) >> 16;
+  const unsigned cnt = __popc(out);
+  if (out != 0xFFFFu) fp_compact16(out, codes, badm);
+  const unsigned inc = mk_wave_scan_incl(cnt);
+  fp_row_or(row, brow, filled + inc - cnt, cnt, codes, badm);
+  return mk_wave_last(inc);
+}
+
+struct FpSpanCounts {
+  unsigned seps = 0, nbad = 0, nhi = 0, low = 0, entry_unknown = 0;
+};
+
+__device__ __forceinline__ unsigned fp_span_pack(const uint8_t* __restrict__ raw, size_t begin, size_t n, size_t s0,
+                                                 u64* row, unsigned* brow, FpSpanCounts& cnt, unsigned& tail) {
+  const int lane = threadIdx.x & 63;
+  row[lane] = 0;
+  brow[lane] = 0;
+  if (lane == 0) { row[64] = 0; brow[64] = 0; }
+  unsigned state = 0, prev_nl = 1;
+  if (s0 > begin) {
+    unsigned nl, gt, st, low, hi;
+    (void)classify16(raw, s0 - 1024 + fp_lane16(), begin, n, nl, gt, st, low, hi);
+    const u64 has = __ballot(nl != 0);
+    if (has == 0) {
+      cnt.entry_unknown = 1;
+      prev_nl = 0;
+    } else {
+      const int L = 63 - __builtin_clzll(has);
+      const unsigned nlL = (unsigned)__builtin_amdgcn_readlane((int)nl, L);
+      const int hb = 31 - __builtin_clz(nlL);
+      const unsigned gtL = (unsigned)__builtin_amdgcn_readlane((int)gt, L);
+      const unsigned gtN = (unsigned)__builtin_amdgcn_readlane((int)gt, L < 63 ? L + 1 : 63);
+      state = hb < 15 ? (gtL >> (hb + 1)) & 1u : (L < 63 ? gtN & 1u : 0u);
+      prev_nl = ((unsigned)__builtin_amdgcn_readlane((int)nl, 63) >> 15) & 1u;
+    }
+  }
+  __builtin_amdgcn_fence(__ATOMIC_RELEASE, "wavefront");
+  __builtin_amdgcn_wave_barrier();
+  __builtin_amdgcn_fence(__ATOMIC_ACQUIRE, "wavefront");
+  unsigned filled = 0;
+#pragma unroll 1
+  for (int sub = 0; sub < FP_SPAN / 1024; ++sub) {
+    unsigned out, sep, bl, hi, badk;
+    filled += fp_span_step(raw, begin, n, s0 + (size_t)sub * 1024, filled, row, brow, state, prev_nl, out, sep, bl, hi, badk);
+    cnt.low |= bl;
+    cnt.seps += __popc(sep);
+    cnt.nbad += __popc(badk & ~sep);
+    cnt.nhi += __popc(hi & out & ~sep);
+  }
+  tail = state | (prev_nl << 1);
+  return filled;
+}
+
+__device__ __forceinline__ void fp_span_finish(const uint8_t* __restrict__ raw, size_t begin, size_t n, size_t s0, int k,
+                                               u64* row, unsigned* brow, unsigned own, unsigned tail, const u64* next_row,
+                                               const unsigned* next_brow, unsigned next_own) {
+  const int lane = threadIdx.x & 63;
+  const unsigned L = (unsigned)(k - 1);
+  unsigned filled = own;
+  unsigned state = tail & 1u;
+  if (state == 0 && s0 + FP_SPAN < n) {
+    if (next_row && next_own >= L) {
+      if (lane == 0) {
+        const u64 top = L ? next_row[0] & ~(~0ull >> (2 * L)) : 0ull;
+        const unsigned bl = next_brow[0] & ((1u << L) - 1);
+        const unsigned w = own >> 5, o = own & 31;
+        if (top >> (2 * o)) atomicOr(&row[w], top >> (2 * o));
+        if (bl << o) atomicOr(&brow[w], bl << o);
+        if (o + L > 32) {
+          if (top << (64 - 2 * o)) atomicOr(&row[w + 1], top << (64 - 2 * o));
+          if (bl >> (32 - o)) atomicOr(&brow[w + 1], bl >> (32 - o));
+        }
+      }
+      filled = own + L;
+    } else {
+      unsigned prev_nl = tail >> 1;
+      size_t pos = s0 + FP_SPAN;
+      while (state == 0 && pos < n && filled - own < L) {
+        unsigned out, sep, bl, hi, badk;
+        filled += fp_span_step(raw, begin, n, pos, filled, row, brow, state, prev_nl, out, sep, bl, hi, badk);
+        if (__ballot(sep != 0)) break;
+        pos += 1024;
+      }
+    }
+  }
+  const unsigned w = (unsigned)lane;
+  if (filled < 32 * (w + 1)) atomicOr(&brow[w], filled <= 32 * w ? ~0u : ~0u << (filled - 32 * w));
+  if (lane == 0 && filled < 32 * 65) atomicOr(&brow[64], filled <= 32 * 64 ? ~0u : ~0u << (filled - 32 * 64));
+  __builtin_amdgcn_fence(__ATOMIC_RELEASE, "wavefront");
+  __builtin_amdgcn_wave_barrier();
+  __builtin_amdgcn_fence(__ATOMIC_ACQUIRE, "wavefront");
+}
diff --git a/mercat2_amd/csrc/mk_skmer.hip b/mercat2_amd/csrc/mk_skmer.hip
--- a/mercat2_amd/csrc/mk_skmer.hip
+++ b/mercat2_amd/csrc/mk_skmer.hip
@@ -1,4 +1,5 @@
 #include "mk_skmer_dev.h"
+#include "mk_fparse_dev.h"
 #include <cstdlib>
 #include <cstdio>
 #include <vector>
@@ -282,11 +283,14 @@
 #endif
 #define SKQ_WAVES (SKQ_THREADS / 64)
 #define SKQ_WALKED 0xFFFFFFFFu
-template <int W, bool CANON, int SKQ_SUBT, int SKQ_QCAP>
+template <int W, bool CANON, int SKQ_SUBT, int SKQ_QCAP, bool RAW>
 __global__ __launch_bounds__(SKQ_THREADS) __attribute__((amdgpu_waves_per_eu(4, 4))) void mk_sk_scatterq_k(const u64* __restrict__ codes, const u64* __restrict__ bad,
                                                          MkChunkInfo* __restrict__ info, const u64* __restrict__ start,
                                                          SkCursor* __restrict__ cursor, ulonglong2* __restrict__ part,
-                                                         int p1_log2, int k, int nkmax, size_t ntiles, unsigned qcap, int nseg) {
+                                                         int p1_log2, int k, int nkmax, size_t ntiles, unsigned qcap, int nseg,
+                                                         const uint8_t* __restrict__ raw, size_t raw_begin, size_t raw_n) {
+  static_assert(!RAW || SKQ_SUBT == 2, "raw-text scatter: two sub-tiles");
+  static_assert(!RAW || FP_SPAN == 64 * SK_R, "a wave's span is its lanes' windows");
   SkCursor* const shared_cursor = cursor + ((size_t)8 << p1_log2);
   const u64* const shared_start = start + ((size_t)8 << p1_log2);
   if (nseg > 1) {
@@ -299,8 +303,13 @@
   __shared__ unsigned lh[SK_LH];
   __shared__ u64 pk_x[SKQ_SUBT][SKQ_WAVES][65];
   __shared__ unsigned queue[SKQ_SUBT][SKQ_WAVES][SKQ_QCAP];
+  __shared__ unsigned brow[RAW ? SKQ_SUBT : 1][SKQ_WAVES][RAW ? FP_ROW_WORDS : 1];
+  __shared__ unsigned s_own[RAW ? SKQ_SUBT : 1][SKQ_WAVES];
+  __shared__ unsigned s_tail[RAW ? SKQ_SUBT : 1][SKQ_WAVES];
+  __shared__ unsigned long long s_cnt[RAW ? 5 : 1];
   __shared__ unsigned s_abort;
   if (threadIdx.x == 0) s_abort = info->part_overflow != 0;
+  if (RAW && threadIdx.x < 5) s_cnt[threadIdx.x] = 0;
   __syncthreads();
   if (s_abort) return;
   unsigned spilled = 0;
@@ -308,10 +317,21 @@
   const unsigned p1 = 1u << p1_log2;
   const unsigned lhn = p1 < (unsigned)SK_LH ? p1 : (unsigned)SK_LH;
   const unsigned nround = p1 / lhn;
-  const size_t seq_len = info->seq_len;
+  const size_t seq_len = RAW ? 0 : info->seq_len;
   const int lane = threadIdx.x & 63;
 #define wv sk_wave_id()
   auto sk_wave_id = [&]() { int w = (int)threadIdx.x; asm volatile("" : "+v"(w)); return w >> 6; };
+  auto valid_of = [&](int st, size_t p0, bool& has) -> unsigned {
+    if constexpr (RAW) {
+      const unsigned own = s_own[st][wv], j0 = (unsigned)lane * SK_R;
+      has = j0 < own;
+      const unsigned mine = !has ? 0u : (own - j0 >= SK_R ? ~0u : (1u << (own - j0)) - 1);
+      return sk_valid32((u64)brow[st][wv][lane] | ((u64)brow[st][wv][lane + 1] << 32), k) & mine;
+    } else {
+      has = p0 < seq_len;
+      return has ? sk_valid32(bad_window(bad, p0), k) : 0u;
+    }
+  };
   for (unsigned i = threadIdx.x; i < lhn; i += blockDim.x) lh[i] = 0;
   __syncthreads();
   u64 tA = 0, tB = 0, tC = 0, tD = 0, tE = 0, tF = 0, t0 = 0, ntile = 0;
@@ -320,6 +340,31 @@
   for (size_t tile = blockIdx.x; tile < ntiles; tile += gridDim.x) {
     ntile += 1;
     unsigned qn[SKQ_SUBT];
+    if constexpr (RAW) {
+#pragma unroll
+      for (int st = 0; st < SKQ_SUBT; ++st) {
+        const size_t s0 = ((tile * SKQ_SUBT + st) * SKQ_WAVES + wv) * (size_t)FP_SPAN;
+        unsigned own = 0, tail = 1;
+        if (s0 < raw_n) {
+          FpSpanCounts pc;
+          own = fp_span_pack(raw, raw_begin, raw_n, s0, pk_x[st][wv], brow[st][wv], pc, tail);
+          const unsigned seps = mk_wave_sum(pc.seps), nbad = mk_wave_sum(pc.nbad), nhi = mk_wave_sum(pc.nhi);
+          const u64 low = __ballot(pc.low != 0), unk = __ballot(pc.entry_unknown != 0);
+          if (lane == 0) {
+            atomicAdd(&s_cnt[0], (unsigned long long)own);
+            if (seps) atomicAdd(&s_cnt[1], (unsigned long long)seps);
+            if (nbad) atomicAdd(&s_cnt[2], (unsigned long long)nbad);
+            if (nhi) atomicAdd(&s_cnt[3], (unsigned long long)nhi);
+            if (low || unk) atomicOr(&s_cnt[4], (low ? 1ull : 0ull) | (unk ? 2ull : 0ull));
+          }
+        } else {
+          pk_x[st][wv][lane] = 0;
+          if (lane == 63) pk_x[st][wv][64] = 0;
+        }
+        if (lane == 0) { s_own[st][wv] = own; s_tail[st][wv] = tail; }
+      }
+      __syncthreads();
+    }
 #pragma unroll
     for (int st = 0; st < SKQ_SUBT; ++st) {
       const size_t t = (tile * SKQ_SUBT + st) * SKQ_THREADS + threadIdx.x;
@@ -329,15 +374,35 @@
       runs.starts = 0;
       runs.pos[0] = runs.pos[1] = runs.pos[2] = runs.pos[3] = 0;
       u64 ww0 = 0, ww1 = 0;
-      if (p0 < seq_len) {
-        ww0 = codes[t];
-        ww1 = codes[t + 1];
-        runs = sk_analyse<W>(ww0, ww1, sk_valid32(bad_window(bad, p0), k), CANON);
-      } else if (p0 < seq_len + SK_R) {
-        ww0 = codes[t];
-      }
-      pk_x[st][wv][lane] = ww0;
-      if (lane == 63) pk_x[st][wv][64] = ww1;
+      if constexpr (RAW) {
+        const size_t s0 = ((tile * SKQ_SUBT + st) * SKQ_WAVES + wv) * (size_t)FP_SPAN;
+        const unsigned own = s_own[st][wv];
+        if (s0 < raw_n) {
+          const bool last_w = wv == SKQ_WAVES - 1;
+          const int nst = last_w ? st + 1 : st, nwv = last_w ? 0 : wv + 1;
+          const bool in_wg = nst < SKQ_SUBT;
+          const int cst = in_wg ? nst : st, cwv = in_wg ? nwv : wv;
+          fp_span_finish(raw, raw_begin, raw_n, s0, k, pk_x[st][wv], brow[st][wv], own, s_tail[st][wv],
+                         in_wg ? pk_x[cst][cwv] : nullptr, brow[cst][cwv], in_wg ? s_own[cst][cwv] : 0u);
+        }
+        bool has;
+        const unsigned valid = valid_of(st, p0, has);
+        if (has) {
+          ww0 = pk_x[st][wv][lane];
+          ww1 = pk_x[st][wv][lane + 1];
+          runs = sk_analyse<W>(ww0, ww1, valid, CANON);
+        }
+      } else {
+        if (p0 < seq_len) {
+          ww0 = codes[t];
+          ww1 = codes[t + 1];
+          runs = sk_analyse<W>(ww0, ww1, sk_valid32(bad_window(bad, p0), k), CANON);
+        } else if (p0 < seq_len + SK_R) {
+          ww0 = codes[t];
+        }
+        pk_x[st][wv][lane] = ww0;
+        if (lane == 63) pk_x[st][wv][64] = ww1;
+      }
       const unsigned s2 = sk_cut_starts(runs.starts, runs.valid, nkmax);
       const unsigned cnt = __popc(s2);
       const unsigned inc = mk_wave_scan_incl(cnt);
@@ -374,7 +439,7 @@
         }
         qn[st] = total;
       } else {
-        if (p0 < seq_len)
+        if (runs.valid)
           sk_walk(runs, ww0, ww1, nkmax, CANON, [&](int, int, unsigned mm) {
             const unsigned b = sk_bucket(mm, p1_log2);
             if ((b >> SK_LH_LOG2) == 0) atomicAdd(&lh[b & (SK_LH - 1)], 1u);
@@ -402,9 +467,11 @@
         } else {
           const size_t t = (tile * SKQ_SUBT + st) * SKQ_THREADS + threadIdx.x;
           const size_t p0 = t * SK_R;
-          if (p0 < seq_len) {
+          bool has;
+          const unsigned valid = valid_of(st, p0, has);
+          if (has) {
             const ulonglong2 w = make_ulonglong2(pk_x[st][wv][lane], pk_x[st][wv][lane + 1]);
-            const SkRuns runs = sk_analyse<W>(w.x, w.y, sk_valid32(bad_window(bad, p0), k), CANON);
+            const SkRuns runs = sk_analyse<W>(w.x, w.y, valid, CANON);
             sk_walk(runs, w.x, w.y, nkmax, CANON, [&](int, int, unsigned mm) {
               const unsigned b = sk_bucket(mm, p1_log2);
               if ((b >> SK_LH_LOG2) == round) atomicAdd(&lh[b & (SK_LH - 1)], 1u);
@@ -492,9 +559,11 @@
       } else {
         const size_t t = (tile * SKQ_SUBT + st) * SKQ_THREADS + threadIdx.x;
         const size_t p0 = t * SK_R;
-        if (p0 < seq_len) {
+        bool has;
+        const unsigned valid = valid_of(st, p0, has);
+        if (has) {
           const ulonglong2 w = make_ulonglong2(pk_x[st][wv][lane], pk_x[st][wv][lane + 1]);
-          const SkRuns runs = sk_analyse<W>(w.x, w.y, sk_valid32(bad_window(bad, p0), k), CANON);
+          const SkRuns runs = sk_analyse<W>(w.x, w.y, valid, CANON);
           sk_walk(runs, w.x, w.y, nkmax, CANON, [&](int jstart, int nk, unsigned mm) {
             const unsigned b = sk_bucket(mm, p1_log2);
             if ((b >> SK_LH_LOG2) != round) return;
@@ -515,6 +584,17 @@
   if (threadIdx.x == 0 && blockIdx.x < 1024) { u64* d = skq_dbg + (size_t)blockIdx.x * 8; d[0] = tA; d[1] = tB; d[2] = tC; d[3] = tD; d[4] = tE; d[5] = tF; d[6] = ntile; }
 #endif
   if (spilled) atomicOr(&info->part_overflow, 4ull);
+  if constexpr (RAW) {
+    __syncthreads();
+    if (threadIdx.x == 0) {
+      const unsigned long long sl = s_cnt[0], sp = s_cnt[1];
+      if (sl) atomicAdd(&info->seq_len, sl);
+      if (sl - sp) atomicAdd(&info->symbols, sl - sp);
+      if (s_cnt[2]) atomicAdd(&info->bad_symbols, s_cnt[2]);
+      if (s_cnt[3]) atomicAdd(&info->non_ascii, s_cnt[3]);
+      if (s_cnt[4]) atomicOr(&info->parse_fallback, s_cnt[4]);
+    }
+  }
 }
 #undef wv
 
@@ -561,7 +641,7 @@
 
 template <int W, bool CANON>
 static void launch_wc(mk_ctx* c, size_t seq_len, int p1_log2, int nkmax, int sample_log2, u64 surv_div, u64 part_cap, u64 surv_cap,
-                     u64* hist, u64* start, SkCursor* cursor, u64* khist, u64* kstart, bool reuse, int nseg) {
+                     u64* hist, u64* start, SkCursor* cursor, u64* khist, u64* kstart, bool reuse, int nseg, bool raw) {
   MkChunkInfo* info = (MkChunkInfo*)c->info.p;
   float sigmas = 6.0f;
   if (const char* e = getenv("MK_SAMPLE_SIGMAS")) sigmas = (float)atof(e);
@@ -578,6 +658,14 @@
                       surv_cap, sigmas, nseg);
   }
   static const bool walked = getenv("MK_SCATTER_WALK") != nullptr;
+  if (raw) {
+    const size_t n_al = c->raw_src_begin + c->raw_src_n;
+    const size_t rtiles = div_up(n_al, (size_t)2 * SKQ_THREADS * SK_R);
+    hipLaunchKernelGGL((mk_sk_scatterq_k<W, CANON, 2, 512, true>), dim3((unsigned)(rtiles < SK_SCAT_GRID ? rtiles : SK_SCAT_GRID)),
+                       dim3(SKQ_THREADS), 0, c->stream, (const u64*)nullptr, (const u64*)nullptr, info, (const u64*)start, cursor,
+                       (ulonglong2*)c->part.p, p1_log2, c->k, nkmax, rtiles, 512u, nseg, c->raw_src, c->raw_src_begin, n_al);
+    return;
+  }
   const int force_subt = getenv("MK_SKQ_SUBT") ? atoi(getenv("MK_SKQ_SUBT")) : 0;
   const bool three = force_subt == 3 || (force_subt != 2 && c->items_hint > 0 && c->items_hint * 64.0 + 48.0 < 376.0);
   unsigned qcap = three ? 376u : 512u;
@@ -590,11 +678,13 @@
     const size_t qtiles = div_up(threads, (size_t)SKQ_THREADS * (three ? 3 : 2));
     const dim3 qgrid((unsigned)(qtiles < SK_SCAT_GRID ? qtiles : SK_SCAT_GRID));
     if (three)
-      hipLaunchKernelGGL((mk_sk_scatterq_k<W, CANON, 3, 376>), qgrid, dim3(SKQ_THREADS), 0, c->stream, (const u64*)c->codes.p,
-                         (const u64*)c->bad.p, info, (const u64*)start, cursor, (ulonglong2*)c->part.p, p1_log2, c->k, nkmax, qtiles, qcap, nseg);
+      hipLaunchKernelGGL((mk_sk_scatterq_k<W, CANON, 3, 376, false>), qgrid, dim3(SKQ_THREADS), 0, c->stream, (const u64*)c->codes.p,
+                         (const u64*)c->bad.p, info, (const u64*)start, cursor, (ulonglong2*)c->part.p, p1_log2, c->k, nkmax, qtiles, qcap, nseg,
+                         (const uint8_t*)nullptr, (size_t)0, (size_t)0);
     else
-      hipLaunchKernelGGL((mk_sk_scatterq_k<W, CANON, 2, 512>), qgrid, dim3(SKQ_THREADS), 0, c->stream, (const u64*)c->codes.p,
-                         (const u64*)c->bad.p, info, (const u64*)start, cursor, (ulonglong2*)c->part.p, p1_log2, c->k, nkmax, qtiles, qcap, nseg);
+      hipLaunchKernelGGL((mk_sk_scatterq_k<W, CANON, 2, 512, false>), qgrid, dim3(SKQ_THREADS), 0, c->stream, (const u64*)c->codes.p,
+                         (const u64*)c->bad.p, info, (const u64*)start, cursor, (ulonglong2*)c->part.p, p1_log2, c->k, nkmax, qtiles, qcap, nseg,
+                         (const uint8_t*)nullptr, (size_t)0, (size_t)0);
   }
 #ifdef MK_STAMP
   if (!walked) {
@@ -614,10 +704,10 @@
 
 template <bool CANON>
 static bool sk_partition(int W, mk_ctx* c, size_t seq_len, int p1_log2, int nkmax, int sample_log2, u64 surv_div, u64 part_cap, u64 surv_cap,
-                         u64* hist, u64* start, SkCursor* cursor, u64* khist, u64* kstart, bool reuse, int nseg) {
+                         u64* hist, u64* start, SkCursor* cursor, u64* khist, u64* kstart, bool reuse, int nseg, bool raw) {
   switch (W) {
 #define SK_CASE(W_)                                                                                                      \
-  case W_: launch_wc<W_, CANON>(c, seq_len, p1_log2, nkmax, sample_log2, surv_div, part_cap, surv_cap, hist, start, cursor, khist, kstart, reuse, nseg); return true;
+  case W_: launch_wc<W_, CANON>(c, seq_len, p1_log2, nkmax, sample_log2, surv_div, part_cap, surv_cap, hist, start, cursor, khist, kstart, reuse, nseg, raw); return true;
     SK_CASE(2) SK_CASE(3) SK_CASE(4) SK_CASE(5) SK_CASE(6) SK_CASE(7)
     SK_CASE(8) SK_CASE(9) SK_CASE(10) SK_CASE(11) SK_CASE(12) SK_CASE(13) SK_CASE(14) SK_CASE(15) SK_CASE(16)
     SK_CASE(17) SK_CASE(18) SK_CASE(19) SK_CASE(20) SK_CASE(21) SK_CASE(22)
@@ -628,12 +718,12 @@
 
 #ifdef SK_TU_CANON
 bool mk_sk_partition_canon(int W, mk_ctx* c, size_t seq_len, int p1_log2, int nkmax, int sample_log2, u64 surv_div, u64 part_cap,
-                           u64 surv_cap, u64* hist, u64* start, SkCursor* cursor, u64* khist, u64* kstart, bool reuse, int nseg) {
-  return sk_partition<true>(W, c, seq_len, p1_log2, nkmax, sample_log2, surv_div, part_cap, surv_cap, hist, start, cursor, khist, kstart, reuse, nseg);
+                           u64 surv_cap, u64* hist, u64* start, SkCursor* cursor, u64* khist, u64* kstart, bool reuse, int nseg, bool raw) {
+  return sk_partition<true>(W, c, seq_len, p1_log2, nkmax, sample_log2, surv_div, part_cap, surv_cap, hist, start, cursor, khist, kstart, reuse, nseg, raw);
 }
 #else
 bool mk_sk_partition_canon(int W, mk_ctx* c, size_t seq_len, int p1_log2, int nkmax, int sample_log2, u64 surv_div, u64 part_cap,
-                           u64 surv_cap, u64* hist, u64* start, SkCursor* cursor, u64* khist, u64* kstart, bool reuse, int nseg);
+                           u64 surv_cap, u64* hist, u64* start, SkCursor* cursor, u64* khist, u64* kstart, bool reuse, int nseg, bool raw);
 
 bool mk_part_inherit(mk_ctx* c, size_t seq_len, int p1_log2, uint64_t min_count, bool sampled, bool exact) {
   if (c->part_cooldown > 0 && !exact) c->part_cooldown -= 1;
@@ -685,6 +775,12 @@
   c->part_nseg = nseg;
   const bool reuse = mk_part_inherit(c, seq_len, p1_log2, min_count, sample_log2 != 0, exact);
   int rc;
+  const bool raw = c->parse_deferred && reuse;
+  if (c->parse_deferred && !raw &&
+      (rc = mk_launch_fparse(c, c->raw_src, c->raw_src_begin, c->raw_src_n, true, false)) != MK_OK)
+    return rc;
+  c->parse_deferred = false;
+  c->raw_scattered = raw;
   if ((rc = mk_buf_reserve(c, c->part_meta, (7 * p1 + 16 + 14 * p1 + 8) * sizeof(u64))) != MK_OK) return rc;
   const size_t part_cap = nseg > 1 ? 2 * seq_len + 64 : seq_len + 64;
   if ((rc = mk_buf_reserve(c, c->part, part_cap * sizeof(ulonglong2))) != MK_OK) return rc;
@@ -709,11 +805,11 @@
   if (!reuse) MK_HIP(hipMemsetAsync(hist, 0, (7 * p1 + 8) * sizeof(u64), c->stream));
   mk_prof_begin(c, MK_K_PART);
   if (c->canonical) {
-    if (!mk_sk_partition_canon(k - SK_M + 1, c, seq_len, p1_log2, nkmax, sample_log2, surv_div, (u64)part_cap, (u64)surv_cap, hist, start, cursor, khist, kstart, reuse, nseg)) {
+    if (!mk_sk_partition_canon(k - SK_M + 1, c, seq_len, p1_log2, nkmax, sample_log2, surv_div, (u64)part_cap, (u64)surv_cap, hist, start, cursor, khist, kstart, reuse, nseg, raw)) {
       c->err = "mk_launch_count_superkmer: k out of range";
       return MK_ERR_ARG;
     }
-  } else if (!sk_partition<false>(k - SK_M + 1, c, seq_len, p1_log2, nkmax, sample_log2, surv_div, (u64)part_cap, (u64)surv_cap, hist, start, cursor, khist, kstart, reuse, nseg)) {
+  } else if (!sk_partition<false>(k - SK_M + 1, c, seq_len, p1_log2, nkmax, sample_log2, surv_div, (u64)part_cap, (u64)surv_cap, hist, start, cursor, khist, kstart, reuse, nseg, raw)) {
     c->err = "mk_launch_count_superkmer: k out of range";
     return MK_ERR_ARG;
   }
diff --git a/mercat2_amd/native.py b/mercat2_amd/native.py
--- a/mercat2_amd/native.py
+++ b/mercat2_amd/native.py
@@ -53,7 +53,8 @@
                [(n, C.c_double) for n in ("ms_parse", "ms_pack", "ms_count", "ms_exotic", "ms_filter", "ms_export")] + \
                [(n, C.c_uint64) for n in ("n_parse", "n_pack", "n_count", "n_exotic", "n_filter", "n_export")] + \
                [("ms_part", C.c_double), ("n_part", C.c_uint64), ("records", C.c_uint64), ("distinct", C.c_uint64),
-                ("part_retries", C.c_uint64), ("part_reused", C.c_uint64), ("fused_chunks", C.c_uint64), ("fuse_spilled", C.c_uint64), ("parse_retries", C.c_uint64)]
+                ("part_retries", C.c_uint64), ("part_reused", C.c_uint64), ("fused_chunks", C.c_uint64), ("fuse_spilled", C.c_uint64), ("parse_retries", C.c_uint64),
+                ("raw_scattered", C.c_uint64)]
 
     def as_dict(self):
         return {n: getattr(self, n) for n, _ in self._fields_}
```

Result: faster. 164.1 billion (median of 6 runs) (+2.7%).
